# Wu0409/DuPL

Hardware: AMD Instinct MI355X
Metric: training img/s at 448^2, VOC dual-student ViT-B/16, phase B step (higher is better)
Workload: dtype f32 storage / accumulation / results; Linear GEMMs (forward, dgrad, wgrad), attention (forward, backward) and the decoder convs as fp32-equivalent f16x3 split products on the f16 MFMA (operands as fp16 hi / lo planes, 3 products per block, fp32 accumulate; error vs fp64 <= the f32 MFMA kernels'); CA

## Files before the change

### dupl_amd/csrc/attn_split.hip

```cpp
#include "common.h"
#include <type_traits>
#include "../../include/dupl_hip.h"

#ifndef ATT_PRIO
#define ATT_PRIO 0
#endif
#ifndef ATT_ABL
#define ATT_ABL 0
#endif

namespace {

typedef _Float16 h8 __attribute__((ext_vector_type(8)));
typedef _Float16 h4 __attribute__((ext_vector_type(4)));
typedef float f32x2 __attribute__((ext_vector_type(2)));
template <int N, int I = 0, class F>
__device__ __forceinline__ void static_for(F&& f) {
    if constexpr (I < N) {
        f(std::integral_constant<int, I>{});
        static_for<N, I + 1>(f);
    }
}
constexpr float LO_INV = 1.f / DUPL_LO_SCALE;
constexpr int HD = 64, KT = 64;
constexpr int PLANE = KT * 128;
constexpr int STAGE = 4 * PLANE;

#define MFMA16(a, b, c) __builtin_amdgcn_mfma_f32_32x32x16_f16((a), (b), (c), 0, 0, 0)

__device__ __forceinline__ float fast_exp(float x) { return __builtin_amdgcn_exp2f(x * 1.4426950408889634f); }

__device__ __forceinline__ void xcd_remap3(int remap, int& bx, int& by, int& bz) {
    bx = blockIdx.x; by = blockIdx.y; bz = blockIdx.z;
    if (!remap) return;
    const int gx = gridDim.x, gy = gridDim.y;
    const int total = gx * gy * gridDim.z;
    const int L = bx + gx * (by + gy * bz);
    const int q = total >> 3, r = total & 7;
    const int xcd = L & 7, idx = L >> 3;
    const int w = (xcd < r ? xcd * (q + 1) : r * (q + 1) + (xcd - r) * q) + idx;
    bx = w % gx;
    by = (w / gx) % gy;
    bz = w / (gx * gy);
}

struct AttnSegs {
    int n;
    int row0[DUPL_ATTN_SEGS_MAX], B[DUPL_ATTN_SEGS_MAX], N[DUPL_ATTN_SEGS_MAX], B_f32[DUPL_ATTN_SEGS_MAX], first[DUPL_ATTN_SEGS_MAX + 1];
    float* out[DUPL_ATTN_SEGS_MAX];
    float* lse[DUPL_ATTN_SEGS_MAX];
};

__global__ __launch_bounds__(256, 2) void attn_fwd16_kernel(const __half* __restrict__ qkv_hi, const __half* __restrict__ qkv_lo,
                                                            __half* __restrict__ out_hi, __half* __restrict__ out_lo,
                                                            const AttnSegs segs, int H, float scale, int remap, float out_scale) {
    __shared__ __attribute__((aligned(1024))) char smem[2 * STAGE];
    const int tid = threadIdx.x, lane = tid & 63, l31 = lane & 31, hf = lane >> 5;
    const int wave = __builtin_amdgcn_readfirstlane(tid >> 6);
    int sg = 0;
#pragma unroll 1
    while (sg + 1 < segs.n && (int)blockIdx.x >= segs.first[sg + 1]) ++sg;
    sg = __builtin_amdgcn_readfirstlane(sg);
    const int N = segs.N[sg], B_f32 = segs.B_f32[sg];
    float* __restrict__ out = segs.out[sg];
    float* __restrict__ lse = segs.lse[sg];
    int bx, h, b;
    {
        const int gx = (N + 127) / 128;
        const int G = gx * H * segs.B[sg];
        const int L = (int)blockIdx.x - segs.first[sg];
        int w = L;
        if (remap) {
            const int q = G >> 3, r = G & 7;
            const int xcd = L & 7, idx = L >> 3;
            w = (xcd < r ? xcd * (q + 1) : r * (q + 1) + (xcd - r) * q) + idx;
        }
        bx = w % gx; h = (w / gx) % H; b = w / (gx * H);
    }
    {
        const size_t r0 = (size_t)segs.row0[sg];
        qkv_hi += r0 * (size_t)(3 * H * HD);
        qkv_lo += r0 * (size_t)(3 * H * HD);
        if (out_hi) { out_hi += r0 * (size_t)(H * HD); out_lo += r0 * (size_t)(H * HD); }
    }
    const int q0 = bx * 128 + wave * 32;
    const int D = H * HD, ld = 3 * D;
    const int qrow = q0 + l31;
    const bool wave_active = q0 < N;

    h8 qh[4], ql[4];
    {
        const size_t off = ((size_t)b * N + min(qrow, N - 1)) * ld + h * HD + 8 * hf;
#pragma unroll
        for (int s = 0; s < 4; ++s) {
            qh[s] = *reinterpret_cast<const h8*>(qkv_hi + off + 16 * s);
            ql[s] = *reinterpret_cast<const h8*>(qkv_lo + off + 16 * s);
        }
    }

    const int prow = lane >> 3, pch = lane & 7;
    const char* kbase[2];
    kbase[0] = reinterpret_cast<const char*>(qkv_hi + (size_t)b * N * ld + D + h * HD);
    kbase[1] = reinterpret_cast<const char*>(qkv_lo + (size_t)b * N * ld + D + h * HD);
    const char* vbase[2];
    vbase[0] = kbase[0] + D * 2;
    vbase[1] = kbase[1] + D * 2;
    int krow[2], kch[2], vrow[2];
    const int vch = ((lane >> 5) * 32 + (lane & 3) * 8) * 2;
#pragma unroll
    for (int j = 0; j < 2; ++j) {
        const int r = 8 * (wave + 4 * j) + prow;
        const int c = pch ^ ((r >> 1) & 7);
        krow[j] = r;
        kch[j] = c * 16;
        const int q = wave + 4 * j, srow = (lane >> 2) & 7;
        vrow[j] = (q >> 1) * 16 + (srow >> 2) * 8 + (q & 1) * 4 + (srow & 3);
    }
    const size_t tstride = (size_t)KT * ld * 2;
    unsigned koff[2], voff[2];
#pragma unroll
    for (int j = 0; j < 2; ++j) {
        koff[j] = (unsigned)krow[j] * (unsigned)(ld * 2) + kch[j];
        voff[j] = (unsigned)vrow[j] * (unsigned)(ld * 2) + vch;
    }
    auto dma16 = [](const char* ubase, const unsigned off, char* dst) __attribute__((always_inline)) {
        __builtin_amdgcn_global_load_lds((const __attribute__((address_space(1))) void*)(ubase + off),
                                         (__attribute__((address_space(3))) void*)dst, 16, 0, 0);
    };
    auto issue = [&](int t, int buf) __attribute__((always_inline)) {
        char* dst = smem + buf * STAGE + wave * 1024;
        const size_t o = t * tstride;
        if (t * KT + KT <= N) {
#pragma unroll
            for (int i = 0; i < 4; ++i) dma16(kbase[i >> 1] + o, koff[i & 1], dst + i * 4096);
#pragma unroll
            for (int i = 0; i < 4; ++i) dma16(vbase[i >> 1] + o, voff[i & 1], dst + (4 + i) * 4096);
        } else {
#pragma unroll
            for (int i = 0; i < 4; ++i)
                dma16(kbase[i >> 1] + o, (unsigned)(min(t * KT + krow[i & 1], N - 1) - t * KT) * (unsigned)(ld * 2) + kch[i & 1], dst + i * 4096);
#pragma unroll
            for (int i = 0; i < 4; ++i)
                dma16(vbase[i >> 1] + o, (unsigned)(min(t * KT + vrow[i & 1], N - 1) - t * KT) * (unsigned)(ld * 2) + vch, dst + (4 + i) * 4096);
        }
    };

    const int g4 = (l31 >> 2) & 3;
    const int krow_a = (l31 & ~12) | ((g4 == 1 ? 2 : (g4 == 2 ? 1 : g4)) << 2);
    const int k_off = krow_a * 128, k_sw = (krow_a >> 1) & 7;
    const int vg = lane >> 4, vq = lane & 15;
    const unsigned v_lds = (unsigned)(uintptr_t)((__attribute__((address_space(3))) char*)smem) + 2 * PLANE +
                           ((vg >> 1) * 4 + (vq >> 2)) * 64 + (16 * (vg & 1) + 4 * (vq & 3)) * 2;

    f32x16 oM[2], oX[2];
#pragma unroll
    for (int d = 0; d < 2; ++d)
#pragma unroll
        for (int e = 0; e < 16; ++e) { oM[d][e] = 0.f; oX[d][e] = 0.f; }
    float m_run = -INFINITY, l_run = 0.f;

    const int nkt = (N + KT - 1) / KT;
    long long tph[4] = {0, 0, 0, 0}, tlast = 0;
    if (ATT_ABL & 16) tlast = clock64();
#define ATT_STAMP(i)                                  \
    if (ATT_ABL & 16) {                               \
        const long long now_ = clock64();             \
        tph[i] += now_ - tlast;                       \
        tlast = now_;                                 \
    }
    issue(0, 0);
    for (int t = 0; t < nkt; ++t) {
        asm volatile("s_waitcnt vmcnt(0)" ::: "memory");
        __syncthreads();
        if (t + 1 < nkt) issue(t + 1, (t + 1) & 1);
        if (!wave_active) continue;
        const char* st = smem + (t & 1) * STAGE;
        ATT_STAMP(0)

        f32x16 sM[2], sX[2];
        const f32x16 zero16 = {0.f, 0.f, 0.f, 0.f, 0.f, 0.f, 0.f, 0.f, 0.f, 0.f, 0.f, 0.f, 0.f, 0.f, 0.f, 0.f};
        h8 kh[2][2], kl[2][2];
        auto k_read = [&](const int sstep, h8(&fh)[2], h8(&fl)[2]) __attribute__((always_inline)) {
            const int ch = ((2 * sstep + hf) ^ k_sw) * 16;
#pragma unroll
            for (int kt2 = 0; kt2 < 2; ++kt2) {
                fh[kt2] = *reinterpret_cast<const h8*>(st + kt2 * 4096 + k_off + ch);
                fl[kt2] = *reinterpret_cast<const h8*>(st + PLANE + kt2 * 4096 + k_off + ch);
            }
        };
        k_read(0, kh[0], kl[0]);
        __builtin_amdgcn_s_setprio(ATT_PRIO);
#pragma unroll
        for (int sstep = 0; sstep < 4; ++sstep) {
            const int cur = sstep & 1;
            if (sstep + 1 < 4) k_read(sstep + 1, kh[cur ^ 1], kl[cur ^ 1]);
            __builtin_amdgcn_sched_barrier(0);
            sM[0] = MFMA16(kh[cur][0], qh[sstep], sstep == 0 ? zero16 : sM[0]);
            sM[1] = MFMA16(kh[cur][1], qh[sstep], sstep == 0 ? zero16 : sM[1]);
            sX[0] = MFMA16(kh[cur][0], ql[sstep], sstep == 0 ? zero16 : sX[0]);
            sX[1] = MFMA16(kh[cur][1], ql[sstep], sstep == 0 ? zero16 : sX[1]);
            sX[0] = MFMA16(kl[cur][0], qh[sstep], sX[0]);
            sX[1] = MFMA16(kl[cur][1], qh[sstep], sX[1]);
            __builtin_amdgcn_sched_barrier(0);
        }
        __builtin_amdgcn_s_setprio(0);
        if (ATT_ABL & 16) { asm volatile("" ::"v"(sM[0]), "v"(sM[1]), "v"(sX[0]), "v"(sX[1])); }
        ATT_STAMP(1)
        h4 vf[2][8];
        const unsigned v_st = v_lds + (t & 1) * STAGE;
        auto tr_read = [](const unsigned addr, auto offc) __attribute__((always_inline)) {
            h4 v;
            asm volatile("ds_read_b64_tr_b16 %0, %1 offset:%2" : "=v"(v) : "v"(addr), "n"(decltype(offc)::value) : "memory");
            return v;
        };
        auto v_read = [&](auto sgc, h4(&f)[8]) __attribute__((always_inline)) {
            constexpr int SG = decltype(sgc)::value;
            static_for<8>([&](auto ic) __attribute__((always_inline)) {
                constexpr int i = decltype(ic)::value, pl = i >> 2, dd = (i >> 1) & 1, jj = i & 1;
                f[i] = tr_read(v_st, std::integral_constant<int, pl * PLANE + ((SG * 2 + jj) * 2 + dd) * 512>{});
            });
        };
        v_read(std::integral_constant<int, 0>{}, vf[0]);
        const float c1 = scale * 1.4426950408889634f, c2 = c1 * LO_INV;
        if (t == nkt - 1) {
            const int kbase_t = t * KT + 8 * hf;
#pragma unroll
            for (int kt2 = 0; kt2 < 2; ++kt2)
#pragma unroll
                for (int e = 0; e < 16; ++e)
                    if (kbase_t + 32 * kt2 + 16 * (e >> 3) + (e & 7) >= N) sM[kt2][e] = -INFINITY;
        }
        float mx = -INFINITY;
#pragma unroll
        for (int kt2 = 0; kt2 < 2; ++kt2)
#pragma unroll
            for (int e = 0; e < 16; ++e) mx = fmaxf(mx, sM[kt2][e]);
        {
            typedef unsigned u2v __attribute__((ext_vector_type(2)));
            const u2v sw = __builtin_amdgcn_permlane32_swap(__float_as_uint(mx), __float_as_uint(mx), false, false);
            mx = fmaxf(__uint_as_float(sw[0]), __uint_as_float(sw[1])) * c1;
        }
        const float m_cand = fmaxf(m_run, mx);
        const bool move = __builtin_amdgcn_ballot_w64(m_cand - m_run > 8.f) != 0;
        const float m_run2 = move ? m_cand : m_run;
        const float m_new = m_run2 == -INFINITY ? 0.f : m_run2;
        const float alpha = __builtin_amdgcn_exp2f(m_run - m_new);
        f32x2 psum2 = {0.f, 0.f};
        h8 ph[4], pl[4];
        typedef _Float16 h2v __attribute__((ext_vector_type(2)));
#pragma unroll
        for (int kt2 = 0; kt2 < 2; ++kt2)
#pragma unroll
            for (int e = 0; e < 16; e += 2) {
                const f32x2 m2 = {sM[kt2][e], sM[kt2][e + 1]}, x2 = {sX[kt2][e], sX[kt2][e + 1]};
                const f32x2 v2 = __builtin_elementwise_fma(x2, f32x2{c2, c2}, __builtin_elementwise_fma(m2, f32x2{c1, c1}, f32x2{-m_new, -m_new}));
                const f32x2 p2 = {__builtin_amdgcn_exp2f(v2[0]), __builtin_amdgcn_exp2f(v2[1])};
                psum2 += p2;
                const h2v hh = __builtin_convertvector(p2, h2v);
                const f32x2 q2 = p2 * f32x2{DUPL_LO_SCALE, DUPL_LO_SCALE};
                const int idx = 2 * kt2 + (e >> 3);
                ph[idx][e & 7] = hh[0];
                ph[idx][(e & 7) + 1] = hh[1];
                pl[idx][e & 7] = (_Float16)__builtin_fmaf((float)hh[0], -DUPL_LO_SCALE, q2[0]);
                pl[idx][(e & 7) + 1] = (_Float16)__builtin_fmaf((float)hh[1], -DUPL_LO_SCALE, q2[1]);
            }
        const float psum = psum2[0] + psum2[1];
        l_run = l_run * alpha + psum;
        if (move) {
#pragma unroll
            for (int d = 0; d < 2; ++d)
#pragma unroll
                for (int e = 0; e < 16; ++e) { oM[d][e] *= alpha; oX[d][e] *= alpha; }
        }
        m_run = m_run2;
        if (ATT_ABL & 16) { asm volatile("" ::"v"(ph[0]), "v"(ph[3]), "v"(pl[0]), "v"(pl[3]), "v"(oM[0]), "v"(oX[1])); }
        ATT_STAMP(2)
        __builtin_amdgcn_s_setprio(ATT_PRIO);
        static_for<4>([&](auto sgc) __attribute__((always_inline)) {
            constexpr int sg = decltype(sgc)::value, cur = sg & 1;
            if constexpr (sg + 1 < 4) {
                v_read(std::integral_constant<int, sg + 1>{}, vf[cur ^ 1]);
                asm volatile("s_waitcnt lgkmcnt(8)" ::: "memory");
            } else {
                asm volatile("s_waitcnt lgkmcnt(0)" ::: "memory");
            }
            __builtin_amdgcn_sched_barrier(0);
            const h4(&f)[8] = vf[cur];
            const h8 vh0 = __builtin_shufflevector(f[0], f[1], 0, 1, 2, 3, 4, 5, 6, 7), vh1 = __builtin_shufflevector(f[2], f[3], 0, 1, 2, 3, 4, 5, 6, 7);
            const h8 vl0 = __builtin_shufflevector(f[4], f[5], 0, 1, 2, 3, 4, 5, 6, 7), vl1 = __builtin_shufflevector(f[6], f[7], 0, 1, 2, 3, 4, 5, 6, 7);
            oM[0] = MFMA16(vh0, ph[sg], oM[0]);
            oM[1] = MFMA16(vh1, ph[sg], oM[1]);
            oX[0] = MFMA16(vh0, pl[sg], oX[0]);
            oX[1] = MFMA16(vh1, pl[sg], oX[1]);
            oX[0] = MFMA16(vl0, ph[sg], oX[0]);
            oX[1] = MFMA16(vl1, ph[sg], oX[1]);
            __builtin_amdgcn_sched_barrier(0);
        });
        __builtin_amdgcn_s_setprio(0);
        if (ATT_ABL & 16) { asm volatile("" ::"v"(oM[0]), "v"(oM[1]), "v"(oX[0]), "v"(oX[1])); }
        ATT_STAMP(3)
    }
    if ((ATT_ABL & 16) && lse && tid == 0) {
        long long* q = reinterpret_cast<long long*>(lse + (((size_t)gridDim.z * H * N + 1) & ~(size_t)1)) +
                       (size_t)(blockIdx.x + gridDim.x * (blockIdx.y + gridDim.y * blockIdx.z)) * 4;
        q[0] = tph[0]; q[1] = tph[1]; q[2] = tph[2]; q[3] = tph[3];
    }
    if (!wave_active) return;
    const float l_tot = l_run + __shfl_xor(l_run, 32, 64);
    const float inv = 1.f / l_tot;
    if (b >= B_f32) { out = nullptr; lse = nullptr; }
    if (qrow < N) {
        const size_t ro = ((size_t)b * N + qrow) * D + h * HD;
#pragma unroll
        for (int d = 0; d < 2; ++d)
#pragma unroll
            for (int g = 0; g < 4; ++g) {
                float v[4];
#pragma unroll
                for (int j = 0; j < 4; ++j) v[j] = (oM[d][4 * g + j] + oX[d][4 * g + j] * LO_INV) * inv;
                const int col = d * 32 + 8 * g + 4 * hf;
                if (out) *reinterpret_cast<float4*>(out + ro + col) = make_float4(v[0], v[1], v[2], v[3]);
                if (out_hi) {
                    __half hh[4], ll[4];
#pragma unroll
                    for (int j = 0; j < 4; ++j) {
                        if (out_scale > 0.f) split_f32_u(v[j] * out_scale, hh[j], ll[j]);
                        else split_f32(v[j], hh[j], ll[j]);
                    }
                    *reinterpret_cast<uint2*>(out_hi + ro + col) = *reinterpret_cast<const uint2*>(hh);
                    *reinterpret_cast<uint2*>(out_lo + ro + col) = *reinterpret_cast<const uint2*>(ll);
                }
            }
        if (lse && hf == 0) lse[((size_t)b * H + h) * N + qrow] = m_run * 0.6931471805599453f + logf(l_tot);
    }
}


}

constexpr int g_attn16_remap = 1;

static int attn_fwd16_launch(const void* qkv_hi, const void* qkv_lo, void* out_hi, void* out_lo, const dupl_attn_seg* sv, int32_t n,
                             int32_t H, int32_t hd, float scale, int32_t out_exp, dupl_stream_t s) {
    if (out_exp < 0 || out_exp > 15 || !sv || n < 1 || n > DUPL_ATTN_SEGS_MAX) return DUPL_ERR_ARG;
    if (!qkv_hi || !qkv_lo || ((out_hi == nullptr) != (out_lo == nullptr)) || H <= 0 || hd != HD) return DUPL_ERR_ARG;
    auto al16 = [](const void* q) { return (reinterpret_cast<uintptr_t>(q) & 15) == 0; };
    if (!al16(qkv_hi) || !al16(qkv_lo)) return DUPL_ERR_ARG;
    int order[DUPL_ATTN_SEGS_MAX];
    for (int i = 0; i < n; ++i) order[i] = i;
    for (int i = 1; i < n; ++i)
        for (int j = i; j > 0 && sv[order[j]].N > sv[order[j - 1]].N; --j) { const int t = order[j]; order[j] = order[j - 1]; order[j - 1] = t; }
    AttnSegs g;
    g.n = n;
    int total = 0;
    for (int k = 0; k < n; ++k) {
        const dupl_attn_seg& q = sv[order[k]];
        int bf = q.B_f32 == 0 ? q.B : q.B_f32;
        if (q.B <= 0 || q.N <= 0 || q.row0 < 0 || bf < 0 || bf > q.B || (!q.out && !out_hi) || (bf < q.B && q.out && !out_hi)) return DUPL_ERR_ARG;
        g.row0[k] = (int)q.row0; g.B[k] = q.B; g.N[k] = q.N; g.B_f32[k] = bf; g.out[k] = q.out; g.lse[k] = q.lse;
        g.first[k] = total;
        total += ((q.N + 127) / 128) * H * q.B;
    }
    g.first[n] = total;
    DUPL_LAUNCH(attn_fwd16_kernel, dim3((unsigned)total), dim3(256), 0, (hipStream_t)s, (const __half*)qkv_hi, (const __half*)qkv_lo,
                       (__half*)out_hi, (__half*)out_lo, g, H, scale, g_attn16_remap, out_exp ? ldexpf(1.f, out_exp) : 0.f);
    return dupl_launch_status();
}

extern "C" int dupl_attention_fwd16(const void* qkv_hi, const void* qkv_lo, float* out, void* out_hi, void* out_lo, float* lse,
                                    int32_t B, int32_t N, int32_t H, int32_t hd, float scale, int32_t B_f32, int32_t out_exp,
                                    dupl_stream_t s) {
    if (B_f32 < 0 || B_f32 > B || (B_f32 != 0 && B_f32 < B && !out_hi) || (!out && !out_hi)) return DUPL_ERR_ARG;
    dupl_attn_seg q;
    q.row0 = 0; q.B = B; q.N = N; q.B_f32 = B_f32; q.out = out; q.lse = lse;
    return attn_fwd16_launch(qkv_hi, qkv_lo, out_hi, out_lo, &q, 1, H, hd, scale, out_exp, s);
}

extern "C" int dupl_attention_fwd16_segs(const void* qkv_hi, const void* qkv_lo, void* out_hi, void* out_lo, const dupl_attn_seg* segs,
                                         int32_t n, int32_t H, int32_t hd, float scale, int32_t out_exp, dupl_stream_t s) {
    return attn_fwd16_launch(qkv_hi, qkv_lo, out_hi, out_lo, segs, n, H, hd, scale, out_exp, s);
}
```

### dupl_amd/csrc/attn_split_bwd.hip

```cpp
#include "common.h"
#include "../../include/dupl_hip.h"

namespace {

typedef _Float16 h8 __attribute__((ext_vector_type(8)));
typedef _Float16 h4 __attribute__((ext_vector_type(4)));
constexpr float LO_INV = 1.f / DUPL_LO_SCALE;
constexpr int HD = 64, TT = 32;
constexpr int PL = 4096;
constexpr int MAXN = 2048;

#define MFMA16(a, b, c) __builtin_amdgcn_mfma_f32_32x32x16_f16((a), (b), (c), 0, 0, 0)

__device__ __forceinline__ float fast_exp(float x) { return __builtin_amdgcn_exp2f(x * 1.4426950408889634f); }

__device__ __forceinline__ void xcd_remap3(int remap, int& bx, int& by, int& bz) {
    bx = blockIdx.x; by = blockIdx.y; bz = blockIdx.z;
    if (!remap) return;
    const int gx = gridDim.x, gy = gridDim.y;
    const int total = gx * gy * gridDim.z;
    const int L = bx + gx * (by + gy * bz);
    const int q = total >> 3, r = total & 7;
    const int xcd = L & 7, idx = L >> 3;
    const int w = (xcd < r ? xcd * (q + 1) : r * (q + 1) + (xcd - r) * q) + idx;
    bx = w % gx;
    by = (w / gx) % gy;
    bz = w / (gx * gy);
}

__device__ __forceinline__ void dma16(const char* src, char* dst) {
    __builtin_amdgcn_global_load_lds((const __attribute__((address_space(1))) void*)src,
                                     (__attribute__((address_space(3))) void*)dst, 16, 0, 0);
}

__device__ __forceinline__ int pi_row(int r) {
    const int g = (r >> 2) & 3;
    return (r & ~12) | ((g == 1 ? 2 : (g == 2 ? 1 : g)) << 2);
}

__device__ __forceinline__ int km_piece_row(int wave, int lane) {
    const int srow = (lane >> 2) & 7;
    return (wave >> 1) * 16 + (srow >> 2) * 8 + (wave & 1) * 4 + (srow & 3);
}
__device__ __forceinline__ int km_piece_col_bytes(int lane) { return ((lane >> 5) * 32 + (lane & 3) * 8) * 2; }
__device__ __forceinline__ int km_read_lane_off(int lane) {
    const int g = lane >> 4, q = lane & 15;
    return ((g >> 1) * 4 + (q >> 2)) * 64 + (16 * (g & 1) + 4 * (q & 3)) * 2;
}
template <int OFF>
__device__ __forceinline__ h4 km_tr_read(const unsigned addr) {
    h4 v;
    asm volatile("ds_read_b64_tr_b16 %0, %1 offset:%2" : "=v"(v) : "v"(addr), "n"(OFF) : "memory");
    return v;
}
__device__ __forceinline__ void km_read_tile(const unsigned base_hi, h4 (&f)[8][2]) {
#define KM_RD(SG, DD, PLN, JJ) f[((SG) * 2 + (DD)) * 2 + (PLN)][JJ] = km_tr_read<(PLN) * PL + (((SG) * 2 + (JJ)) * 2 + (DD)) * 512>(base_hi)
    KM_RD(0, 0, 0, 0); KM_RD(0, 0, 0, 1); KM_RD(0, 0, 1, 0); KM_RD(0, 0, 1, 1);
    KM_RD(0, 1, 0, 0); KM_RD(0, 1, 0, 1); KM_RD(0, 1, 1, 0); KM_RD(0, 1, 1, 1);
    KM_RD(1, 0, 0, 0); KM_RD(1, 0, 0, 1); KM_RD(1, 0, 1, 0); KM_RD(1, 0, 1, 1);
    KM_RD(1, 1, 0, 0); KM_RD(1, 1, 0, 1); KM_RD(1, 1, 1, 0); KM_RD(1, 1, 1, 1);
#undef KM_RD
}
__device__ __forceinline__ void km_wait(h4 (&f)[8][2]) {
    asm volatile("s_waitcnt lgkmcnt(0)"
                 : "+v"(f[0][0]), "+v"(f[0][1]), "+v"(f[1][0]), "+v"(f[1][1]), "+v"(f[2][0]), "+v"(f[2][1]), "+v"(f[3][0]), "+v"(f[3][1]),
                   "+v"(f[4][0]), "+v"(f[4][1]), "+v"(f[5][0]), "+v"(f[5][1]), "+v"(f[6][0]), "+v"(f[6][1]), "+v"(f[7][0]), "+v"(f[7][1])
                 :
                 : "memory");
    __builtin_amdgcn_sched_barrier(0);
}
__device__ __forceinline__ h8 h8of(const h4 lo, const h4 hi) { return __builtin_shufflevector(lo, hi, 0, 1, 2, 3, 4, 5, 6, 7); }

__device__ __forceinline__ void split_regs(const f32x16& v, h8 (&hi)[2], h8 (&lo)[2]) {
    typedef _Float16 h2v __attribute__((ext_vector_type(2)));
    typedef float f2v __attribute__((ext_vector_type(2)));
#pragma unroll
    for (int e = 0; e < 16; e += 2) {
        const f2v x2 = {v[e], v[e + 1]};
        const h2v hh = __builtin_convertvector(x2, h2v);
        const f2v q2 = x2 * f2v{DUPL_LO_SCALE, DUPL_LO_SCALE};
        hi[e >> 3][e & 7] = hh[0];
        hi[e >> 3][(e & 7) + 1] = hh[1];
        lo[e >> 3][e & 7] = (_Float16)__builtin_fmaf((float)hh[0], -DUPL_LO_SCALE, q2[0]);
        lo[e >> 3][(e & 7) + 1] = (_Float16)__builtin_fmaf((float)hh[1], -DUPL_LO_SCALE, q2[1]);
    }
}

__device__ __forceinline__ void attn_bwd_amax_flush(unsigned int* amax_out, float amx) {
    if (!amax_out) return;
    amx = wave_max(amx);
    if ((threadIdx.x & 63) == 0 && amx > 0.f) atomicMax(amax_out, __float_as_uint(amx));
}

__global__ __launch_bounds__(256) void delta_kernel(const float* __restrict__ out, const float* __restrict__ dout,
                                                    float* __restrict__ delta, int B, int N, int H) {
    const long idx = (long)blockIdx.x * blockDim.x + threadIdx.x;
    const long total = (long)B * N * H;
    if (idx >= total) return;
    const int h = (int)(idx % H);
    const long bn = idx / H;
    const int n = (int)(bn % N), b = (int)(bn / N);
    const float4* o = reinterpret_cast<const float4*>(out + bn * (long)(H * HD) + h * HD);
    const float4* d = reinterpret_cast<const float4*>(dout + bn * (long)(H * HD) + h * HD);
    float s = 0.f;
#pragma unroll
    for (int i = 0; i < HD / 4; ++i) {
        const float4 a = o[i], c = d[i];
        s += (a.x * c.x + a.y * c.y) + (a.z * c.z + a.w * c.w);
    }
    delta[((long)b * H + h) * N + n] = s;
}

__device__ __forceinline__ void attn_bwd16_dq_body(char* __restrict__ smem, const int bx, const int h, const int b,
                                                   const __half* __restrict__ qkv_hi, const __half* __restrict__ qkv_lo,
                                                   const __half* __restrict__ do_hi, const __half* __restrict__ do_lo,
                                                   const float* __restrict__ lse, const float* __restrict__ delta,
                                                   const float* __restrict__ slot, float* __restrict__ dqkv, unsigned int* __restrict__ amax_out, int N, int H,
                                                   float scale) {
    constexpr int STAGE = 6 * PL;
    const int tid = threadIdx.x, lane = tid & 63, wave = tid >> 6, l31 = lane & 31, hf = lane >> 5;
    const int q0 = bx * 128 + wave * 32;
    const int D = H * HD, ld = 3 * D;
    const int qrow = q0 + l31;
    const bool wave_active = q0 < N, qv = qrow < N;
    const float s_do = slot[0], inv_s = slot[1];

    h8 qh[4], ql[4], oh[4], ol[4];
    {
        const int rr = min(qrow, N - 1);
        const size_t qo = ((size_t)b * N + rr) * ld + h * HD + 8 * hf;
        const size_t oo = ((size_t)b * N + rr) * D + h * HD + 8 * hf;
#pragma unroll
        for (int s = 0; s < 4; ++s) {
            qh[s] = *reinterpret_cast<const h8*>(qkv_hi + qo + 16 * s);
            ql[s] = *reinterpret_cast<const h8*>(qkv_lo + qo + 16 * s);
            oh[s] = *reinterpret_cast<const h8*>(do_hi + oo + 16 * s);
            ol[s] = *reinterpret_cast<const h8*>(do_lo + oo + 16 * s);
        }
    }
    const float my_lse = qv ? lse[((size_t)b * H + h) * N + qrow] : 0.f;
    const float my_delta = qv ? delta[((size_t)b * H + h) * N + qrow] * s_do : 0.f;

    const int rrow = 8 * wave + (lane >> 3), rch = ((lane & 7) ^ ((rrow >> 1) & 7)) * 16;
    const int trow = km_piece_row(wave, lane), tcb = km_piece_col_bytes(lane);
    const char* k_hi = reinterpret_cast<const char*>(qkv_hi + (size_t)b * N * ld + D + h * HD);
    const char* k_lo = reinterpret_cast<const char*>(qkv_lo + (size_t)b * N * ld + D + h * HD);
    auto issue = [&](int t, int buf) __attribute__((always_inline)) {
        char* dst = smem + buf * STAGE + wave * 1024;
        const size_t ro = (size_t)min(t * TT + rrow, N - 1) * (ld * 2) + rch;
        dma16(k_hi + ro, dst);
        dma16(k_lo + ro, dst + PL);
        dma16(k_hi + ro + D * 2, dst + 2 * PL);
        dma16(k_lo + ro + D * 2, dst + 3 * PL);
        const size_t to = (size_t)min(t * TT + trow, N - 1) * (ld * 2) + tcb;
        dma16(k_hi + to, dst + 4 * PL);
        dma16(k_lo + to, dst + 5 * PL);
    };
    const int prow = pi_row(l31);
    const int a_off = prow * 128, a_sw = (prow >> 1) & 7;
    const unsigned km_lds = (unsigned)(uintptr_t)((__attribute__((address_space(3))) char*)smem) + 4 * PL + km_read_lane_off(lane);

    f32x16 dqM[2], dqX[2];
#pragma unroll
    for (int d = 0; d < 2; ++d)
#pragma unroll
        for (int e = 0; e < 16; ++e) { dqM[d][e] = 0.f; dqX[d][e] = 0.f; }

    const int nkt = (N + TT - 1) / TT;
    issue(0, 0);
    for (int t = 0; t < nkt; ++t) {
        asm volatile("s_waitcnt vmcnt(0)" ::: "memory");
        __syncthreads();
        if (t + 1 < nkt) issue(t + 1, (t + 1) & 1);
        if (!wave_active) continue;
        const char* st = smem + (t & 1) * STAGE;
        f32x16 sM, sX, pM, pX;
#pragma unroll
        for (int e = 0; e < 16; ++e) { sM[e] = 0.f; sX[e] = 0.f; pM[e] = 0.f; pX[e] = 0.f; }
#pragma unroll
        for (int s = 0; s < 4; ++s) {
            const int ch = ((2 * s + hf) ^ a_sw) * 16;
            const h8 kh = *reinterpret_cast<const h8*>(st + a_off + ch);
            const h8 kl = *reinterpret_cast<const h8*>(st + PL + a_off + ch);
            const h8 vh = *reinterpret_cast<const h8*>(st + 2 * PL + a_off + ch);
            const h8 vl = *reinterpret_cast<const h8*>(st + 3 * PL + a_off + ch);
            sM = MFMA16(kh, qh[s], sM);
            sX = MFMA16(kh, ql[s], sX);
            sX = MFMA16(kl, qh[s], sX);
            pM = MFMA16(vh, oh[s], pM);
            pX = MFMA16(vh, ol[s], pX);
            pX = MFMA16(vl, oh[s], pX);
        }
        const int kb = t * TT + 8 * hf;
        f32x16 ds;
#pragma unroll
        for (int e = 0; e < 16; ++e) {
            const bool kvld = kb + 16 * (e >> 3) + (e & 7) < N;
            const float sv = (sM[e] + sX[e] * LO_INV) * scale;
            const float p = kvld ? fast_exp(sv - my_lse) : 0.f;
            ds[e] = __fmul_rn(p, __fsub_rn(pM[e] + pX[e] * LO_INV, my_delta));
        }
        h4 kf[8][2];
        km_read_tile(km_lds + (t & 1) * STAGE, kf);
        h8 dh[2], dl[2];
        split_regs(ds, dh, dl);
        km_wait(kf);
#pragma unroll
        for (int sg = 0; sg < 2; ++sg) {
#pragma unroll
            for (int d = 0; d < 2; ++d) {
                const h8 th = h8of(kf[(sg * 2 + d) * 2][0], kf[(sg * 2 + d) * 2][1]);
                const h8 tl = h8of(kf[(sg * 2 + d) * 2 + 1][0], kf[(sg * 2 + d) * 2 + 1][1]);
                dqM[d] = MFMA16(th, dh[sg], dqM[d]);
                dqX[d] = MFMA16(th, dl[sg], dqX[d]);
                dqX[d] = MFMA16(tl, dh[sg], dqX[d]);
            }
        }
    }
    float amx = 0.f;
    if (wave_active && qv) {
        const float f = scale * inv_s;
        float* op = dqkv + ((size_t)b * N + qrow) * ld + h * HD;
#pragma unroll
        for (int d = 0; d < 2; ++d)
#pragma unroll
            for (int g = 0; g < 4; ++g) {
                float4 v;
                v.x = (dqM[d][4 * g + 0] + dqX[d][4 * g + 0] * LO_INV) * f;
                v.y = (dqM[d][4 * g + 1] + dqX[d][4 * g + 1] * LO_INV) * f;
                v.z = (dqM[d][4 * g + 2] + dqX[d][4 * g + 2] * LO_INV) * f;
                v.w = (dqM[d][4 * g + 3] + dqX[d][4 * g + 3] * LO_INV) * f;
                amx = fmaxf(fmaxf(amx, fmaxf(fabsf(v.x), fabsf(v.y))), fmaxf(fabsf(v.z), fabsf(v.w)));
                *reinterpret_cast<float4*>(op + d * 32 + 8 * g + 4 * hf) = v;
            }
    }
    attn_bwd_amax_flush(amax_out, amx);
}

template <int MODE>
__device__ __forceinline__ void attn_bwd16_dkv_body(char* __restrict__ smem, const int bx, const int h, const int b,
                                                    const __half* __restrict__ qkv_hi, const __half* __restrict__ qkv_lo,
                                                    const __half* __restrict__ do_hi, const __half* __restrict__ do_lo,
                                                    const float* __restrict__ lse, const float* __restrict__ delta,
                                                    const float* __restrict__ slot, float* __restrict__ dqkv, unsigned int* __restrict__ amax_out, int N, int H,
                                                    float scale) {
    constexpr int NPL = MODE == 0 ? 4 : 6;
    constexpr int STAGE = NPL * PL;
    float* Ls = reinterpret_cast<float*>(smem + 2 * STAGE);
    float* Ds = Ls + MAXN;
    const int tid = threadIdx.x, lane = tid & 63, wave = tid >> 6, l31 = lane & 31, hf = lane >> 5;
    const int k0 = bx * 128 + wave * 32;
    const int D = H * HD, ld = 3 * D;
    const int krow = k0 + l31;
    const bool wave_active = k0 < N, kv = krow < N;
    const float s_do = slot[0], inv_s = slot[1];

    for (int i = tid; i < N; i += 256) {
        Ls[i] = lse[((size_t)b * H + h) * N + i];
        if (MODE == 1) Ds[i] = delta[((size_t)b * H + h) * N + i] * s_do;
    }

    h8 kh[4], kl[4], vh[4], vl[4];
    {
        const size_t ko = ((size_t)b * N + min(krow, N - 1)) * ld + D + h * HD + 8 * hf;
#pragma unroll
        for (int s = 0; s < 4; ++s) {
            kh[s] = *reinterpret_cast<const h8*>(qkv_hi + ko + 16 * s);
            kl[s] = *reinterpret_cast<const h8*>(qkv_lo + ko + 16 * s);
            if (MODE == 1) {
                vh[s] = *reinterpret_cast<const h8*>(qkv_hi + ko + D + 16 * s);
                vl[s] = *reinterpret_cast<const h8*>(qkv_lo + ko + D + 16 * s);
            }
        }
    }

    const int rrow = 8 * wave + (lane >> 3), rch = ((lane & 7) ^ ((rrow >> 1) & 7)) * 16;
    const int trow = km_piece_row(wave, lane), tcb = km_piece_col_bytes(lane);
    const char* q_hi = reinterpret_cast<const char*>(qkv_hi + (size_t)b * N * ld + h * HD);
    const char* q_lo = reinterpret_cast<const char*>(qkv_lo + (size_t)b * N * ld + h * HD);
    const char* o_hi = reinterpret_cast<const char*>(do_hi + (size_t)b * N * D + h * HD);
    const char* o_lo = reinterpret_cast<const char*>(do_lo + (size_t)b * N * D + h * HD);
    auto issue = [&](int t, int buf) __attribute__((always_inline)) {
        char* dst = smem + buf * STAGE + wave * 1024;
        const int rr = min(t * TT + rrow, N - 1);
        dma16(q_hi + (size_t)rr * (ld * 2) + rch, dst);
        dma16(q_lo + (size_t)rr * (ld * 2) + rch, dst + PL);
        if (MODE == 1) {
            dma16(o_hi + (size_t)rr * (D * 2) + rch, dst + 2 * PL);
            dma16(o_lo + (size_t)rr * (D * 2) + rch, dst + 3 * PL);
        }
        const int tr = min(t * TT + trow, N - 1);
        if (MODE == 0) {
            dma16(o_hi + (size_t)tr * (D * 2) + tcb, dst + (NPL - 2) * PL);
            dma16(o_lo + (size_t)tr * (D * 2) + tcb, dst + (NPL - 1) * PL);
        } else {
            dma16(q_hi + (size_t)tr * (ld * 2) + tcb, dst + (NPL - 2) * PL);
            dma16(q_lo + (size_t)tr * (ld * 2) + tcb, dst + (NPL - 1) * PL);
        }
    };
    const int prow = pi_row(l31);
    const int a_off = prow * 128, a_sw = (prow >> 1) & 7;
    const unsigned km_lds = (unsigned)(uintptr_t)((__attribute__((address_space(3))) char*)smem) + (NPL - 2) * PL + km_read_lane_off(lane);

    f32x16 gM[2], gX[2];
#pragma unroll
    for (int d = 0; d < 2; ++d)
#pragma unroll
        for (int e = 0; e < 16; ++e) { gM[d][e] = 0.f; gX[d][e] = 0.f; }

    const int nqt = (N + TT - 1) / TT;
    issue(0, 0);
    for (int t = 0; t < nqt; ++t) {
        asm volatile("s_waitcnt vmcnt(0)" ::: "memory");
        __syncthreads();
        if (t + 1 < nqt) issue(t + 1, (t + 1) & 1);
        if (!wave_active) continue;
        const char* st = smem + (t & 1) * STAGE;
        f32x16 sM, sX, pM, pX;
#pragma unroll
        for (int e = 0; e < 16; ++e) { sM[e] = 0.f; sX[e] = 0.f; pM[e] = 0.f; pX[e] = 0.f; }
#pragma unroll
        for (int s = 0; s < 4; ++s) {
            const int ch = ((2 * s + hf) ^ a_sw) * 16;
            const h8 ah = *reinterpret_cast<const h8*>(st + a_off + ch);
            const h8 al = *reinterpret_cast<const h8*>(st + PL + a_off + ch);
            sM = MFMA16(ah, kh[s], sM);
            sX = MFMA16(ah, kl[s], sX);
            sX = MFMA16(al, kh[s], sX);
            if (MODE == 1) {
                const h8 bh = *reinterpret_cast<const h8*>(st + 2 * PL + a_off + ch);
                const h8 bl = *reinterpret_cast<const h8*>(st + 3 * PL + a_off + ch);
                pM = MFMA16(bh, vh[s], pM);
                pX = MFMA16(bh, vl[s], pX);
                pX = MFMA16(bl, vh[s], pX);
            }
        }
        const int qb = t * TT + 8 * hf;
        f32x16 w;
#pragma unroll
        for (int e = 0; e < 16; ++e) {
            const int qi = qb + 16 * (e >> 3) + (e & 7);
            const bool ok = qi < N && kv;
            const int qc = min(qi, N - 1);
            const float sv = (sM[e] + sX[e] * LO_INV) * scale;
            const float p = ok ? fast_exp(sv - Ls[qc]) : 0.f;
            w[e] = MODE == 0 ? p : __fmul_rn(p, __fsub_rn(pM[e] + pX[e] * LO_INV, Ds[qc]));
        }
        h4 xf[8][2];
        km_read_tile(km_lds + (t & 1) * STAGE, xf);
        h8 wh[2], wl[2];
        split_regs(w, wh, wl);
        km_wait(xf);
#pragma unroll
        for (int sg = 0; sg < 2; ++sg) {
#pragma unroll
            for (int d = 0; d < 2; ++d) {
                const h8 th = h8of(xf[(sg * 2 + d) * 2][0], xf[(sg * 2 + d) * 2][1]);
                const h8 tl = h8of(xf[(sg * 2 + d) * 2 + 1][0], xf[(sg * 2 + d) * 2 + 1][1]);
                gM[d] = MFMA16(th, wh[sg], gM[d]);
                gX[d] = MFMA16(th, wl[sg], gX[d]);
                gX[d] = MFMA16(tl, wh[sg], gX[d]);
            }
        }
    }
    float amx = 0.f;
    if (wave_active && kv) {
        const float f = MODE == 0 ? inv_s : scale * inv_s;
        float* op = dqkv + ((size_t)b * N + krow) * ld + (MODE == 0 ? 2 * D : D) + h * HD;
#pragma unroll
        for (int d = 0; d < 2; ++d)
#pragma unroll
            for (int g = 0; g < 4; ++g) {
                float4 v;
                v.x = (gM[d][4 * g + 0] + gX[d][4 * g + 0] * LO_INV) * f;
                v.y = (gM[d][4 * g + 1] + gX[d][4 * g + 1] * LO_INV) * f;
                v.z = (gM[d][4 * g + 2] + gX[d][4 * g + 2] * LO_INV) * f;
                v.w = (gM[d][4 * g + 3] + gX[d][4 * g + 3] * LO_INV) * f;
                amx = fmaxf(fmaxf(amx, fmaxf(fabsf(v.x), fabsf(v.y))), fmaxf(fabsf(v.z), fabsf(v.w)));
                *reinterpret_cast<float4*>(op + d * 32 + 8 * g + 4 * hf) = v;
            }
    }
    attn_bwd_amax_flush(amax_out, amx);
}

constexpr int ATTNB_LDS = 2 * 6 * PL + 2 * MAXN * 4;
__global__ __launch_bounds__(256, 2) void attn_bwd16_all_kernel(const __half* __restrict__ qkv_hi, const __half* __restrict__ qkv_lo,
                                                                const __half* __restrict__ do_hi, const __half* __restrict__ do_lo,
                                                                const float* __restrict__ lse, const float* __restrict__ delta,
                                                                const float* __restrict__ slot, float* __restrict__ dqkv,
                                                                unsigned int* __restrict__ amax_out, int N, int H, int B, float scale,
                                                                int remap) {
    __shared__ __attribute__((aligned(1024))) char smem[ATTNB_LDS];
    const int gx = (N + 127) / 128;
    const int G = gx * H * B;
    const int role = __builtin_amdgcn_readfirstlane((int)blockIdx.x / G);
    const int L = (int)blockIdx.x - role * G;
    int w = L;
    if (remap) {
        const int q = G >> 3, r = G & 7;
        const int xcd = L & 7, idx = L >> 3;
        w = (xcd < r ? xcd * (q + 1) : r * (q + 1) + (xcd - r) * q) + idx;
    }
    const int bx = w % gx, h = (w / gx) % H, b = w / (gx * H);
    if (role == 0) attn_bwd16_dkv_body<1>(smem, bx, h, b, qkv_hi, qkv_lo, do_hi, do_lo, lse, delta, slot, dqkv, amax_out, N, H, scale);
    else if (role == 1) attn_bwd16_dq_body(smem, bx, h, b, qkv_hi, qkv_lo, do_hi, do_lo, lse, delta, slot, dqkv, amax_out, N, H, scale);
    else attn_bwd16_dkv_body<0>(smem, bx, h, b, qkv_hi, qkv_lo, do_hi, do_lo, lse, delta, slot, dqkv, amax_out, N, H, scale);
}

}

constexpr int g_attnb16_remap = 1;

extern "C" int dupl_attention_bwd16(const void* qkv_hi, const void* qkv_lo, const float* out, const float* dout, const void* do_hi,
                                    const void* do_lo, const float* do_slot, const float* lse, float* delta, float* dqkv, int32_t B,
                                    int32_t N, int32_t H, int32_t hd, float scale, void* amax_out, dupl_stream_t stream) {
    unsigned int* ax = static_cast<unsigned int*>(amax_out);
    if (!qkv_hi || !qkv_lo || !out || !dout || !do_hi || !do_lo || !do_slot || !lse || !delta || !dqkv || B <= 0 || N <= 0 ||
        N > MAXN || H <= 0 || hd != HD)
        return DUPL_ERR_ARG;
    hipStream_t s = (hipStream_t)stream;
    const long total = (long)B * N * H;
    DUPL_LAUNCH(delta_kernel, dim3((unsigned)((total + 255) / 256)), dim3(256), 0, s, out, dout, delta, B, N, H);
    const unsigned blocks = 3u * (unsigned)(((N + 127) / 128) * H * B);
    DUPL_LAUNCH(attn_bwd16_all_kernel, dim3(blocks), dim3(256), 0, s, (const __half*)qkv_hi, (const __half*)qkv_lo,
                       (const __half*)do_hi, (const __half*)do_lo, lse, delta, do_slot, dqkv, ax, N, H, B, scale, g_attnb16_remap);
    return dupl_launch_status();
}
```

### dupl_amd/engine.py

```python
from __future__ import annotations

import os
from dataclasses import dataclass, field
from typing import Dict, List, Optional, Tuple

import torch

from . import ops

Tensor = torch.Tensor

GEMM_MODE = os.environ.get("DUPL_GEMM", "f16x3")


def set_gemm_mode(mode: str):
    global GEMM_MODE
    assert mode in ("f32", "f16x3"), mode
    GEMM_MODE = mode


@dataclass(frozen=True)
class EncoderConfig:
    embed_dim: int = 768
    depth: int = 12
    num_heads: int = 12
    mlp_ratio: int = 4
    patch: int = 16
    img_size: int = 224
    aux_layer: int = -3
    ln_eps: float = 1e-6
    head_classes: int = 1000
    decoder_dim: int = 512
    decoder_dilation: int = 5

    @property
    def grid(self) -> int:
        return self.img_size // self.patch

    @property
    def head_dim(self) -> int:
        return self.embed_dim // self.num_heads


def student_param_shapes(cfg: EncoderConfig, num_classes: int) -> Dict[str, Tuple[int, ...]]:
    D, Hd = cfg.embed_dim, cfg.embed_dim * cfg.mlp_ratio
    s: Dict[str, Tuple[int, ...]] = {}
    s["encoder.cls_token"] = (1, 1, D)
    s["encoder.pos_embed"] = (1, cfg.grid * cfg.grid + 1, D)
    s["encoder.patch_embed.proj.weight"] = (D, 3, cfg.patch, cfg.patch)
    s["encoder.patch_embed.proj.bias"] = (D,)
    for i in range(cfg.depth):
        p = f"encoder.blocks.{i}."
        s[p + "norm1.weight"] = (D,)
        s[p + "norm1.bias"] = (D,)
        s[p + "attn.qkv.weight"] = (3 * D, D)
        s[p + "attn.qkv.bias"] = (3 * D,)
        s[p + "attn.proj.weight"] = (D, D)
        s[p + "attn.proj.bias"] = (D,)
        s[p + "norm2.weight"] = (D,)
        s[p + "norm2.bias"] = (D,)
        s[p + "mlp.fc1.weight"] = (Hd, D)
        s[p + "mlp.fc1.bias"] = (Hd,)
        s[p + "mlp.fc2.weight"] = (D, Hd)
        s[p + "mlp.fc2.bias"] = (D,)
    s["encoder.norm.weight"] = (D,)
    s["encoder.norm.bias"] = (D,)
    s["encoder.head.weight"] = (cfg.head_classes, D)
    s["encoder.head.bias"] = (cfg.head_classes,)
    s["decoder.conv6.weight"] = (cfg.decoder_dim, D, 3, 3)
    s["decoder.conv7.weight"] = (cfg.decoder_dim, cfg.decoder_dim, 3, 3)
    s["decoder.conv8.weight"] = (num_classes, cfg.decoder_dim, 1, 1)
    s["classifier.weight"] = (num_classes - 1, D, 1, 1)
    s["aux_classifier.weight"] = (num_classes - 1, D, 1, 1)
    return s


SEG_FROZEN, SEG_BACKBONE, SEG_NORM, SEG_CLS, SEG_DECODER = 0, 1, 2, 3, 4


def param_segment(key: str) -> int:
    if key in ("encoder.pos_embed", "encoder.head.weight", "encoder.head.bias"):
        return SEG_FROZEN
    if key.startswith("encoder."):
        return SEG_NORM if "norm" in key[len("encoder."):] else SEG_BACKBONE
    if key.startswith("decoder."):
        return SEG_DECODER
    return SEG_CLS


FMT1 = os.environ.get("DUPL_FMT1", "1") != "0"
KM_BWD = os.environ.get("DUPL_KM_BWD", "1") != "0"
SK_DGRAD = os.environ.get("DUPL_SK_DGRAD", "1") != "0"
WGRAD_GROUP = os.environ.get("DUPL_WGRAD_GROUP", "1") != "0"

SK_DGRAD_MAX_COLS = 1024
ZERO_WS = os.environ.get("DUPL_ZERO_WS", "1") != "0"
FUSED_PLANES = os.environ.get("DUPL_ADAMW_PLANES", "1") != "0"
MERGED_PASS = int(os.environ.get("DUPL_MERGED_PASS", "16384"))
ATTN_SEGS = int(os.environ.get("DUPL_ATTN_SEGS", "1536"))


class FlatStorage:

    def __init__(self, cfg: EncoderConfig, num_classes: int, n_students: int, device="cpu"):
        self.cfg, self.num_classes, self.n_students = cfg, num_classes, n_students
        shapes = student_param_shapes(cfg, num_classes)
        self.shapes = shapes
        self.layout: Dict[str, Tuple[int, int]] = {}
        self.seg_bounds: List[Tuple[int, int]] = []
        off = 0
        for seg in range(5):
            start = off
            for k, shp in shapes.items():
                if param_segment(k) != seg:
                    continue
                n = 1
                for d in shp:
                    n *= d
                self.layout[k] = (off, n)
                off += (n + 7) // 8 * 8
            self.seg_bounds.append((start, off))
        self.student_numel = off
        self.data = torch.zeros(n_students * off, dtype=torch.float32, device=device)
        self.grad = torch.zeros(n_students * off, dtype=torch.float32, device=device)
        self.seg_has_grad = [[False] * 5 for _ in range(n_students)]
        self.streams: List = []
        self.version_anchor = None
        self.gemm16_tuning = dict(ops.GEMM16_TUNING)
        self.data16: Optional[Tensor] = None
        self.dirty = 0
        self.rewrites = 0
        self._w16_key = [None] * n_students
        self._planes_fresh: Dict = {}
        self._w16T: Dict = {}
        self._w16F0: Dict = {}
        self.guard = RangeGuard(self)

    def wait_streams(self):
        if self.streams:
            cur = torch.cuda.current_stream()
            for s in self.streams:
                cur.wait_stream(s)

    def view(self, student: int, key: str, grad: bool = False) -> Tensor:
        off, n = self.layout[key]
        base = student * self.student_numel + off
        buf = self.grad if grad else self.data
        return buf[base:base + n].view(self.shapes[key])

    def apply(self, fn):
        self.data = fn(self.data)
        self.grad = fn(self.grad)
        self.data16 = None
        self._w16_key = [None] * self.n_students
        self._w16T = {}

    def mark_dirty(self, rewritten: bool = False):
        self.dirty += 1
        if rewritten:
            self.rewrites += 1

    def _param_key(self):
        a = self.version_anchor
        return (self.data._version + (a._version if a is not None else 0), self.dirty, self.data.data_ptr(), self.rewrites)

    def planes_current(self, student: int) -> bool:
        return FUSED_PLANES and self.data16 is not None and self._w16_key[student] == self._param_key()

    def plane_pointers(self, offset: int, seg: int):
        lo, hi = self.seg_bounds[seg]
        assert lo <= offset % self.student_numel < max(hi, lo + 1), \
            f"offset {offset} is not inside segment {seg}: the optimiser's ranges must be the plane-format ranges of ensure_w16"
        return (self.data16.data_ptr() + 2 * offset, self.data16.data_ptr() + 2 * (self.data.numel() + offset),
                ops.EXP_W if (FMT1 and seg == SEG_BACKBONE) else 0)

    def planes_written(self, student: int):
        self._planes_fresh[student] = self._param_key()

    def ensure_w16(self, student: int):
        key = self._param_key()
        if self._w16_key[student] == key and self.data16 is not None:
            return
        if self.data16 is None or self.data16.device != self.data.device:
            self.data16 = torch.empty((2, self.data.numel()), device=self.data.device, dtype=torch.float16)
            self._w16_key = [None] * self.n_students
            self._planes_fresh = {}
        n, base = self.student_numel, student * self.student_numel
        tot = self.data.numel()
        if self._planes_fresh.get(student) == key:
            pass
        elif FMT1:
            b0, b1 = self.seg_bounds[SEG_BACKBONE]
            for lo_, hi_, e in ((0, b0, 0), (b0, b1, ops.EXP_W), (b1, n, 0)):
                if hi_ > lo_:
                    o = base + lo_
                    args = (self.data.data_ptr() + 4 * o, self.data16.data_ptr() + 2 * o, self.data16.data_ptr() + 2 * (tot + o), hi_ - lo_)
                    if e:
                        ops.L().dupl_split_f16x2b(*args, e, ops._stream())
                    else:
                        ops.L().dupl_split_f16x2(*args, ops._stream())
        else:
            ops.L().dupl_split_f16x2(self.data.data_ptr() + 4 * base, self.data16.data_ptr() + 2 * base,
                                     self.data16.data_ptr() + 2 * (tot + base), n, ops._stream())
        old = self._w16_key[student]
        self._w16_key[student] = key
        self.guard.params_changed(student, rewritten=(old is None or old[0] != key[0] or old[2] != key[2] or old[3] != key[3]),
                                  key=key)

    def w16T(self, student: int, key: str, rows: int):
        ver = self._param_key()
        hit = self._w16T.get((student, key))
        if hit is not None and hit[0] == ver:
            return hit[1]
        w = self.view(student, key).view(rows, -1)
        _, T, _ = ops.split_prepare(w, scaled=False, want_rm=False, want_T=True, rows_pad=rows)
        self._w16T[(student, key)] = (ver, T)
        return T

    def w16T_missing(self, student: int, keys_rows):
        ver = self._param_key()
        out = []
        for key, rows in keys_rows:
            hit = self._w16T.get((student, key))
            if hit is None or hit[0] != ver:
                out.append((key, rows, self.view(student, key).view(rows, -1)))
        return out

    def w16T_put(self, student: int, key: str, T):
        self._w16T[(student, key)] = (self._param_key(), T)

    def w16(self, student: int, key: str, rows: int, fmt1: Optional[bool] = None) -> "ops.W16":
        off, n = self.layout[key]
        base = student * self.student_numel + off
        p = self.data16.data_ptr()
        have = ops.EXP_W if (FMT1 and param_segment(key) == SEG_BACKBONE) else 0
        if fmt1 is None:
            fmt1 = bool(have)
        if bool(have) == bool(fmt1):
            return ops.W16(p + 2 * base, p + 2 * (self.data.numel() + base), rows, n // rows, have)
        assert not fmt1
        ver = self._param_key()
        hit = self._w16F0.get((student, key))
        if hit is None or hit[0] != ver:
            hit = (ver, ops.split16(self.view(student, key).view(rows, -1)))
            self._w16F0[(student, key)] = hit
        return hit[1]

    def trainable_range(self, student: int) -> Tuple[int, int]:
        s = student * self.student_numel
        return s + self.seg_bounds[SEG_BACKBONE][0], s + self.seg_bounds[SEG_DECODER][1]

    def block_range(self, i: int) -> Tuple[int, int]:
        pre = f"encoder.blocks.{i}."
        offs = [(o, n) for k, (o, n) in self.layout.items() if k.startswith(pre) and param_segment(k) == SEG_BACKBONE]
        return min(o for o, _ in offs), max((o + n + 7) // 8 * 8 for o, n in offs)

    def grad_buckets(self, student: int, blocks_per_bucket: int = 2) -> List[Tuple[int, int, object]]:
        s = student * self.student_numel
        depth = self.cfg.depth
        k = max(1, int(blocks_per_bucket))
        out = [(s + self.seg_bounds[SEG_CLS][0], s + self.seg_bounds[SEG_DECODER][1], "heads")]
        i = depth
        while i - k > 0:
            out.append((s + self.block_range(i - k)[0], s + self.block_range(i - 1)[1], i - k))
            i -= k
        out.append((s + self.seg_bounds[SEG_BACKBONE][0], s + self.block_range(i - 1)[1], "stem"))
        out.append((s + self.seg_bounds[SEG_NORM][0], s + self.seg_bounds[SEG_NORM][1], "stem"))
        return out


F16_MAX = 65504.0


class RangeGuard:

    SITES = ("qkv", "attn", "proj", "fc1", "fc2")

    def __init__(self, store: "FlatStorage", margin: float = 2.0, period: int = 8):
        self.store, self.margin, self.period = store, float(margin), int(period)
        cfg = store.cfg
        self.entries: List[Tuple[str, int, int]] = []
        D, Hd, dd = cfg.embed_dim, cfg.embed_dim * cfg.mlp_ratio, cfg.decoder_dim

        def add(key, rows):
            n = store.layout[key][1]
            self.entries.append((key, rows, n // rows))

        add("encoder.patch_embed.proj.weight", D)
        for i in range(cfg.depth):
            p = f"encoder.blocks.{i}."
            for k, r in ((p + "norm1.weight", 1), (p + "norm1.bias", 1), (p + "attn.qkv.weight", 3 * D), (p + "attn.qkv.bias", 1),
                         (p + "attn.proj.weight", D), (p + "norm2.weight", 1), (p + "norm2.bias", 1), (p + "mlp.fc1.weight", Hd),
                         (p + "mlp.fc1.bias", 1), (p + "mlp.fc2.weight", D)):
                add(k, r)
        for k, r in (("encoder.norm.weight", 1), ("encoder.norm.bias", 1), ("decoder.conv6.weight", dd), ("decoder.conv7.weight", dd)):
            add(k, r)
        self.index = {k: i for i, (k, _, _) in enumerate(self.entries)}
        self._table = None
        self._dev_out = None
        self._host = None
        self._event = None
        self._pending = False
        self._steps = [0] * store.n_students
        self.safe: List[Optional[dict]] = [None] * store.n_students
        self.headroom = float("inf")
        self.headroom1 = float("inf")
        self.checks = 0
        self._checked_key = None

    def _ensure_buffers(self):
        dev = self.store.data.device
        if self._table is None or self._table.device != dev:
            import numpy as np
            tab = np.zeros((len(self.entries), 2), dtype=np.int64)
            for i, (k, rows, cols) in enumerate(self.entries):
                tab[i, 0] = self.store.layout[k][0]
                tab[i, 1] = rows | (cols << 32)
            self._table = torch.from_numpy(tab).to(dev)
            self._dev_out = torch.zeros((self.store.n_students, len(self.entries), 2), device=dev, dtype=torch.float32)
            self._host = torch.zeros((self.store.n_students, len(self.entries), 2), dtype=torch.float32).pin_memory()
            self._event = torch.cuda.Event()

    def _launch(self, students):
        self._ensure_buffers()
        st = self.store
        for s in students:
            ops.L().dupl_param_bounds(st.data.data_ptr() + 4 * s * st.student_numel, self._table.data_ptr(), len(self.entries),
                                      self._dev_out[s].data_ptr(), ops._stream())
        self._host.copy_(self._dev_out, non_blocking=True)
        self._event.record()
        self._pending = True

    def _harvest(self, wait: bool):
        if not self._pending:
            return
        if wait:
            self._event.synchronize()
        elif not self._event.query():
            return
        self._pending = False
        self.headroom = self.headroom1 = float("inf")
        for s in range(self.store.n_students):
            self.safe[s] = self._decide(self._host[s].double().numpy())
        self.checks += 1

    def _decide(self, v):
        cfg = self.store.cfg
        sq = float(cfg.embed_dim) ** 0.5
        lim = F16_MAX / self.margin
        ix = self.index
        worst = [0.0]

        def ok(*bounds):
            good = True
            for b in bounds:
                b = float(b)
                if not (b <= lim):
                    good = False
                if b == b:
                    worst[0] = max(worst[0], b)
            return good

        def amax(k):
            return v[ix[k], 0]

        def rown(k):
            return v[ix[k], 1]

        sw = 2.0 ** ops.EXP_W
        worst1 = [0.0]

        def exp1(ea_, ew_):
            if not FMT1 or not (ew_ * sw <= lim):
                worst1[0] = max(worst1[0], ew_ * sw if FMT1 else 0.0)
                return 0
            for e in range(ops.EXP_ACT, 0, -1):
                if ea_ * 2.0 ** e <= lim:
                    worst1[0] = max(worst1[0], ea_ * 2.0 ** e, ew_ * sw)
                    return e
            worst1[0] = max(worst1[0], ea_ * 2.0)
            return 0

        wp = amax("encoder.patch_embed.proj.weight")
        out = {"patch": ok(wp), "blocks": []}
        out["patch_f1"] = exp1(3.0, wp) if out["patch"] else 0
        for i in range(cfg.depth):
            p = f"encoder.blocks.{i}."
            g1, g2 = amax(p + "norm1.weight"), amax(p + "norm2.weight")
            el1, n1 = g1 * sq + amax(p + "norm1.bias"), g1 * sq + rown(p + "norm1.bias")
            el2, n2 = g2 * sq + amax(p + "norm2.bias"), g2 * sq + rown(p + "norm2.bias")
            e_qkv = n1 * rown(p + "attn.qkv.weight") + amax(p + "attn.qkv.bias")
            e_h = n2 * rown(p + "mlp.fc1.weight") + amax(p + "mlp.fc1.bias")
            ops_ = {"qkv": (el1, amax(p + "attn.qkv.weight")), "proj": (e_qkv, amax(p + "attn.proj.weight")),
                    "fc1": (el2, amax(p + "mlp.fc1.weight")), "fc2": (e_h, amax(p + "mlp.fc2.weight"))}
            blk = {"attn": ok(e_qkv)}
            for site, (ea_, ew_) in ops_.items():
                blk[site] = ok(ea_, ew_)
                blk[site + "_f1"] = exp1(ea_, ew_) if blk[site] else 0
            out["blocks"].append(blk)
        gf = amax("encoder.norm.weight")
        elf, nf = gf * sq + amax("encoder.norm.bias"), gf * sq + rown("encoder.norm.bias")
        e_c6 = 3.0 * nf * rown("decoder.conv6.weight")
        out["conv6"] = ok(elf, amax("decoder.conv6.weight"))
        out["conv7"] = ok(e_c6, amax("decoder.conv7.weight"))
        self.headroom = min(self.headroom, float(lim / max(worst[0], 1e-30)))
        self.headroom1 = min(self.headroom1, float(lim / max(worst1[0], 1e-30)))
        return out

    def params_changed(self, student: int, rewritten: bool, key=None):
        if rewritten or self.safe[student] is None:
            if key is not None and key == self._checked_key and self.safe[student] is not None:
                return
            self._launch(range(self.store.n_students))
            self._harvest(wait=True)
            self._steps = [0] * self.store.n_students
            self._checked_key = key
            return
        self._steps[student] += 1
        if student == 0 and self._steps[0] % self.period == 0:
            self._harvest(wait=True)
            self._launch(range(self.store.n_students))

    def sites(self, student: int) -> dict:
        if self.safe[student] is None:
            self._launch(range(self.store.n_students))
            self._harvest(wait=True)
        return self.safe[student]

    def summary(self) -> dict:
        n = n0 = 0
        for s in self.safe:
            if s is None:
                continue
            n += sum(not s[k] for k in ("patch", "conv6", "conv7")) + sum(not b[k] for b in s["blocks"] for k in self.SITES)
            if FMT1:
                n0 += int(s["patch"] and not s["patch_f1"]) + sum(b[k] and not b[k + "_f1"] for b in s["blocks"]
                                                                  for k in ("qkv", "proj", "fc1", "fc2"))
        return {"sites_on_f32": n, "sites_on_fmt0": n0, "checks": self.checks, "margin": self.margin,
                "headroom": (None if self.headroom == float("inf") else round(self.headroom, 1)),
                "headroom_fmt1": (None if self.headroom1 == float("inf") else round(self.headroom1, 1))}



def _lin16(P: "StudentParams", *a, **kw):
    return ops.linear16(*a, tuning=P.store.gemm16_tuning, **kw)


class StudentParams:

    def __init__(self, store: FlatStorage, student: int):
        self.store, self.student = store, student
        self.cfg, self.num_classes = store.cfg, store.num_classes
        self.w = {k: store.view(student, k) for k in store.layout}
        self.g = {k: store.view(student, k, grad=True) for k in store.layout}
        self._pos_cache: Dict[Tuple[int, int], Tensor] = {}
        self._pos_version = None

    def pos_embed_for(self, h: int, w: int) -> Tensor:
        pe = self.w["encoder.pos_embed"]
        ver = (pe._version, pe.data_ptr())
        if ver != self._pos_version:
            self._pos_cache.clear()
            self._pos_version = ver
        key = (h, w)
        if key not in self._pos_cache:
            self._pos_cache[key] = ops.pos_embed_resize(pe, self.cfg.grid, h, w)
        return self._pos_cache[key]

    def mark_grad(self, seg: int):
        self.store.seg_has_grad[self.student][seg] = True

    def w16(self, key: str, rows: int, fmt1: Optional[bool] = None):
        return self.store.w16(self.student, key, rows, fmt1)

    def w16T(self, key: str, rows: int):
        return self.store.w16T(self.student, key, rows)


@dataclass
class BlockSaved:
    x_in: Tensor = None
    mean1: Tensor = None
    rstd1: Tensor = None
    ln1: Tensor = None
    qkv: Tensor = None
    lse: Tensor = None
    att: Tensor = None
    x_mid: Tensor = None
    mean2: Tensor = None
    rstd2: Tensor = None
    ln2: Tensor = None
    pre1: Tensor = None
    h1: Tensor = None
    qkv16: object = None
    ln1_16: object = None
    att16: object = None
    ln2_16: object = None
    h1_16: object = None


@dataclass
class EncoderSaved:
    B: int = 0
    h: int = 0
    w: int = 0
    x_img: Tensor = None
    blocks: List[BlockSaved] = field(default_factory=list)
    x_last: Tensor = None
    mean_f: Tensor = None
    rstd_f: Tensor = None
    guard: dict = None


def encoder_forward(P: StudentParams, x: Tensor, save: bool, save_rows: int = 0):
    if GEMM_MODE == "f16x3":
        return _encoder_forward16(P, [x], save, save_rows)[0]
    cfg = P.cfg
    B, _, Himg, Wimg = x.shape
    h, w = Himg // cfg.patch, Wimg // cfg.patch
    n, D, H, hd = h * w, cfg.embed_dim, cfg.num_heads, cfg.head_dim
    N = n + 1
    W = P.w
    rows = ops.patch_im2row(x, cfg.patch)
    patch = ops.linear(rows, W["encoder.patch_embed.proj.weight"], W["encoder.patch_embed.proj.bias"])
    del rows
    t = ops.assemble_tokens(patch, W["encoder.cls_token"], P.pos_embed_for(h, w), B, n, D)
    del patch
    sv = EncoderSaved(B=B, h=h, w=w, x_img=x if save else None) if save else None
    aux_idx = cfg.aux_layer % cfg.depth
    aux = None
    scale = hd ** -0.5
    for i in range(cfg.depth):
        p = f"encoder.blocks.{i}."
        ln1, m1, r1 = ops.layernorm_fwd(t, W[p + "norm1.weight"], W[p + "norm1.bias"], cfg.ln_eps, save)
        qkv = ops.linear(ln1, W[p + "attn.qkv.weight"], W[p + "attn.qkv.bias"])
        att, lse = ops.attention_fwd(qkv, B, N, H, hd, scale, need_lse=save)
        x_mid = ops.linear(att, W[p + "attn.proj.weight"], W[p + "attn.proj.bias"], res=t)
        ln2, m2, r2 = ops.layernorm_fwd(x_mid, W[p + "norm2.weight"], W[p + "norm2.bias"], cfg.ln_eps, save)
        pre1 = torch.empty((t.shape[0], D * cfg.mlp_ratio), device=t.device, dtype=torch.float32) if save else None
        h1 = ops.linear(ln2, W[p + "mlp.fc1.weight"], W[p + "mlp.fc1.bias"], gelu=True, store_pre=pre1)
        x_out = ops.linear(h1, W[p + "mlp.fc2.weight"], W[p + "mlp.fc2.bias"], res=x_mid)
        if save:
            sv.blocks.append(BlockSaved(x_in=t, mean1=m1, rstd1=r1, ln1=ln1, qkv=qkv, lse=lse, att=att, x_mid=x_mid,
                                        mean2=m2, rstd2=r2, ln2=ln2, pre1=pre1, h1=h1))
        t = x_out
        if i == aux_idx and i != cfg.depth - 1:
            aux = t
    tf, mf, rf = ops.layernorm_fwd(t, W["encoder.norm.weight"], W["encoder.norm.bias"], cfg.ln_eps, save)
    if save:
        sv.x_last, sv.mean_f, sv.rstd_f = t, mf, rf
    if aux is None:
        aux = tf
    return tf, aux, sv


def _encoder_forward16(P: StudentParams, xs, save: bool, save_rows: int = 0, whole: bool = False):
    cfg = P.cfg
    D, H, hd = cfg.embed_dim, cfg.num_heads, cfg.head_dim
    W = P.w
    P.store.ensure_w16(P.student)
    guard = P.store.guard.sites(P.student)
    if save_rows and not partial_save_ok(P, guard):
        save_rows = 0
    assert not (save and len(xs) > 1 and not save_rows), "a merged pass can only save a row prefix of its first batch (partial_save_ok)"
    def ea(site_flags, site):
        return int(site_flags[site + "_f1"]) if FMT1 else 0
    toks, groups = [], []
    r0 = 0
    for x in xs:
        B, _, Himg, Wimg = x.shape
        h, w = Himg // cfg.patch, Wimg // cfg.patch
        n = h * w
        if guard["patch"]:
            e = ea(guard, "patch")
            rows16 = ops.split16(ops.patch_im2row(x, cfg.patch), exp=e)
            patch, _ = _lin16(P, rows16, P.w16("encoder.patch_embed.proj.weight", D, bool(e)), W["encoder.patch_embed.proj.bias"])
            del rows16
        else:
            patch = ops.linear(ops.patch_im2row(x, cfg.patch), W["encoder.patch_embed.proj.weight"], W["encoder.patch_embed.proj.bias"])
        toks.append(ops.assemble_tokens(patch, W["encoder.cls_token"], P.pos_embed_for(h, w), B, n, D))
        groups.append((r0, B, n + 1, h, w))
        r0 += B * (n + 1)
    t = torch.cat(toks, dim=0) if len(toks) > 1 else toks[0]
    del toks
    R = t.shape[0]
    sv = None
    if save:
        _, B, _, h, w = groups[0]
        sv = EncoderSaved(B=B, h=h, w=w, x_img=xs[0], guard=guard)
    aux_idx = cfg.aux_layer % cfg.depth
    aux = None
    scale = hd ** -0.5
    for i in range(cfg.depth):
        p = f"encoder.blocks.{i}."
        g = guard["blocks"][i]
        attn16 = hd == 64 and g["attn"]
        km = {st_: bool(save and KM_BWD and g[st_] and ea(g, st_) > 0) for st_ in ("qkv", "proj", "fc1", "fc2")}
        ln1, ln1_16, m1, r1 = ops.layernorm_fwd16(t, W[p + "norm1.weight"], W[p + "norm1.bias"], cfg.ln_eps, save,
                                                  want_f32=(save and not km["qkv"]) or not g["qkv"], f32_rows=save_rows,
                                                  exp=ea(g, "qkv"))
        lse = None
        need_qkv32 = (not attn16) or (save and groups[0][2] > 2048)
        if g["qkv"]:
            qkv, qkv16 = _lin16(P, ln1_16, P.w16(p + "attn.qkv.weight", 3 * D, bool(ln1_16.exp)), W[p + "attn.qkv.bias"],
                                      want_f32=need_qkv32, want16=attn16)
        else:
            qkv = ops.linear(ln1, W[p + "attn.qkv.weight"], W[p + "attn.qkv.bias"])
            qkv16 = ops.split16(qkv) if attn16 else None
        ln1_keep = ln1_16 if km["qkv"] else None
        del ln1_16
        need_att32 = save or not g["proj"]
        att = torch.empty((save_rows or R, D), device=t.device, dtype=torch.float32) if (need_att32 or not attn16) else None
        att16 = ops.split16_empty(R, D, t.device, ea(g, "proj")) if (attn16 and g["proj"]) else None
        lse = None
        use_segs = attn16 and 1 < len(groups) <= ops._lib.ATTN_SEGS_MAX and \
            sum(B_ * H * ((N_ + 127) // 128) for (_, B_, N_, _, _) in groups) <= ATTN_SEGS
        if use_segs:
            segs = []
            for gi, (g0, B, N, _, _) in enumerate(groups):
                planes_only = bool(save_rows and gi > 0) or att is None
                bf = save_rows // N if (save_rows and gi == 0) else 0
                segs.append((g0, B, N, None if planes_only else att[g0:g0 + (bf or B) * N], bool(save and gi == 0), bf))
            lse = ops.attention_fwd16_segs(qkv16, segs, H, hd, scale, out16=att16)[0]
        for gi, (g0, B, N, _, _) in enumerate(() if use_segs else groups):
            if attn16:
                if save_rows and gi > 0:
                    ops.attention_fwd16(qkv16.rows_slice(g0, g0 + B * N), B, N, H, hd, scale, need_lse=False, out=None,
                                        out16=att16.rows_slice(g0, g0 + B * N))
                    continue
                bf = save_rows // N if save_rows else 0
                lse_g = ops.attention_fwd16(qkv16.rows_slice(g0, g0 + B * N), B, N, H, hd, scale, need_lse=save,
                                            out=att[g0:g0 + (bf or B) * N] if att is not None else None,
                                            out16=att16.rows_slice(g0, g0 + B * N) if att16 is not None else None, b_f32=bf)
            else:
                _, lse_g = ops.attention_fwd(qkv[g0:g0 + B * N], B, N, H, hd, scale, need_lse=save, out=att[g0:g0 + B * N])
            if gi == 0:
                lse = lse_g
        if not attn16 and g["proj"]:
            att16 = ops.split16(att, exp=ea(g, "proj"))
        qkv16_keep = qkv16 if (save and attn16) else None
        del qkv16
        if g["proj"]:
            x_mid, _ = _lin16(P, att16, P.w16(p + "attn.proj.weight", D, bool(att16.exp)), W[p + "attn.proj.bias"], res=t)
        else:
            x_mid = ops.linear(att, W[p + "attn.proj.weight"], W[p + "attn.proj.bias"], res=t)
        att_keep = att16 if (km["proj"] and att16 is not None and att16.exp > 0) else None
        del att16
        ln2, ln2_16, m2, r2 = ops.layernorm_fwd16(x_mid, W[p + "norm2.weight"], W[p + "norm2.bias"], cfg.ln_eps, save,
                                                  want_f32=(save and not km["fc1"]) or not g["fc1"], f32_rows=save_rows,
                                                  exp=ea(g, "fc1"))
        pre1 = torch.empty((save_rows or R, D * cfg.mlp_ratio), device=t.device, dtype=torch.float32) if save else None
        if g["fc1"]:
            e2 = ea(g, "fc2") if ln2_16.exp else 0
            km["fc2"] = km["fc2"] and e2 > 0
            h1, h1_16 = _lin16(P, ln2_16, P.w16(p + "mlp.fc1.weight", D * cfg.mlp_ratio, bool(ln2_16.exp)), W[p + "mlp.fc1.bias"],
                                     gelu=True, store_pre=pre1, want_f32=(save and not km["fc2"]) or not g["fc2"], want16=g["fc2"],
                                     c_rows=save_rows, out_exp=e2)
        else:
            h1 = ops.linear(ln2, W[p + "mlp.fc1.weight"], W[p + "mlp.fc1.bias"], gelu=True, store_pre=pre1)
            h1_16 = ops.split16(h1, exp=ea(g, "fc2")) if g["fc2"] else None
            km["fc2"] = False
        ln2_keep = ln2_16 if km["fc1"] else None
        h1_keep = h1_16 if km["fc2"] else None
        del ln2_16
        if g["fc2"]:
            x_out, _ = _lin16(P, h1_16, P.w16(p + "mlp.fc2.weight", D, bool(h1_16.exp)), W[p + "mlp.fc2.bias"], res=x_mid)
        else:
            x_out = ops.linear(h1, W[p + "mlp.fc2.weight"], W[p + "mlp.fc2.bias"], res=x_mid)
        del h1_16
        if save:
            sv.blocks.append(BlockSaved(x_in=t, mean1=m1, rstd1=r1, ln1=ln1, qkv=qkv, lse=lse, att=att, x_mid=x_mid,
                                        mean2=m2, rstd2=r2, ln2=ln2, pre1=pre1, h1=h1, qkv16=qkv16_keep,
                                        ln1_16=ln1_keep, att16=att_keep, ln2_16=ln2_keep, h1_16=h1_keep))
        del ln1_keep, att_keep, ln2_keep, h1_keep
        t = x_out
        if i == aux_idx and i != cfg.depth - 1:
            aux = t
    tf, mf, rf = ops.layernorm_fwd(t, W["encoder.norm.weight"], W["encoder.norm.bias"], cfg.ln_eps, save)
    if save:
        sv.x_last, sv.mean_f, sv.rstd_f = t, mf, rf
    if aux is None:
        aux = tf
    outs = [(tf[g0:g0 + B * N], aux[g0:g0 + B * N], sv) for (g0, B, N, _, _) in groups]
    if whole:
        return outs, tf, aux
    return outs


def partial_save_ok(P: StudentParams, guard=None) -> bool:
    if GEMM_MODE != "f16x3" or P.cfg.head_dim != 64:
        return False
    guard = guard if guard is not None else P.store.guard.sites(P.student)
    return all(b[k] for b in guard["blocks"] for k in RangeGuard.SITES)


def cam_logits(P: StudentParams, x: Tensor):
    tf, aux, _ = encoder_forward(P, x, save=False)
    Wc = P.w["classifier.weight"].view(P.num_classes - 1, -1)
    Wa = P.w["aux_classifier.weight"].view(P.num_classes - 1, -1)
    cam = ops.linear(tf, Wc)
    cam_aux = ops.linear(aux, Wa)
    return cam_aux, cam


def cam_logits_multi(P: StudentParams, xs):
    cfg = P.cfg
    D, H, hd = cfg.embed_dim, cfg.num_heads, cfg.head_dim
    W = P.w
    if GEMM_MODE == "f16x3":
        C = P.num_classes - 1
        outs, tf_all, aux_all = _encoder_forward16(P, list(xs), save=False, whole=True)
        cam = ops.linear(tf_all, W["classifier.weight"].view(C, -1))
        cam_aux = ops.linear(aux_all, W["aux_classifier.weight"].view(C, -1))
        res, g0 = [], 0
        for o in outs:
            r = o[0].shape[0]
            res.append((cam_aux[g0:g0 + r], cam[g0:g0 + r]))
            g0 += r
        return res
    toks, groups = [], []
    r0 = 0
    for x in xs:
        B, _, Himg, Wimg = x.shape
        h, w = Himg // cfg.patch, Wimg // cfg.patch
        n = h * w
        rows = ops.patch_im2row(x, cfg.patch)
        patch = ops.linear(rows, W["encoder.patch_embed.proj.weight"], W["encoder.patch_embed.proj.bias"])
        toks.append(ops.assemble_tokens(patch, W["encoder.cls_token"], P.pos_embed_for(h, w), B, n, D))
        groups.append((r0, B, n + 1))
        r0 += B * (n + 1)
    t = torch.cat(toks, dim=0) if len(toks) > 1 else toks[0]
    del toks
    aux_idx = cfg.aux_layer % cfg.depth
    aux = None
    scale = hd ** -0.5
    for i in range(cfg.depth):
        p = f"encoder.blocks.{i}."
        ln1, _, _ = ops.layernorm_fwd(t, W[p + "norm1.weight"], W[p + "norm1.bias"], cfg.ln_eps, False)
        qkv = ops.linear(ln1, W[p + "attn.qkv.weight"], W[p + "attn.qkv.bias"])
        att = torch.empty((t.shape[0], D), device=t.device, dtype=torch.float32)
        for (g0, B, N) in groups:
            ops.attention_fwd(qkv[g0:g0 + B * N], B, N, H, hd, scale, out=att[g0:g0 + B * N])
        x_mid = ops.linear(att, W[p + "attn.proj.weight"], W[p + "attn.proj.bias"], res=t)
        ln2, _, _ = ops.layernorm_fwd(x_mid, W[p + "norm2.weight"], W[p + "norm2.bias"], cfg.ln_eps, False)
        h1 = ops.linear(ln2, W[p + "mlp.fc1.weight"], W[p + "mlp.fc1.bias"], gelu=True)
        t = ops.linear(h1, W[p + "mlp.fc2.weight"], W[p + "mlp.fc2.bias"], res=x_mid)
        if i == aux_idx and i != cfg.depth - 1:
            aux = t
    tf, _, _ = ops.layernorm_fwd(t, W["encoder.norm.weight"], W["encoder.norm.bias"], cfg.ln_eps, False)
    if aux is None:
        aux = tf
    C = P.num_classes - 1
    cam = ops.linear(tf, W["classifier.weight"].view(C, -1))
    cam_aux = ops.linear(aux, W["aux_classifier.weight"].view(C, -1))
    return [(cam_aux[g0:g0 + B * N], cam[g0:g0 + B * N]) for (g0, B, N) in groups]


@dataclass
class HeadSaved:
    enc: EncoderSaved = None
    tf: Tensor = None
    aux: Tensor = None
    pooled: Tensor = None
    pooled_idx: Tensor = None
    pooled_aux: Tensor = None
    pooled_aux_idx: Tensor = None
    col6: Tensor = None
    h6: Tensor = None
    col7: Tensor = None
    h7: Tensor = None
    guard: dict = None


def _prefix_saved(sv: EncoderSaved, b: int, rows: int) -> EncoderSaved:
    out = EncoderSaved(B=b, h=sv.h, w=sv.w, x_img=sv.x_img[:b], guard=sv.guard)
    for s in sv.blocks:
        def pre(t_):
            return t_[:rows] if t_ is not None else None

        out.blocks.append(BlockSaved(x_in=s.x_in[:rows], mean1=s.mean1[:rows], rstd1=s.rstd1[:rows], ln1=pre(s.ln1),
                                     qkv=s.qkv[:rows] if s.qkv is not None else None, lse=s.lse[:b], att=s.att[:rows],
                                     x_mid=s.x_mid[:rows],
                                     mean2=s.mean2[:rows], rstd2=s.rstd2[:rows], ln2=pre(s.ln2), pre1=s.pre1[:rows],
                                     h1=pre(s.h1), qkv16=s.qkv16.rows_slice(0, rows) if s.qkv16 is not None else None,
                                     ln1_16=s.ln1_16, att16=s.att16, ln2_16=s.ln2_16, h1_16=s.h1_16))
    out.x_last, out.mean_f, out.rstd_f = sv.x_last[:rows], sv.mean_f[:rows], sv.rstd_f[:rows]
    return out


def cam_logits_shared(P: StudentParams, x2: Tensor, b: int):
    C = P.num_classes - 1
    Wc = P.w["classifier.weight"].view(C, -1)
    Wa = P.w["aux_classifier.weight"].view(C, -1)
    rows = (x2.shape[0] // 2) * ((x2.shape[2] // P.cfg.patch) * (x2.shape[3] // P.cfg.patch) + 1)
    tf, aux, enc = encoder_forward(P, x2, save=True, save_rows=rows)
    cam = ops.linear(tf, Wc)
    cam_aux = ops.linear(aux, Wa)
    assert rows == tf.shape[0] // 2
    return cam_aux, cam, (tf[:rows], aux[:rows], _prefix_saved(enc, b, rows))


def cam_logits_shared_multi(P: StudentParams, xs, b: int):
    C = P.num_classes - 1
    n0 = (xs[0].shape[2] // P.cfg.patch) * (xs[0].shape[3] // P.cfg.patch) + 1
    rows = (xs[0].shape[0] // 2) * n0
    P.store.ensure_w16(P.student)
    if not partial_save_ok(P):
        cam_aux_t, cam_t, cache = cam_logits_shared(P, xs[0], b)
        return [(cam_aux_t, cam_t)] + (cam_logits_multi(P, xs[1:]) if len(xs) > 1 else []), cache
    outs, tf, aux = _encoder_forward16(P, list(xs), save=True, save_rows=rows, whole=True)
    enc = outs[0][2]
    cam = ops.linear(tf, P.w["classifier.weight"].view(C, -1))
    cam_aux = ops.linear(aux, P.w["aux_classifier.weight"].view(C, -1))
    res, g0 = [], 0
    for o in outs:
        r = o[0].shape[0]
        res.append((cam_aux[g0:g0 + r], cam[g0:g0 + r]))
        g0 += r
    return res, (tf[:rows], aux[:rows], _prefix_saved(enc, b, rows))


def network_forward(P: StudentParams, x: Tensor, save: bool, enc_cache=None):
    cfg = P.cfg
    if enc_cache is not None:
        tf, aux, enc = enc_cache
    else:
        tf, aux, enc = encoder_forward(P, x, save)
    B = x.shape[0]
    h, w = x.shape[2] // cfg.patch, x.shape[3] // cfg.patch
    n, D, C = h * w, cfg.embed_dim, P.num_classes - 1
    Wc = P.w["classifier.weight"].view(C, D)
    Wa = P.w["aux_classifier.weight"].view(C, D)
    pooled, pidx = ops.gmp_fwd(tf, B, n, D)
    pooled_a, paidx = ops.gmp_fwd(aux, B, n, D)
    cls_x4 = ops.linear(pooled, Wc)
    cls_aux = ops.linear(pooled_a, Wa)
    x4 = ops.tokens_to_nchw(tf, B, n, D, h, w, skip_cls=True)
    dd, dil = cfg.decoder_dim, cfg.decoder_dilation
    col6 = torch.empty((B * n, 9 * D), device=x.device, dtype=torch.float32)
    ops.L().dupl_im2col_dil3(tf.data_ptr() + 4 * D, col6.data_ptr(), B, h, w, D, dil, D, (n + 1) * D, ops._stream())
    f16 = GEMM_MODE == "f16x3"
    guard = None
    if f16:
        P.store.ensure_w16(P.student)
        guard = P.store.guard.sites(P.student)
    if f16 and guard["conv6"]:
        h6, _ = _lin16(P, ops.split16(col6), P.w16("decoder.conv6.weight", dd), relu=True)
    else:
        h6 = ops.linear(col6, P.w["decoder.conv6.weight"].view(dd, -1), relu=True)
    col7 = torch.empty((B * n, 9 * dd), device=x.device, dtype=torch.float32)
    ops.L().dupl_im2col_dil3(h6.data_ptr(), col7.data_ptr(), B, h, w, dd, dil, dd, n * dd, ops._stream())
    if f16 and guard["conv7"]:
        h7, _ = _lin16(P, ops.split16(col7), P.w16("decoder.conv7.weight", dd), relu=True)
    else:
        h7 = ops.linear(col7, P.w["decoder.conv7.weight"].view(dd, -1), relu=True)
    seg_tok = ops.linear(h7, P.w["decoder.conv8.weight"].view(P.num_classes, dd))
    seg = ops.tokens_to_nchw(seg_tok, B, n, P.num_classes, h, w, skip_cls=False)
    sv = None
    if save:
        sv = HeadSaved(enc=enc, tf=tf, aux=aux, pooled=pooled, pooled_idx=pidx, pooled_aux=pooled_a, pooled_aux_idx=paidx,
                       col6=col6, h6=h6, col7=col7, h7=h7, guard=guard)
    return (cls_x4, seg, x4, cls_aux), sv


def large_fov_forward(x: Tensor, W6: Tensor, W7: Tensor, W8: Tensor, dil: int, keep: Optional[list] = None) -> Tensor:
    B, C, h, w = x.shape
    n, dd, NC = h * w, W6.shape[0], W8.shape[0]
    tok = ops.zeros((B * n, C), x.device)
    ops.nchw_to_tokens_add(x, tok, B, n, C, skip_cls=False)
    col6 = torch.empty((B * n, 9 * C), device=x.device, dtype=torch.float32)
    ops.L().dupl_im2col_dil3(tok.data_ptr(), col6.data_ptr(), B, h, w, C, dil, C, n * C, ops._stream())
    h6 = ops.linear(col6, W6.reshape(dd, -1), relu=True)
    col7 = torch.empty((B * n, 9 * dd), device=x.device, dtype=torch.float32)
    ops.L().dupl_im2col_dil3(h6.data_ptr(), col7.data_ptr(), B, h, w, dd, dil, dd, n * dd, ops._stream())
    h7 = ops.linear(col7, W7.reshape(W7.shape[0], -1), relu=True)
    seg_tok = ops.linear(h7, W8.reshape(NC, -1))
    seg = ops.tokens_to_nchw(seg_tok, B, n, NC, h, w, skip_cls=False)
    if keep is not None:
        keep.extend((col6, h6, col7, h7))
    return seg


class LargeFOVFn(torch.autograd.Function):

    @staticmethod
    def forward(ctx, x, W6, W7, W8, dil):
        keep = []
        with torch.no_grad():
            seg = large_fov_forward(x.contiguous().float(), W6, W7, W8, dil, keep=keep)
        ctx.save_for_backward(W6, W7, W8, *keep)
        ctx.dil, ctx.xshape = dil, tuple(x.shape)
        return seg

    @staticmethod
    def backward(ctx, dseg):
        W6, W7, W8, col6, h6, col7, h7 = ctx.saved_tensors
        B, C, h, w = ctx.xshape
        n, dd, NC, dil = h * w, W6.shape[0], W8.shape[0], ctx.dil
        dev = dseg.device
        dseg_tok = ops.zeros((B * n, NC), dev)
        ops.nchw_to_tokens_add(dseg.contiguous().float(), dseg_tok, B, n, NC, skip_cls=False)
        need = ctx.needs_input_grad
        dW8 = dW7 = dW6 = dx = None
        if need[3]:
            dW8 = torch.empty_like(W8)
            ops.linear_wgrad(dseg_tok, h7, dW8)
        dh7 = ops.linear_dgrad(dseg_tok, W8.reshape(NC, dd), relumask_of=h7)
        if need[2]:
            dW7 = torch.empty_like(W7)
            ops.linear_wgrad(dh7, col7, dW7)
        dcol7 = ops.linear_dgrad(dh7, W7.reshape(dd, -1))
        dh6 = torch.empty((B * n, dd), device=dev, dtype=torch.float32)
        ops.L().dupl_col2im_dil3(dcol7.data_ptr(), dh6.data_ptr(), B, h, w, dd, dil, dd, n * dd, 0, h6.data_ptr(), ops._stream())
        del dcol7
        if need[1]:
            dW6 = torch.empty_like(W6)
            ops.linear_wgrad(dh6, col6, dW6)
        if need[0]:
            dcol6 = ops.linear_dgrad(dh6, W6.reshape(dd, -1))
            dtok = torch.empty((B * n, C), device=dev, dtype=torch.float32)
            ops.L().dupl_col2im_dil3(dcol6.data_ptr(), dtok.data_ptr(), B, h, w, C, dil, C, n * C, 0, None, ops._stream())
            dx = ops.tokens_to_nchw(dtok, B, n, C, h, w, skip_cls=False)
        return dx, dW6, dW7, dW8, None


def _linear_backward32(P: StudentParams, dy: Tensor, x: Tensor, name: str, dgelu_of: Optional[Tensor] = None,
                       has_bias: bool = True) -> Tensor:
    N = dy.shape[1]
    ops.linear_wgrad(dy, x, P.g[name + ".weight"], accumulate=True)
    if has_bias:
        ops.colsum(dy, P.g[name + ".bias"], accumulate=True)
    return ops.linear_dgrad(dy, P.w[name + ".weight"].view(N, -1), dgelu_of=dgelu_of)


def _linear_backward16_km(P: StudentParams, dy: Tensor, x16, name: str, dgelu_of: Optional[Tensor] = None,
                          dx_feeds_split: bool = False, wgrads: Optional[list] = None) -> Tensor:
    M, N = dy.shape
    Kp = max(96, (M + 31) // 32 * 32)
    fuse_bias = not ops.deterministic()
    dy16, _, alpha = ops.split_prepare(dy, scaled=True, want_rm=True, want_T=False, fmt1=True, rm_rows=Kp,
                                       colsum_into=P.g[name + ".bias"] if fuse_bias else None)
    gw = P.g[name + ".weight"]
    if wgrads is not None:
        wgrads.append((dy16, x16, gw.view(N, -1), alpha))
    else:
        _lin16(P, dy16, x16, out=gw.view(N, -1), accumulate=True, alpha=alpha, a_kmajor=True, b_kmajor=True, k_pad=Kp)
    if not fuse_bias:
        ops.colsum(dy, P.g[name + ".bias"], accumulate=True)
    W16 = P.w16(name + ".weight", N, True)
    if SK_DGRAD and dgelu_of is None and not dx_feeds_split and not ops.deterministic() and W16.cols <= SK_DGRAD_MAX_COLS:
        dx = ops.zero_workspace(M, W16.cols, dy.device) if ZERO_WS else ops.zeros((M, W16.cols), dy.device)
        _lin16(P, dy16.rows_slice(0, M), W16, out=dx, accumulate=True, alpha=alpha, b_kmajor=True)
        return dx
    dx, _ = _lin16(P, dy16.rows_slice(0, M), W16, alpha=alpha, dgelu_of=dgelu_of, amax_for_next=dx_feeds_split, b_kmajor=True)
    return dx


def _linear_backward16(P: StudentParams, dy: Tensor, x: Tensor, name: str, dgelu_of: Optional[Tensor] = None,
                       has_bias: bool = True, dx_feeds_split: bool = False, xT16=None) -> Tensor:
    M, N = dy.shape
    Mp = (M + 31) // 32 * 32
    fuse_bias = has_bias and not ops.deterministic()
    dy16, dyT16, alpha = ops.split_prepare(dy, scaled=True, want_rm=True, want_T=True, rows_pad=Mp,
                                           colsum_into=P.g[name + ".bias"] if fuse_bias else None)
    if xT16 is None:
        _, xT16, _ = ops.split_prepare(x, scaled=False, want_rm=False, want_T=True, rows_pad=Mp)
    gw = P.g[name + ".weight"]
    _lin16(P, dyT16, xT16, out=gw.view(N, -1), accumulate=True, alpha=alpha)
    if has_bias and not fuse_bias:
        ops.colsum(dy, P.g[name + ".bias"], accumulate=True)
    dx, _ = _lin16(P, dy16, P.w16T(name + ".weight", N), alpha=alpha, dgelu_of=dgelu_of, amax_for_next=dx_feeds_split)
    return dx


BLOCK_OPERANDS_MULTI = os.environ.get("DUPL_BLOCK_OPERANDS_MULTI", "1") != "0"


def _block_operands16(P: StudentParams, p: str, s: "BlockSaved", g: dict, D: int, Hd: int) -> dict:
    sites = [("fc2", s.h1, "mlp.fc2", D, s.h1_16), ("fc1", s.ln2, "mlp.fc1", Hd, s.ln2_16), ("proj", s.att, "attn.proj", D, s.att16),
             ("qkv", s.ln1, "attn.qkv", 3 * D, s.ln1_16)]
    sites = [t[:4] for t in sites if g[t[0]] and t[4] is None]
    if not sites:
        return {}
    items = []
    for _, x, _, _ in sites:
        items.append((x, False, True, (x.shape[0] + 31) // 32 * 32))
    stale = P.store.w16T_missing(P.student, [(p + nm + ".weight", N) for _, _, nm, N in sites])
    for _, rows, w in stale:
        items.append((w, False, True, rows))
    out = ops.split_prepare_multi(items)
    for (key, _, _), (_, T) in zip(stale, out[len(sites):]):
        P.store.w16T_put(P.student, key, T)
    return {site: T for (site, _, _, _), (_, T) in zip(sites, out)}


def network_backward(P: StudentParams, sv: HeadSaved, dcls: Optional[Tensor], dseg: Optional[Tensor],
                     dx4: Optional[Tensor], dcls_aux: Optional[Tensor], on_ready=None):
    cfg = P.cfg
    enc = sv.enc
    B, h, w = enc.B, enc.h, enc.w
    n, D, C, NC = h * w, cfg.embed_dim, P.num_classes - 1, P.num_classes
    N = n + 1
    dev = sv.tf.device
    G, W = P.g, P.w
    dtf = ops.zeros((B * N, D), dev)
    dta = None
    aux_is_final = sv.aux.data_ptr() == sv.tf.data_ptr()
    if dx4 is not None:
        ops.nchw_to_tokens_add(dx4.contiguous(), dtf, B, n, D, skip_cls=True)
    if dcls is not None:
        dcls = dcls.contiguous()
        ops.linear_wgrad(dcls, sv.pooled, G["classifier.weight"], accumulate=True)
        dpool = ops.linear_dgrad(dcls, W["classifier.weight"].view(C, D))
        ops.gmp_bwd(dpool, sv.pooled_idx, dtf, B, n, D)
        P.mark_grad(SEG_CLS)
    if dcls_aux is not None:
        dcls_aux = dcls_aux.contiguous()
        ops.linear_wgrad(dcls_aux, sv.pooled_aux, G["aux_classifier.weight"], accumulate=True)
        dpool = ops.linear_dgrad(dcls_aux, W["aux_classifier.weight"].view(C, D))
        if aux_is_final:
            ops.gmp_bwd(dpool, sv.pooled_aux_idx, dtf, B, n, D)
        else:
            dta = ops.zeros((B * N, D), dev)
            ops.gmp_bwd(dpool, sv.pooled_aux_idx, dta, B, n, D)
        P.mark_grad(SEG_CLS)
    if dseg is not None:
        dd, dil = cfg.decoder_dim, cfg.decoder_dilation
        dseg_tok = ops.zeros((B * n, NC), dev)
        ops.nchw_to_tokens_add(dseg.contiguous(), dseg_tok, B, n, NC, skip_cls=False)
        ops.linear_wgrad(dseg_tok, sv.h7, G["decoder.conv8.weight"], accumulate=True)
        dh7 = ops.linear_dgrad(dseg_tok, W["decoder.conv8.weight"].view(NC, dd), relumask_of=sv.h7)
        f16 = GEMM_MODE == "f16x3"
        guard = (sv.guard or P.store.guard.sites(P.student)) if f16 else None
        conv_bwd = _linear_backward16 if (f16 and guard["conv7"]) else _linear_backward32
        dcol7 = conv_bwd(P, dh7, sv.col7, "decoder.conv7", has_bias=False)
        dh6 = torch.empty((B * n, dd), device=dev, dtype=torch.float32)
        ops.L().dupl_col2im_dil3(dcol7.data_ptr(), dh6.data_ptr(), B, h, w, dd, dil, dd, n * dd, 0, sv.h6.data_ptr(), ops._stream())
        del dcol7
        conv_bwd = _linear_backward16 if (f16 and guard["conv6"]) else _linear_backward32
        dcol6 = conv_bwd(P, dh6, sv.col6, "decoder.conv6", has_bias=False)
        ops.L().dupl_col2im_dil3(dcol6.data_ptr(), dtf.data_ptr() + 4 * D, B, h, w, D, dil, D, N * D, 1, None, ops._stream())
        del dcol6
        P.mark_grad(SEG_DECODER)
    if on_ready is not None:
        on_ready("heads")
    encoder_backward(P, enc, dtf, dta, on_ready=on_ready)


def encoder_backward(P: StudentParams, enc: "EncoderSaved", dtf: Tensor, dta: Optional[Tensor], on_ready=None):
    cfg = P.cfg
    B, h, w = enc.B, enc.h, enc.w
    n, D = h * w, cfg.embed_dim
    N = n + 1
    G, W = P.g, P.w
    f16 = GEMM_MODE == "f16x3"
    gb = (enc.guard or P.store.guard.sites(P.student))["blocks"] if f16 else None
    dx = ops.layernorm_bwd(dtf, enc.x_last, W["encoder.norm.weight"], enc.mean_f, enc.rstd_f,
                           G["encoder.norm.weight"], G["encoder.norm.bias"], amax_for_next=f16 and gb[cfg.depth - 1]["fc2"])
    aux_idx = cfg.aux_layer % cfg.depth
    Hh, hd = cfg.num_heads, cfg.head_dim
    scale = hd ** -0.5
    for i in reversed(range(cfg.depth)):
        p = f"encoder.blocks.{i}."
        s = enc.blocks[i]
        if dta is not None and i == aux_idx:
            ops.axpy_(dx, dta, 1.0)
            dx._dupl_amax = None
        g = gb[i] if f16 else None

        def lin_bwd(site):
            return _linear_backward16 if (f16 and g[site]) else _linear_backward32

        wg = [] if WGRAD_GROUP else None

        def lin(site, dy_, x_, x16_, nm, **kw):
            if f16 and g[site] and x16_ is not None:
                return _linear_backward16_km(P, dy_, x16_, nm, dgelu_of=kw.get("dgelu_of"), dx_feeds_split=kw.get("dx_feeds_split", False),
                                             wgrads=wg)
            return lin_bwd(site)(P, dy_, x_, nm, **kw)

        def feeds(site):
            return {"dx_feeds_split": bool(g[site])} if f16 else {}
        att16 = f16 and s.qkv16 is not None and N <= 2048
        xT = _block_operands16(P, p, s, g, D, D * cfg.mlp_ratio) if (f16 and BLOCK_OPERANDS_MULTI) else {}

        def pre(site):
            return {"xT16": xT[site]} if site in xT else {}
        dpre1 = lin("fc2", dx, s.h1, s.h1_16, p + "mlp.fc2", dgelu_of=s.pre1, **(feeds("fc1") if g and g["fc2"] else {}), **pre("fc2"))
        dln2 = lin("fc1", dpre1, s.ln2, s.ln2_16, p + "mlp.fc1", **pre("fc1"))
        del dpre1
        dx_mid = ops.layernorm_bwd(dln2, s.x_mid, W[p + "norm2.weight"], s.mean2, s.rstd2,
                                   G[p + "norm2.weight"], G[p + "norm2.bias"], dres=dx, amax_for_next=f16 and g["proj"])
        datt = lin("proj", dx_mid, s.att, s.att16, p + "attn.proj",
                   **({"dx_feeds_split": bool(att16)} if g and g["proj"] else {}), **pre("proj"))
        if att16:
            dqkv = ops.attention_bwd16(s.qkv16, s.att, datt, s.lse, B, N, Hh, hd, scale, amax_for_next=bool(g["qkv"]))
        else:
            dqkv = ops.attention_bwd(s.qkv, s.att, datt, s.lse, B, N, Hh, hd, scale)
        dln1 = lin("qkv", dqkv, s.ln1, s.ln1_16, p + "attn.qkv", **pre("qkv"))
        del dqkv, datt, xT
        dx = ops.layernorm_bwd(dln1, s.x_in, W[p + "norm1.weight"], s.mean1, s.rstd1,
                               G[p + "norm1.weight"], G[p + "norm1.bias"], dres=dx_mid,
                               amax_for_next=f16 and i > 0 and gb[i - 1]["fc2"])
        if wg:
            ops.wgrad16_group(wg, tuning=P.store.gemm16_tuning)
        del wg
        enc.blocks[i] = None
        if on_ready is not None:
            on_ready(i)
    dpatch = ops.assemble_tokens_bwd(dx, G["encoder.cls_token"], B, n, D)
    rows = ops.patch_im2row(enc.x_img, cfg.patch)
    ops.linear_wgrad(dpatch, rows, G["encoder.patch_embed.proj.weight"], accumulate=True)
    ops.colsum(dpatch, G["encoder.patch_embed.proj.bias"], accumulate=True)
    P.mark_grad(SEG_BACKBONE)
    P.mark_grad(SEG_NORM)
    if on_ready is not None:
        on_ready("stem")
```

### dupl_amd/ops.py

```python
from __future__ import annotations

import ctypes
import os
from typing import Optional, Sequence

import numpy as np
import torch

from . import _lib
from ._lib import GemmDesc

Tensor = torch.Tensor


def L():
    return _lib.lib()


_DETERMINISTIC = [os.environ.get("DUPL_DETERMINISTIC", "0") == "1"]


def deterministic() -> bool:
    return _DETERMINISTIC[0]


def set_deterministic(on) -> None:
    _DETERMINISTIC[0] = bool(on)


def _stream() -> int:
    return torch.cuda.current_stream().cuda_stream


def _p(t: Optional[Tensor]) -> Optional[int]:
    return None if t is None else t.data_ptr()


def _chk(t: Tensor, dtype=torch.float32):
    assert t.is_cuda, "dupl_amd ops need device tensors (no CPU fallback)"
    assert t.dtype == dtype, f"expected {dtype}, got {t.dtype}"
    assert t.is_contiguous(), "expected a contiguous tensor"
    return t


GEMM32_TUNING = {"tile_rows": 0, "tile_cols": 0, "group": 0}


def gemm_raw(A: int, B: int, C: int, M: int, N: int, K: int, lda: int, ldb: int, ldc: int, *, flags: int = 0,
             bias: Optional[int] = None, res: Optional[int] = None, ldr: int = 0, aux: Optional[int] = None,
             ldaux: int = 0, alpha: float = 1.0, batch: int = 1, zdiv: int = 1,
             sA=(0, 0), sB=(0, 0), sC=(0, 0), sR=(0, 0), sX=(0, 0), sBias=(0, 0)):
    d = GemmDesc()
    d.A, d.B, d.C = A, B, C
    d.bias, d.res, d.aux = bias, res, aux
    d.M, d.N, d.K = M, N, K
    d.lda, d.ldb, d.ldc, d.ldr, d.ldaux = lda, ldb, ldc, ldr, ldaux
    d.batch, d.zdiv = batch, zdiv
    d.sA0, d.sA1 = sA
    d.sB0, d.sB1 = sB
    d.sC0, d.sC1 = sC
    d.sR0, d.sR1 = sR
    d.sX0, d.sX1 = sX
    d.sBias0, d.sBias1 = sBias
    d.alpha, d.flags = alpha, flags
    d.deterministic = int(deterministic())
    d.tile_rows, d.tile_cols, d.group = GEMM32_TUNING["tile_rows"], GEMM32_TUNING["tile_cols"], GEMM32_TUNING["group"]
    L().dupl_gemm_f32(ctypes.byref(d), _stream())


class Split16:
    __slots__ = ("planes", "rows", "cols", "exp", "fmt", "valid_rows")

    def __init__(self, planes: Tensor, exp: int = 0, fmt: Optional[int] = None, valid_rows: Optional[int] = None):
        assert planes.dtype == torch.float16 and planes.dim() == 3 and planes.shape[0] == 2 and planes.is_contiguous()
        self.planes, self.rows, self.cols, self.exp = planes, planes.shape[1], planes.shape[2], int(exp)
        self.fmt = int(fmt) if fmt is not None else int(exp > 0)
        self.valid_rows = int(valid_rows) if valid_rows is not None else self.rows

    @property
    def hi(self) -> int:
        return self.planes.data_ptr()

    @property
    def lo(self) -> int:
        return self.planes.data_ptr() + 2 * self.rows * self.cols

    def rows_slice(self, r0: int, r1: int) -> "Split16View":
        return Split16View(self, r0, r1)


class Split16View:
    __slots__ = ("hi", "lo", "rows", "cols", "base", "exp", "fmt")

    def __init__(self, base: Split16, r0: int, r1: int):
        self.base = base
        self.exp = base.exp
        self.fmt = base.fmt
        self.hi = base.hi + 2 * r0 * base.cols
        self.lo = base.lo + 2 * r0 * base.cols
        self.rows, self.cols = r1 - r0, base.cols


class W16:
    __slots__ = ("hi", "lo", "rows", "cols", "exp", "fmt")

    def __init__(self, hi: int, lo: int, rows: int, cols: int, exp: int = 0):
        self.hi, self.lo, self.rows, self.cols, self.exp = hi, lo, rows, cols, int(exp)
        self.fmt = int(exp > 0)


import os as _os
GEMM16_TUNING = {"tile": int(_os.environ.get("DUPL_GEMM16_TILE", "0")), "concurrency": 1,
                 "persist_blocks": int(_os.environ.get("DUPL_PERSIST_BLOCKS", "0")), "group": 0,
                 "sk_slices": int(_os.environ.get("DUPL_SK_SLICES", "0"))}


EXP_ACT, EXP_W = 3, 9


def split16_empty(rows: int, cols: int, device, exp: int = 0) -> Split16:
    return Split16(torch.empty((2, rows, cols), device=device, dtype=torch.float16), exp)


def split16(x: Tensor, out: Optional[Split16] = None, exp: int = 0) -> Split16:
    _chk(x)
    rows, cols = x.shape[0], x.numel() // x.shape[0]
    out = out if out is not None else split16_empty(rows, cols, x.device, exp)
    assert out.exp == exp
    if exp:
        L().dupl_split_f16x2b(x.data_ptr(), out.hi, out.lo, x.numel(), exp, _stream())
    else:
        L().dupl_split_f16x2(x.data_ptr(), out.hi, out.lo, x.numel(), _stream())
    return out


_SCALE_RINGS = {}
_RING = 128


def _scale_ring(device):
    key = (device.index, torch.cuda.current_stream(device).cuda_stream)
    ring = _SCALE_RINGS.get(key)
    if ring is None:
        ring = [torch.zeros((_RING, 4), device=device, dtype=torch.float32), 0, None, 0]
        _SCALE_RINGS[key] = ring
    return ring


def _scale_slot(device):
    ring = _scale_ring(device)
    buf, i = ring[0], ring[1]
    ring[1] = (i + 1) % _RING
    ring[3] += 1
    base = buf.data_ptr()
    return base + 16 * i, base + 16 * ((i + 1) % _RING) + 8, buf[i]


class _Alpha(int):

    def bind(self, ring, stream):
        self.ring, self.stream, self.gen = ring, stream, ring[3]
        return self

    def check(self):
        cur = torch.cuda.current_stream().cuda_stream
        assert cur == self.stream, "a scaled operand's alpha is only valid on the stream that prepared it"
        assert self.ring[3] - self.gen < _RING - 1, "scale slot reused: the alpha of a scaled split_prepare expires after ~128 later ones"


class _AmaxToken:
    __slots__ = ("word",)


def reserve_amax(device):
    ring = _scale_ring(device)
    if ring[2] is not None:
        return None, None
    tok = _AmaxToken()
    tok.word = ring[0].data_ptr() + 16 * ring[1] + 8
    ring[2] = tok
    return tok.word, tok


def split_prepare(x: Tensor, scaled: bool, want_rm: bool, want_T: bool, rows_pad: int = 0, target_exp: int = 15,
                  colsum_into: Optional[Tensor] = None, fmt1: bool = False, rm_rows: int = 0):
    _chk(x)
    R, C = x.shape
    Rp = rows_pad if rows_pad else (R + 31) // 32 * 32
    rm = None
    if want_rm:
        rm = Split16(torch.empty((2, max(R, rm_rows), C), device=x.device, dtype=torch.float16), 0, fmt=int(fmt1), valid_rows=R)
    T = Split16(torch.empty((2, C, Rp), device=x.device, dtype=torch.float16), 0, fmt=int(fmt1)) if want_T else None
    slot = nxt = rec = None
    amax_mode = 0
    if scaled:
        ring = _scale_ring(x.device)
        pending, ring[2] = ring[2], None
        if pending is not None:
            amax_mode = 1 if getattr(x, "_dupl_amax", None) is pending else 2
        slot, nxt, rec = _scale_slot(x.device)
        assert pending is None or pending.word == slot + 8
    d = _lib.SplitDesc()
    d.x, d.ld, d.R, d.C = x.data_ptr(), x.stride(0), R, C
    d.slot, d.next_bits = slot, nxt
    d.hi, d.lo = (rm.hi, rm.lo) if rm else (None, None)
    d.hiT, d.loT = (T.hi, T.lo) if T else (None, None)
    d.Rp, d.target_exp, d.colsum_accum, d.amax_mode = Rp, target_exp, _p(colsum_into), amax_mode
    d.fmt, d.rows_zero_to = int(fmt1), (rm_rows if (rm is not None and rm_rows > R) else 0)
    d.deterministic = int(deterministic())
    L().dupl_split_prepare(ctypes.byref(d), _stream())
    if scaled:
        for o in (rm, T):
            if o is not None:
                o.planes._dupl_scale = rec
        return rm, T, _Alpha(slot + 4).bind(ring, torch.cuda.current_stream(x.device).cuda_stream)
    return rm, T, None


def split_prepare_multi(items):
    out, descs = [], []
    for x, want_rm, want_T, rows_pad in items:
        _chk(x)
        R, C = x.shape
        Rp = rows_pad if rows_pad else (R + 31) // 32 * 32
        rm = split16_empty(R, C, x.device) if want_rm else None
        T = split16_empty(C, Rp, x.device) if want_T else None
        d = _lib.SplitItem()
        d.x, d.ld, d.R, d.C, d.Rp = x.data_ptr(), x.stride(0), R, C, Rp
        d.hi, d.lo = (rm.hi, rm.lo) if rm else (None, None)
        d.hiT, d.loT = (T.hi, T.lo) if T else (None, None)
        descs.append(d)
        out.append((rm, T))
    for i in range(0, len(descs), _lib.SPLIT_MULTI_MAX):
        chunk = descs[i:i + _lib.SPLIT_MULTI_MAX]
        arr = (_lib.SplitItem * len(chunk))(*chunk)
        L().dupl_split_prepare_multi(ctypes.cast(arr, ctypes.c_void_p), len(chunk), _stream())
    return out


def linear16(x, W: Split16, bias: Optional[Tensor] = None, *, gelu: bool = False, relu: bool = False,
             res: Optional[Tensor] = None, out: Optional[Tensor] = None, store_pre: Optional[Tensor] = None,
             want_f32: bool = True, out16: Optional[Split16] = None, want16: bool = False, device=None,
             alpha: Optional[int] = None, accumulate: bool = False, dgelu_of: Optional[Tensor] = None,
             relumask_of: Optional[Tensor] = None, c_rows: int = 0, amax_for_next: bool = False, out_exp: int = 0,
             a_kmajor: bool = False, b_kmajor: bool = False, k_pad: int = 0, post_exp: int = 0, tuning: Optional[dict] = None):
    M, Ka = (x.cols, x.rows) if a_kmajor else (x.rows, x.cols)
    N, Kb = (W.cols, W.rows) if b_kmajor else (W.rows, W.cols)
    if a_kmajor or b_kmajor:
        K = k_pad if k_pad else max(Ka, Kb)
        assert K % 32 == 0 and K >= 96 and (a_kmajor or Ka == K) and (b_kmajor or Kb == K), (Ka, Kb, K)
    else:
        K = Ka
        assert Kb == K and K % 32 == 0
    if dgelu_of is not None or relumask_of is not None:
        assert store_pre is None
        store_pre = dgelu_of if dgelu_of is not None else relumask_of
    dev = device if device is not None else (x.planes.device if isinstance(x, Split16) else x.base.planes.device)
    y = None
    if want_f32 or out is not None:
        y = out if out is not None else torch.empty((c_rows or M, N), device=dev, dtype=torch.float32)
    y16 = out16 if out16 is not None else (split16_empty(M, N, dev, out_exp) if want16 else None)
    d = _lib.Gemm16Desc()
    d.deterministic = int(deterministic())
    xe, we = getattr(x, "exp", 0), getattr(W, "exp", 0)
    xf, wf = getattr(x, "fmt", int(xe > 0)), getattr(W, "fmt", int(we > 0))
    assert xf == wf, f"operand planes in different formats (fmt {xf} / {wf}, exp {xe} / {we})"
    if xf:
        assert (a_kmajor or b_kmajor) or (not accumulate and not amax_for_next)
        assert not (accumulate and b_kmajor and not a_kmajor and deterministic()), "stream-K data gradients use fp32 atomics"
        d.fmt, d.post_scale = 1, 2.0 ** -(xe + we + post_exp)
    if a_kmajor or b_kmajor:
        assert xf == 1, "k-major operands need format 1 planes"
        d.a_layout, d.b_layout = int(a_kmajor), int(b_kmajor)
        d.ka_valid = min(Ka, K) if a_kmajor else 0
        d.kb_valid = min(Kb, K) if b_kmajor else 0
    if y16 is not None:
        assert y16.exp == 0 or xe, "format 1 output planes come from format 1 GEMMs"
        d.out_exp = y16.exp
    d.A_hi, d.A_lo, d.B_hi, d.B_lo = x.hi, x.lo, W.hi, W.lo
    d.C = _p(y)
    d.C_hi, d.C_lo = (y16.hi, y16.lo) if y16 is not None else (None, None)
    d.bias, d.res, d.aux = _p(bias), _p(res), _p(store_pre)
    d.M, d.N, d.K = M, N, K
    d.lda, d.ldb = x.cols, W.cols
    d.ldc = y.stride(0) if y is not None else 0
    d.ldo = N
    d.ldr = res.stride(0) if res is not None else 0
    d.ldaux = store_pre.stride(0) if store_pre is not None else 0
    aux_flag = _lib.GEMM_MUL_DGELU if dgelu_of is not None else (_lib.GEMM_MUL_RELUMASK if relumask_of is not None else
                                                                  (_lib.GEMM_STORE_PRE if store_pre is not None else 0))
    d.flags = (_lib.GEMM_GELU if gelu else 0) | (_lib.GEMM_RELU if relu else 0) | aux_flag | (_lib.GEMM_ACCUM if accumulate else 0)
    if isinstance(alpha, _Alpha):
        alpha.check()
    d.alpha_dev = int(alpha) if alpha is not None else None
    d.c_rows = int(c_rows)
    tn = tuning if tuning is not None else GEMM16_TUNING
    d.tile, d.concurrency = tn["tile"], tn["concurrency"]
    d.persist_blocks, d.group = tn["persist_blocks"], tn["group"]
    d.sk_slices = tn["sk_slices"]
    tok = None
    if amax_for_next and y is not None and not accumulate and not c_rows:
        d.amax_out, tok = reserve_amax(dev)
    if c_rows:
        assert y16 is not None and (y is None or y.shape[0] >= c_rows) and (store_pre is None or store_pre.shape[0] >= c_rows)
    L().dupl_gemm_f16x3(ctypes.byref(d), _stream())
    if tok is not None:
        y._dupl_amax = tok
    return y, y16


def wgrad16_group(items, tuning: Optional[dict] = None):
    descs = []
    for dy16, x16, out, alpha in items:
        assert dy16.fmt == 1 and getattr(x16, "fmt", 0) == 1, "grouped weight gradients read format 1 planes k-major"
        Kp = dy16.rows
        assert Kp % 32 == 0 and Kp >= 96 and out.is_contiguous() and out.shape == (dy16.cols, x16.cols)
        if isinstance(alpha, _Alpha):
            alpha.check()
        d = _lib.Gemm16Desc()
        d.deterministic = int(deterministic())
        d.A_hi, d.A_lo, d.B_hi, d.B_lo = dy16.hi, dy16.lo, x16.hi, x16.lo
        d.C = out.data_ptr()
        d.M, d.N, d.K = dy16.cols, x16.cols, Kp
        d.lda, d.ldb, d.ldc, d.ldo = dy16.cols, x16.cols, out.stride(0), x16.cols
        d.flags = _lib.GEMM_ACCUM
        d.alpha_dev = int(alpha) if alpha is not None else None
        d.fmt, d.post_scale = 1, 2.0 ** -(getattr(dy16, "exp", 0) + getattr(x16, "exp", 0))
        d.a_layout, d.b_layout = 1, 1
        d.ka_valid, d.kb_valid = Kp, min(x16.rows, Kp)
        d.group = (tuning if tuning is not None else GEMM16_TUNING)["group"]
        descs.append(d)
    for i in range(0, len(descs), _lib.GEMM16_GROUP_MAX):
        chunk = descs[i:i + _lib.GEMM16_GROUP_MAX]
        arr = (_lib.Gemm16Desc * len(chunk))(*chunk)
        L().dupl_gemm_f16x3_group(arr, len(chunk), _stream())


def linear(x: Tensor, W: Tensor, bias: Optional[Tensor] = None, *, gelu: bool = False, relu: bool = False,
           res: Optional[Tensor] = None, out: Optional[Tensor] = None, store_pre: Optional[Tensor] = None) -> Tensor:
    M, K = x.shape
    N = W.shape[0]
    assert W.numel() == N * K
    y = out if out is not None else torch.empty((M, N), device=x.device, dtype=torch.float32)
    fl = (_lib.GEMM_GELU if gelu else 0) | (_lib.GEMM_RELU if relu else 0)
    if store_pre is not None:
        fl |= _lib.GEMM_STORE_PRE
    gemm_raw(x.data_ptr(), W.data_ptr(), y.data_ptr(), M, N, K, x.stride(0), K, y.stride(0), flags=fl,
             bias=_p(bias), res=_p(res), ldr=(res.stride(0) if res is not None else 0),
             aux=_p(store_pre), ldaux=(store_pre.stride(0) if store_pre is not None else 0))
    return y


def linear_dgrad(dy: Tensor, W: Tensor, *, dgelu_of: Optional[Tensor] = None, relumask_of: Optional[Tensor] = None,
                 out: Optional[Tensor] = None, accumulate: bool = False) -> Tensor:
    M, N = dy.shape
    K = W.numel() // N
    dx = out if out is not None else torch.empty((M, K), device=dy.device, dtype=torch.float32)
    fl = _lib.GEMM_B_NCONTIG | (_lib.GEMM_ACCUM if accumulate else 0)
    aux = None
    if dgelu_of is not None:
        fl |= _lib.GEMM_MUL_DGELU
        aux = dgelu_of
    if relumask_of is not None:
        fl |= _lib.GEMM_MUL_RELUMASK
        aux = relumask_of
    gemm_raw(dy.data_ptr(), W.data_ptr(), dx.data_ptr(), M, K, N, dy.stride(0), K, dx.stride(0), flags=fl,
             aux=_p(aux), ldaux=(aux.stride(0) if aux is not None else 0))
    return dx


def linear_wgrad(dy: Tensor, x: Tensor, out: Tensor, accumulate: bool = False):
    M, N = dy.shape
    K = x.shape[1]
    assert out.numel() == N * K
    fl = _lib.GEMM_A_MCONTIG | _lib.GEMM_B_NCONTIG | (_lib.GEMM_ACCUM if accumulate else 0)
    gemm_raw(dy.data_ptr(), x.data_ptr(), out.data_ptr(), N, K, M, dy.stride(0), x.stride(0), K, flags=fl)


def colsum(x: Tensor, out: Tensor, accumulate: bool = False):
    M, N = x.shape
    L().dupl_colsum(x.data_ptr(), out.data_ptr(), M, N, x.stride(0), int(accumulate), int(deterministic()), _stream())


def layernorm_fwd(x: Tensor, gamma: Tensor, beta: Tensor, eps: float, save: bool = False):
    rows, D = x.shape
    y = torch.empty_like(x)
    mean = rstd = None
    if save:
        mean = torch.empty(rows, device=x.device, dtype=torch.float32)
        rstd = torch.empty(rows, device=x.device, dtype=torch.float32)
    L().dupl_layernorm_fwd(x.data_ptr(), gamma.data_ptr(), beta.data_ptr(), y.data_ptr(), _p(mean), _p(rstd), rows, D,
                           eps, _stream())
    return y, mean, rstd


def layernorm_fwd16(x: Tensor, gamma: Tensor, beta: Tensor, eps: float, save: bool = False, want_f32: bool = False,
                    f32_rows: int = 0, exp: int = 0):
    rows, D = x.shape
    keep = f32_rows or rows
    y = torch.empty((keep, D), device=x.device, dtype=torch.float32) if want_f32 else None
    y16 = split16_empty(rows, D, x.device, exp)
    mean = rstd = None
    if save:
        mean = torch.empty(keep, device=x.device, dtype=torch.float32)
        rstd = torch.empty(keep, device=x.device, dtype=torch.float32)
    L().dupl_layernorm_fwd16(x.data_ptr(), gamma.data_ptr(), beta.data_ptr(), _p(y), y16.hi, y16.lo, _p(mean), _p(rstd), rows, D,
                             eps, int(f32_rows), int(exp), _stream())
    return y, y16, mean, rstd


LNB_ROWS_PER_WAVE = 0


def layernorm_bwd(dy: Tensor, x: Tensor, gamma: Tensor, mean: Tensor, rstd: Tensor, dgamma: Tensor, dbeta: Tensor,
                  dres: Optional[Tensor] = None, amax_for_next: bool = False, two_stage: Optional[bool] = None) -> Tensor:
    rows, D = x.shape
    if two_stage is None:
        two_stage = deterministic()
    dx = torch.empty_like(x)
    word, tok = reserve_amax(x.device) if amax_for_next else (None, None)
    part, nb = None, 0
    if two_stage:
        nb = L().dupl_layernorm_bwd_blocks(rows, LNB_ROWS_PER_WAVE)
        part = torch.empty((nb, 2 * D), device=x.device, dtype=torch.float32)
    ws = getattr(dy, "_dupl_zero_ws", None)
    if ws is not None:
        assert ws.stream == _stream() and ws.dirty == dy.numel(), "a zero_workspace view is produced and consumed on its own stream"
    L().dupl_layernorm_bwd(dy.data_ptr(), x.data_ptr(), gamma.data_ptr(), mean.data_ptr(), rstd.data_ptr(), _p(dres),
                           dx.data_ptr(), dgamma.data_ptr(), dbeta.data_ptr(), rows, D, word, _p(part), nb, LNB_ROWS_PER_WAVE,
                           dy.data_ptr() if ws is not None else None, int(deterministic()), _stream())
    if ws is not None:
        ws.dirty = 0
    if tok is not None:
        dx._dupl_amax = tok
    return dx


_ZERO_WS = {}
_ZERO_WS_MAX = 8


class _ZeroWs:
    __slots__ = ("buf", "dirty", "stream")

    def __init__(self, n, device, stream):
        self.buf = torch.zeros(n, device=device, dtype=torch.float32)
        self.dirty = 0
        self.stream = stream


def zero_workspace(rows: int, cols: int, device) -> Tensor:
    stream = torch.cuda.current_stream(device).cuda_stream
    key = (device.index, stream)
    n = rows * cols
    ws = _ZERO_WS.pop(key, None)
    if ws is None or ws.buf.numel() < n:
        ws = _ZeroWs(n, device, stream)
    _ZERO_WS[key] = ws
    while len(_ZERO_WS) > _ZERO_WS_MAX:
        _ZERO_WS.pop(next(iter(_ZERO_WS)))
    if ws.dirty:
        fill_(ws.buf[:ws.dirty], 0.0)
    ws.dirty = n
    view = ws.buf[:n].view(rows, cols)
    view._dupl_zero_ws = ws
    return view


def attention_fwd(qkv: Tensor, B: int, N: int, H: int, hd: int, scale: float, need_lse: bool = False, out: Tensor = None):
    if out is None:
        out = torch.empty((B * N, H * hd), device=qkv.device, dtype=torch.float32)
    else:
        assert out.shape == (B * N, H * hd) and out.is_contiguous() and qkv.is_contiguous()
    lse = torch.empty((B, H, N), device=qkv.device, dtype=torch.float32) if need_lse else None
    L().dupl_attention_fwd(qkv.data_ptr(), out.data_ptr(), _p(lse), B, N, H, hd, scale, _stream())
    return out, lse


def attention_fwd16(qkv16, B: int, N: int, H: int, hd: int, scale: float, need_lse: bool = False,
                    out: Optional[Tensor] = None, out16=None, b_f32: int = 0):
    assert hd == 64 and qkv16.rows == B * N and qkv16.cols == 3 * H * hd and (out is not None or out16 is not None)
    dev = out.device if out is not None else (out16.planes.device if isinstance(out16, Split16) else out16.base.planes.device)
    bf = b_f32 or B
    lse = torch.empty((bf, H, N), device=dev, dtype=torch.float32) if need_lse else None
    if out is not None:
        assert out.shape == (bf * N, H * hd) and out.is_contiguous()
    assert getattr(qkv16, "exp", 0) == 0, "the split attention reads format 0 planes"
    L().dupl_attention_fwd16(qkv16.hi, qkv16.lo, _p(out), out16.hi if out16 is not None else None,
                              out16.lo if out16 is not None else None, _p(lse), B, N, H, hd, float(scale), bf,
                              out16.exp if out16 is not None else 0, _stream())
    return lse


def attention_fwd16_segs(qkv16, segs, H: int, hd: int, scale: float, out16=None):
    assert hd == 64 and 1 <= len(segs) <= _lib.ATTN_SEGS_MAX and getattr(qkv16, "exp", 0) == 0
    dev = qkv16.planes.device if isinstance(qkv16, Split16) else qkv16.base.planes.device
    arr = (_lib.AttnSeg * len(segs))()
    lses = []
    for i, (row0, B, N, out, need_lse, b_f32) in enumerate(segs):
        bf = b_f32 or B
        assert out is not None or out16 is not None
        if out is not None:
            assert out.shape == (bf * N, H * hd) and out.is_contiguous()
        lse = torch.empty((bf, H, N), device=dev, dtype=torch.float32) if need_lse else None
        lses.append(lse)
        arr[i].row0, arr[i].B, arr[i].N, arr[i].B_f32 = int(row0), int(B), int(N), int(b_f32)
        arr[i].out, arr[i].lse = _p(out), _p(lse)
    L().dupl_attention_fwd16_segs(qkv16.hi, qkv16.lo, out16.hi if out16 is not None else None,
                                   out16.lo if out16 is not None else None, ctypes.cast(arr, ctypes.c_void_p), len(segs), H, hd,
                                   float(scale), out16.exp if out16 is not None else 0, _stream())
    return lses


def attention_bwd16(qkv16, out: Tensor, dout: Tensor, lse: Tensor, B: int, N: int, H: int, hd: int, scale: float,
                    amax_for_next: bool = False) -> Tensor:
    assert hd == 64 and N <= 2048 and qkv16.rows == B * N
    dev = out.device
    dout = dout.contiguous()
    do16, _, alpha = split_prepare(dout, scaled=True, want_rm=True, want_T=False, target_exp=4)
    alpha.check()
    delta = torch.empty((B, H, N), device=dev, dtype=torch.float32)
    dqkv = torch.empty((B * N, 3 * H * hd), device=dev, dtype=torch.float32)
    word, tok = reserve_amax(dev) if amax_for_next else (None, None)
    L().dupl_attention_bwd16(qkv16.hi, qkv16.lo, out.data_ptr(), dout.data_ptr(), do16.hi, do16.lo, int(alpha) - 4, lse.data_ptr(),
                             delta.data_ptr(), dqkv.data_ptr(), B, N, H, hd, float(scale), word, _stream())
    if tok is not None:
        dqkv._dupl_amax = tok
    return dqkv


def attention_bwd(qkv: Tensor, out: Tensor, dout: Tensor, lse: Tensor, B: int, N: int, H: int, hd: int, scale: float) -> Tensor:
    dqkv = torch.empty_like(qkv)
    delta = torch.empty((B, H, N), device=qkv.device, dtype=torch.float32)
    L().dupl_attention_bwd(qkv.data_ptr(), out.data_ptr(), dout.data_ptr(), lse.data_ptr(), delta.data_ptr(),
                           dqkv.data_ptr(), B, N, H, hd, scale, _stream())
    return dqkv


def patch_im2row(x: Tensor, P: int) -> Tensor:
    B, C, H, W = x.shape
    assert C == 3
    rows = torch.empty((B * (H // P) * (W // P), 3 * P * P), device=x.device, dtype=torch.float32)
    L().dupl_patch_im2row(x.data_ptr(), rows.data_ptr(), B, H, W, P, _stream())
    return rows


def pos_embed_resize(pos_embed: Tensor, g: int, h: int, w: int) -> Tensor:
    D = pos_embed.shape[-1]
    out = torch.empty((1 + h * w, D), device=pos_embed.device, dtype=torch.float32)
    L().dupl_pos_embed_resize(pos_embed.data_ptr(), out.data_ptr(), g, h, w, D, _stream())
    return out


def assemble_tokens(patch: Tensor, cls: Tensor, pos: Tensor, B: int, n: int, D: int) -> Tensor:
    tok = torch.empty((B * (n + 1), D), device=patch.device, dtype=torch.float32)
    L().dupl_assemble_tokens(patch.data_ptr(), cls.data_ptr(), pos.data_ptr(), tok.data_ptr(), B, n, D, _stream())
    return tok


def assemble_tokens_bwd(dtok: Tensor, dcls: Tensor, B: int, n: int, D: int) -> Tensor:
    dpatch = torch.empty((B * n, D), device=dtok.device, dtype=torch.float32)
    L().dupl_assemble_tokens_bwd(dtok.data_ptr(), dpatch.data_ptr(), dcls.data_ptr(), B, n, D, _stream())
    return dpatch


def gmp_fwd(tokens: Tensor, B: int, n: int, D: int):
    out = torch.empty((B, D), device=tokens.device, dtype=torch.float32)
    idx = torch.empty((B, D), device=tokens.device, dtype=torch.int32)
    L().dupl_gmp_fwd(tokens.data_ptr(), out.data_ptr(), idx.data_ptr(), B, n, D, _stream())
    return out, idx


def gmp_bwd(dout: Tensor, idx: Tensor, dtokens: Tensor, B: int, n: int, D: int):
    L().dupl_gmp_bwd(dout.data_ptr(), idx.data_ptr(), dtokens.data_ptr(), B, n, D, _stream())


def tokens_to_nchw(tokens: Tensor, B: int, n: int, D: int, h: int, w: int, skip_cls: bool = True) -> Tensor:
    out = torch.empty((B, D, h, w), device=tokens.device, dtype=torch.float32)
    L().dupl_tokens_to_nchw(tokens.data_ptr(), out.data_ptr(), B, n, D, int(skip_cls), _stream())
    return out


def nchw_to_tokens_add(dnchw: Tensor, dtokens: Tensor, B: int, n: int, D: int, skip_cls: bool = True):
    L().dupl_nchw_to_tokens_add(dnchw.data_ptr(), dtokens.data_ptr(), B, n, D, int(skip_cls), _stream())


def resize_bilinear(x: Tensor, Ho: int, Wo: int, flip_cat: bool = False, align_corners: bool = False) -> Tensor:
    B, C, Hi, Wi = x.shape
    x = _chk(x.contiguous())
    out = torch.empty(((2 * B) if flip_cat else B, C, Ho, Wo), device=x.device, dtype=torch.float32)
    L().dupl_resize_bilinear(x.data_ptr(), out.data_ptr(), B, C, Hi, Wi, Ho, Wo, int(flip_cat), int(align_corners), _stream())
    return out


def cam_fuse(lows: Sequence[Tensor], sizes: Sequence[tuple], B: int, C: int, H: int, W: int, row_off: int, ldc: int,
             impl: int = 0, band_blocks: int = 0):
    n = len(lows)
    ptrs = (ctypes.c_void_p * n)(*[t.data_ptr() for t in lows])
    hs = (ctypes.c_int32 * n)(*[s[0] for s in sizes])
    ws = (ctypes.c_int32 * n)(*[s[1] for s in sizes])
    cam = torch.empty((B, C, H, W), device=lows[0].device, dtype=torch.float32)
    mm = torch.empty((B * C, 2), device=lows[0].device, dtype=torch.float32)
    L().dupl_cam_fuse(ctypes.cast(ptrs, ctypes.c_void_p), ctypes.cast(hs, ctypes.c_void_p), ctypes.cast(ws, ctypes.c_void_p),
                      n, row_off, ldc, cam.data_ptr(), mm.data_ptr(), B, C, H, W, int(impl), int(band_blocks), _stream())
    return cam, mm


def cam_normalise_(cam: Tensor, mm: Optional[Tensor] = None) -> Tensor:
    _chk(cam)
    planes = cam.shape[0] * cam.shape[1]
    HW = cam.shape[2] * cam.shape[3]
    have = mm is not None
    if mm is None:
        mm = torch.empty((planes, 2), device=cam.device, dtype=torch.float32)
    L().dupl_cam_minmax_normalise(cam.data_ptr(), mm.data_ptr(), planes, HW, int(have), _stream())
    return cam


def cam_to_label(cam: Tensor, cls_label: Tensor, img_box: Optional[Tensor], high_thre: Optional[Tensor], bkg_thre: float,
                 low_thre: float, ignore_mid: bool, ignore_index: int, want_valid: bool = False):
    b, C, h, w = cam.shape
    _chk(cam), _chk(cls_label)
    label = torch.empty((b, h, w), device=cam.device, dtype=torch.int64)
    valid = torch.empty_like(cam) if want_valid else None
    L().dupl_cam_to_label(cam.data_ptr(), cls_label.data_ptr(), _p(img_box), _p(high_thre), float(bkg_thre),
                          float(low_thre if low_thre is not None else 0.0), int(ignore_mid),
                          int(ignore_index if ignore_index is not None else 0), label.data_ptr(), _p(valid), b, C, h, w,
                          _stream())
    return valid, label


def denormalize_img(x: Tensor, mean=None, std=None) -> Tensor:
    B, C, H, W = x.shape
    assert C == 3
    x = _chk(x.contiguous())
    out = torch.empty_like(x)
    ms = None
    if mean is not None or std is not None:
        m = list(mean) if mean is not None else [123.675, 116.28, 103.53]
        sd = list(std) if std is not None else [58.395, 57.12, 57.375]
        assert len(m) == 3 and len(sd) == 3
        ms = (ctypes.c_float * 6)(*m, *sd)
    L().dupl_denormalize_img(x.data_ptr(), out.data_ptr(), B, H * W, ms, _stream())
    return out


def par_pos_term(dilations: Sequence[int], w1: float = 0.3, w2: float = 0.01) -> np.ndarray:
    ker = np.ones(8, dtype=np.float32)
    ker[[0, 2, 5, 7]] = np.float32(np.sqrt(2))
    pos = np.concatenate([ker * np.float32(d) for d in dilations]).astype(np.float32)
    std = np.float32(np.std(pos.astype(np.float64), ddof=1))
    a = -((pos / (std + np.float32(1e-8)) / np.float32(w1)) ** 2)
    e = np.exp(a - a.max())
    return (np.float32(w2) * (e / e.sum())).astype(np.float32)


def par_affinity(imgs: Tensor, dilations: Sequence[int], pos_term: Tensor) -> Tensor:
    B, C, h, w = imgs.shape
    assert C == 3
    nd = len(dilations)
    aff = torch.empty((B, 8 * nd, h, w), device=imgs.device, dtype=torch.float32)
    dil = (ctypes.c_int32 * nd)(*dilations)
    L().dupl_par_affinity(imgs.data_ptr(), aff.data_ptr(), ctypes.cast(dil, ctypes.c_void_p), nd, pos_term.data_ptr(), B, h, w,
                          _stream())
    return aff


def par_propagate(aff: Tensor, masks: Tensor, job_img: Tensor, job_K: Tensor, dilations: Sequence[int], num_iter: int) -> Tensor:
    njobs, Kmax, h, w = masks.shape
    nd = len(dilations)
    dil = (ctypes.c_int32 * nd)(*dilations)
    a, b = masks, torch.empty_like(masks)
    for _ in range(num_iter):
        L().dupl_par_propagate(aff.data_ptr(), a.data_ptr(), b.data_ptr(), job_img.data_ptr(), job_K.data_ptr(),
                               ctypes.cast(dil, ctypes.c_void_p), nd, njobs, Kmax, h, w, _stream())
        a, b = b, a
    return a


def refine_pre(cams: Tensor, thr_map: Optional[Tensor], thr: Optional[Tensor], job_img: Tensor, job_K: Tensor, keys: Tensor,
               down_scale: int = 2) -> Tensor:
    b, C, H, W = cams.shape
    _chk(cams)
    njobs, Kmax = keys.shape
    h, w = H // down_scale, W // down_scale
    masks = zeros((njobs, Kmax, h, w), cams.device)
    L().dupl_refine_pre(cams.data_ptr(), _p(thr_map), _p(thr), job_img.data_ptr(), job_K.data_ptr(), keys.data_ptr(), njobs, Kmax,
                        masks.data_ptr(), C, H, W, h, w, _stream())
    return masks


def refine_post(masks: Tensor, job_img: Tensor, job_K: Tensor, keys: Tensor, box: Tensor, ignore_index: float,
                out_size=None) -> Tensor:
    njobs, Kmax, h, w = masks.shape
    H, W = out_size if out_size is not None else (2 * h, 2 * w)
    label = torch.empty((njobs, H, W), device=masks.device, dtype=torch.float32)
    L().dupl_refine_post(masks.data_ptr(), job_img.data_ptr(), job_K.data_ptr(), keys.data_ptr(), njobs, Kmax, box.data_ptr(),
                         float(ignore_index), label.data_ptr(), h, w, H, W, _stream())
    return label


def refine_merge(lab_h: Tensor, lab_l: Tensor, ignore_index: float) -> Tensor:
    out = torch.empty_like(lab_h)
    L().dupl_refine_merge(lab_h.data_ptr(), lab_l.data_ptr(), out.data_ptr(), float(ignore_index), lab_h.numel(), _stream())
    return out


def to_device_async(host, dtype, device) -> Tensor:
    t = torch.as_tensor(np.asarray(host), dtype=dtype)
    if device.type != "cuda":
        return t.to(device)
    return t.pin_memory().to(device, non_blocking=True)


def fill_(t: Tensor, v: float):
    L().dupl_fill(t.data_ptr(), float(v), t.numel(), _stream())
    return t


def axpy_(y: Tensor, x: Tensor, a: float = 1.0):
    assert y.numel() == x.numel()
    L().dupl_axpy(y.data_ptr(), x.data_ptr(), float(a), y.numel(), _stream())
    return y


def scale_(y: Tensor, a: float):
    L().dupl_scale(y.data_ptr(), float(a), y.numel(), _stream())
    return y


LOSS_SUMS_FLOATS = 136


def zeros(shape, device) -> Tensor:
    t = torch.empty(shape, device=device, dtype=torch.float32)
    return fill_(t, 0.0)


def upsample_argmax(logits: Tensor, H: int, W: int) -> Tensor:
    B, C, h, w = logits.shape
    logits = _chk(logits.contiguous())
    out = torch.empty((B, H, W), device=logits.device, dtype=torch.int64)
    L().dupl_upsample_argmax(logits.data_ptr(), out.data_ptr(), B, C, h, w, int(H), int(W), _stream())
    return out


def msc_seg_accum_(acc: Tensor, segs: Tensor, mode: int) -> Tensor:
    two, C, h, w = segs.shape
    assert two == 2 and acc.shape[1] == C and acc.is_contiguous()
    segs = _chk(segs.contiguous())
    H, W = acc.shape[-2:]
    L().dupl_msc_seg_accum(segs.data_ptr(), acc.data_ptr(), C, h, w, H, W, int(mode), _stream())
    return acc


def argmax_channels(x: Tensor) -> Tensor:
    B, C = x.shape[:2]
    HW = x[0, 0].numel()
    x = _chk(x.contiguous())
    out = torch.empty((B,) + tuple(x.shape[2:]), device=x.device, dtype=torch.int64)
    L().dupl_argmax_channels(x.data_ptr(), out.data_ptr(), B, C, HW, _stream())
    return out


def confusion_accum(gt: Tensor, pred: Tensor, hist: Tensor) -> Tensor:
    assert gt.dtype == torch.int64 and pred.dtype == torch.int64 and hist.dtype == torch.int64
    assert gt.numel() == pred.numel() and gt.is_cuda and pred.is_cuda and hist.is_cuda and hist.is_contiguous()
    gt, pred = gt.contiguous(), pred.contiguous()
    L().dupl_confusion_accum(gt.data_ptr(), pred.data_ptr(), gt.numel(), hist.shape[0], hist.data_ptr(), _stream())
    return hist


def multilabel_f1_accum(logits: Tensor, label: Tensor, total: Tensor) -> Tensor:
    B, C = logits.shape
    logits, label = _chk(logits.contiguous()), _chk(label.contiguous().float())
    L().dupl_multilabel_f1_accum(logits.data_ptr(), label.data_ptr(), B, C, total.data_ptr(), _stream())
    return total
```

### include/dupl_hip.h

```cpp
#ifndef DUPL_HIP_H
#define DUPL_HIP_H

#include <stdint.h>

#ifdef __cplusplus
extern "C" {
#endif

typedef void* dupl_stream_t;

int dupl_abi_version(void);
int dupl_build_digest(char* out, int32_t cap);

#define DUPL_LOSS_SUMS_FLOATS 136
#define DUPL_GEMM_A_MCONTIG 1
#define DUPL_GEMM_B_NCONTIG 2
#define DUPL_GEMM_GELU 4
#define DUPL_GEMM_ACCUM 8
#define DUPL_GEMM_MUL_DGELU 16
#define DUPL_GEMM_RELU 32
#define DUPL_GEMM_MUL_RELUMASK 64
#define DUPL_GEMM_ABS 128
#define DUPL_GEMM_STORE_PRE 256
typedef struct dupl_gemm_desc {
    uint32_t struct_size;
    int32_t tile_rows;
    int32_t tile_cols;
    int32_t group;
    const float* A; const float* B; float* C;
    const float* bias;
    const float* res;
    const float* aux;
    int32_t M, N, K;
    int32_t lda, ldb, ldc, ldr, ldaux;
    int32_t batch;
    int32_t zdiv;
    int64_t sA0, sA1, sB0, sB1, sC0, sC1, sR0, sR1, sX0, sX1, sBias0, sBias1;
    float alpha;
    int32_t flags;
    int32_t deterministic;
    int32_t reserved0;
} dupl_gemm_desc;
int dupl_gemm_f32(const dupl_gemm_desc* d, dupl_stream_t stream);
typedef struct dupl_gemm16_desc {
    uint32_t struct_size;
    int32_t deterministic;
    const void* A_hi; const void* A_lo;
    const void* B_hi; const void* B_lo;
    float* C;
    void* C_hi; void* C_lo;
    const float* bias;
    const float* res;
    float* aux;
    int32_t M, N, K;
    int32_t lda, ldb, ldc, ldo, ldr, ldaux;
    int32_t flags;
    int32_t c_rows;
    const float* alpha_dev;
    int32_t fmt;
    int32_t out_exp;
    float post_scale;
    void* amax_out;
    int32_t a_layout, b_layout;
    int32_t ka_valid, kb_valid;
    int32_t tile;
    int32_t concurrency;
    int32_t persist_blocks;
    int32_t group;
    int32_t sk_slices;
    int32_t reserved1;
} dupl_gemm16_desc;
int dupl_gemm_f16x3(const dupl_gemm16_desc* d, dupl_stream_t stream);
#define DUPL_GEMM16_GROUP_MAX 8
int dupl_gemm_f16x3_group(const dupl_gemm16_desc* descs, int32_t n, dupl_stream_t stream);
int dupl_split_f16x2(const float* x, void* hi, void* lo, int64_t n, dupl_stream_t stream);
int dupl_split_f16x2b(const float* x, void* hi, void* lo, int64_t n, int32_t scale_exp, dupl_stream_t stream);
typedef struct dupl_split_desc {
    uint32_t struct_size;
    int32_t ld, R, C;
    const float* x;
    float* slot; void* next_bits;
    void* hi; void* lo; void* hiT; void* loT;
    int32_t Rp, target_exp;
    float* colsum_accum;
    int32_t amax_mode, fmt, rows_zero_to;
    int32_t deterministic;
} dupl_split_desc;
int dupl_split_prepare(const dupl_split_desc* d, dupl_stream_t stream);
#define DUPL_SPLIT_MULTI_MAX 16
typedef struct dupl_split_item {
    const float* x; void* hi; void* lo; void* hiT; void* loT;
    int32_t ld, R, C, Rp;
} dupl_split_item;
int dupl_split_prepare_multi(const dupl_split_item* items, int32_t n, dupl_stream_t stream);
typedef struct dupl_bound_desc {
    int64_t offset;
    int32_t rows, cols;
} dupl_bound_desc;
int dupl_param_bounds(const float* base, const dupl_bound_desc* table_dev, int32_t n, float* out, dupl_stream_t stream);

int dupl_layernorm_fwd(const float* x, const float* gamma, const float* beta, float* y,
                       float* mean, float* rstd, int64_t rows, int32_t D, float eps, dupl_stream_t s);
int dupl_layernorm_fwd16(const float* x, const float* gamma, const float* beta, float* y, void* y_hi, void* y_lo, float* mean,
                         float* rstd, int64_t rows, int32_t D, float eps, int64_t f32_rows, int32_t plane_exp, dupl_stream_t s);
int dupl_layernorm_bwd_blocks(int64_t rows, int32_t rows_per_wave);
int dupl_layernorm_bwd(const float* dy, const float* x, const float* gamma, const float* mean,
                       const float* rstd, const float* dres, float* dx, float* dgamma, float* dbeta,
                       int64_t rows, int32_t D, void* amax_out, float* partials, int64_t partial_rows, int32_t rows_per_wave,
                       float* dy_clear, int32_t deterministic, dupl_stream_t s);

int dupl_colsum(const float* x, float* out, int64_t M, int32_t N, int32_t ldx, int32_t accumulate,
                int32_t deterministic, dupl_stream_t s);

int dupl_attention_fwd(const float* qkv, float* out, float* lse, int32_t B, int32_t N, int32_t H,
                       int32_t hd, float scale, dupl_stream_t s);
int dupl_attention_fwd16(const void* qkv_hi, const void* qkv_lo, float* out, void* out_hi, void* out_lo, float* lse, int32_t B,
                         int32_t N, int32_t H, int32_t hd, float scale, int32_t B_f32, int32_t out_exp, dupl_stream_t s);
#define DUPL_ATTN_SEGS_MAX 4
typedef struct dupl_attn_seg {
    int64_t row0;
    int32_t B, N, B_f32, reserved0;
    float* out;
    float* lse;
} dupl_attn_seg;
int dupl_attention_fwd16_segs(const void* qkv_hi, const void* qkv_lo, void* out_hi, void* out_lo, const dupl_attn_seg* segs, int32_t n,
                              int32_t H, int32_t hd, float scale, int32_t out_exp, dupl_stream_t s);
int dupl_attention_bwd(const float* qkv, const float* out, const float* dout, const float* lse,
                       float* delta, float* dqkv, int32_t B, int32_t N, int32_t H, int32_t hd,
                       float scale, dupl_stream_t s);

int dupl_patch_im2row(const float* x, float* rows, int32_t B, int32_t H, int32_t W, int32_t P, dupl_stream_t s);
int dupl_pos_embed_resize(const float* pos_embed, float* out, int32_t g, int32_t h, int32_t w, int32_t D, dupl_stream_t s);
int dupl_assemble_tokens(const float* patch, const float* cls, const float* pos, float* tokens,
                         int32_t B, int32_t n, int32_t D, dupl_stream_t s);
int dupl_assemble_tokens_bwd(const float* dtok, float* dpatch, float* dcls, int32_t B, int32_t n, int32_t D, dupl_stream_t s);
int dupl_gmp_fwd(const float* tokens, float* out, int32_t* idx, int32_t B, int32_t n, int32_t D, dupl_stream_t s);
int dupl_gmp_bwd(const float* dout, const int32_t* idx, float* dtokens, int32_t B, int32_t n, int32_t D, dupl_stream_t s);
int dupl_tokens_to_nchw(const float* tokens, float* out, int32_t B, int32_t n, int32_t D, int32_t skip_cls, dupl_stream_t s);
int dupl_nchw_to_tokens_add(const float* dnchw, float* dtokens, int32_t B, int32_t n, int32_t D, int32_t skip_cls, dupl_stream_t s);

int dupl_resize_bilinear(const float* in, float* out, int32_t B, int32_t C, int32_t Hi, int32_t Wi,
                         int32_t Ho, int32_t Wo, int32_t flip_cat, int32_t align_corners, dupl_stream_t s);
int dupl_cam_fuse(const float* const* lows, const int32_t* hs, const int32_t* ws, int32_t nscale, int32_t row_off,
                  int32_t ldc, float* cam, float* mm, int32_t B, int32_t C, int32_t H, int32_t W, int32_t impl,
                  int32_t band_blocks, dupl_stream_t s);
int dupl_cam_minmax_normalise(float* cam, float* mm, int32_t planes, int32_t HW, int32_t have_minmax, dupl_stream_t s);
int dupl_cam_to_label(const float* cam, const float* cls_label, const int32_t* img_box, const float* high_thre,
                      float bkg_thre, float low_thre, int32_t ignore_mid, int32_t ignore_index,
                      int64_t* label, float* valid_cam, int32_t b, int32_t C, int32_t h, int32_t w, dupl_stream_t s);
int dupl_denormalize_img(const float* x, float* out, int32_t B, int32_t HW, const float* mean_std, dupl_stream_t s);

int dupl_par_affinity(const float* imgs, float* aff, const int32_t* dilations, int32_t ndil, const float* pos_term,
                      int32_t B, int32_t h, int32_t w, dupl_stream_t s);
int dupl_par_propagate(const float* aff, const float* in, float* out, const int32_t* job_img, const int32_t* job_K,
                       const int32_t* dilations, int32_t ndil, int32_t njobs, int32_t Kmax, int32_t h, int32_t w,
                       dupl_stream_t s);
int dupl_refine_pre(const float* cams, const float* thr_map, const float* thr, const int32_t* job_img,
                    const int32_t* job_K, const int32_t* keys, int32_t njobs, int32_t Kmax, float* masks, int32_t C,
                    int32_t H, int32_t W, int32_t h, int32_t w, dupl_stream_t s);
int dupl_refine_post(const float* masks, const int32_t* job_img, const int32_t* job_K, const int32_t* keys,
                     int32_t njobs, int32_t Kmax, const int32_t* box, float ignore_index, float* label, int32_t h,
                     int32_t w, int32_t H, int32_t W, dupl_stream_t s);
int dupl_refine_merge(const float* lab_h, const float* lab_l, float* out, float ignore_index, int64_t n, dupl_stream_t s);

int dupl_ptc_reduce(const float* cos, const int64_t* label, const int64_t* mask, int32_t ignore_index, float* sums,
                    int32_t b, int32_t hw, int32_t finish, dupl_stream_t s);
int dupl_ptc_bwd_mask(float* cos_signed, const int64_t* label, const int64_t* mask, int32_t ignore_index,
                      const float* sums, const float* gscale, int32_t b, int32_t hw, dupl_stream_t s);
int dupl_l2norm_rows_fwd(const float* x, float* xhat, float* norm, int64_t rows, int32_t c, int64_t ldx,
                         int32_t rows_per_img, int64_t img_stride, float eps, dupl_stream_t s);
int dupl_l2norm_rows_bwd(const float* dxhat, const float* xhat, const float* norm, float* dx, int64_t rows, int32_t c,
                         int64_t ldx, int32_t rows_per_img, int64_t img_stride, float eps, int32_t accumulate,
                         dupl_stream_t s);
int dupl_seg_loss_fwd(const float* logits, const void* label, int32_t is_i64, int32_t ignore_index, float* sums,
                      int32_t b, int32_t C1, int32_t h, int32_t w, int32_t H, int32_t W, int32_t flip, int32_t finish,
                      dupl_stream_t s);
int dupl_seg_ce_map(const float* logits, const void* label, int32_t is_i64, int32_t ignore_index, float* ce_map,
                    int32_t b, int32_t C1, int32_t h, int32_t w, int32_t H, int32_t W, int32_t flip, dupl_stream_t s);
int dupl_seg_pseudo_label(const float* logits, const float* other_label, int32_t ignore_index, float conf_thr,
                          int64_t* out_label, float* count, int32_t b, int32_t C1, int32_t h, int32_t w, int32_t H,
                          int32_t W, dupl_stream_t s);
#define DUPL_GMM_STATS 16
int dupl_gmm_noise_filter(const float* ce_map, float* label, float* xs_scratch, uint8_t* lab_scratch, float* stats,
                          int32_t B, int32_t HW, int32_t ignore_index, float min_ce, int32_t min_count,
                          float valid_thre, float gamma, float reg_covar, float em_tol, int32_t em_iters, double u0,
                          double u1, double u2, int32_t seeding, const uint32_t* mt_raw_host, dupl_stream_t s);
int dupl_mask_fill(float* label, const uint8_t* mask, float value, int64_t n, dupl_stream_t s);
int dupl_seg_loss_bwd(const float* logits, const void* label, int32_t is_i64, int32_t ignore_index, const float* sums,
                      const float* gscale, float* dlogits, int32_t b, int32_t C1, int32_t h, int32_t w, int32_t H, int32_t W,
                      int32_t flip, int32_t balanced, int32_t deterministic, dupl_stream_t s);
int dupl_cos_sim_fwd(const float* a, const float* b, float* out, float* stats, int32_t B, int32_t n, int32_t c,
                     int64_t ld, int64_t img_stride, float eps, dupl_stream_t s);
int dupl_cos_sim_bwd(const float* a, const float* b, const float* stats, const float* g, float gmul, float* db, int32_t B,
                     int32_t n, int32_t c, int64_t ld, int64_t img_stride, float eps, int32_t accumulate, dupl_stream_t s);
#define DUPL_LOSS_TERMS_MAX 16
int dupl_loss_total(const float* const* terms, const float* add, const int32_t* group, int32_t n_terms, const float* weight,
                    int32_t n_groups, float* total, float* gsums, const float* g, float* gterm, dupl_stream_t s);
int dupl_mean_accum(const float* x, float* loss, int64_t n, float mul, dupl_stream_t s);
int dupl_multilabel_soft_margin(const float* logits, const float* target, float* loss, float* dlogits, const float* gscale,
                                int32_t b, int32_t C, dupl_stream_t s);

int dupl_im2col_dil3(const float* x, float* col, int32_t B, int32_t h, int32_t w, int32_t Cin, int32_t dil, int64_t ld,
                     int64_t img_stride, dupl_stream_t s);
int dupl_col2im_dil3(const float* dcol, float* dx, int32_t B, int32_t h, int32_t w, int32_t Cin, int32_t dil, int64_t ld,
                     int64_t img_stride, int32_t accumulate, const float* relu_of, dupl_stream_t s);

int dupl_adamw(float* p, float* g, float* m, float* v, int64_t n, float lr, float beta1, float beta2,
               float eps, float wd, float bc1, float bc2_sqrt, void* p_hi, void* p_lo, int32_t plane_exp, float grad_scale,
               dupl_stream_t s);
int dupl_fill(float* p, float v, int64_t n, dupl_stream_t s);
int dupl_axpy(float* y, const float* x, float a, int64_t n, dupl_stream_t s);
int dupl_scale(float* y, float a, int64_t n, dupl_stream_t s);

int dupl_upsample_argmax(const float* logits, int64_t* out, int32_t B, int32_t C, int32_t h, int32_t w, int32_t H, int32_t W,
                         dupl_stream_t s);
int dupl_msc_seg_accum(const float* segs, float* acc, int32_t C, int32_t h, int32_t w, int32_t H, int32_t W, int32_t mode,
                       dupl_stream_t s);
int dupl_argmax_channels(const float* x, int64_t* out, int32_t B, int32_t C, int64_t HW, dupl_stream_t s);
int dupl_confusion_accum(const int64_t* gt, const int64_t* pred, int64_t n, int32_t num_classes, int64_t* hist,
                         dupl_stream_t s);
int dupl_multilabel_f1_accum(const float* logits, const float* label, int32_t B, int32_t C, float* sum, dupl_stream_t s);

int dupl_attention_bwd16(const void* qkv_hi, const void* qkv_lo, const float* out, const float* dout, const void* do_hi,
                         const void* do_lo, const float* do_slot, const float* lse, float* delta, float* dqkv, int32_t B, int32_t N,
                         int32_t H, int32_t hd, float scale, void* amax_out, dupl_stream_t stream);

int dupl_aug_to_u8(const float* x, uint8_t* out, int64_t n, dupl_stream_t s);
int dupl_aug_lut_op(uint8_t* img, int32_t H, int32_t W, int32_t mode, uint32_t* hist_scratch, uint8_t* lut_scratch,
                    dupl_stream_t s);
int dupl_aug_posterize(uint8_t* img, int64_t n, int32_t bits, dupl_stream_t s);
int dupl_aug_enhance(uint8_t* img, int32_t H, int32_t W, int32_t mode, float factor, uint64_t* sum_scratch, dupl_stream_t s);
int dupl_aug_sharpness(const uint8_t* in, uint8_t* out, int32_t H, int32_t W, float factor, dupl_stream_t s);
int dupl_aug_finish(const uint8_t* img, float* out, int32_t H, int32_t W, dupl_stream_t s);

int dupl_loader_resample_h(const uint8_t* in, uint8_t* out, const int32_t* coef, const int32_t* bounds, int32_t ksize,
                           int32_t h, int32_t w, int32_t w2, dupl_stream_t s);
int dupl_loader_resample_v_crop(const uint8_t* tmp, uint8_t* out, const int32_t* coef, const int32_t* bounds, int32_t ksize,
                                int32_t w2, int32_t h2, int32_t flip, int32_t h_pad, int32_t w_pad, int32_t h_start,
                                int32_t w_start, int32_t crop, dupl_stream_t s);
int dupl_loader_normalize(const uint8_t* in, float* out, int32_t H, int32_t W, int32_t mode, dupl_stream_t s);

int dupl_photo_enhance(uint8_t* img, int32_t H, int32_t W, int32_t mode, float factor, uint64_t* sum_scratch,
                       dupl_stream_t s);
int dupl_photo_hue(uint8_t* img, int64_t n_px, int32_t shift, dupl_stream_t s);
int dupl_photo_grayscale(uint8_t* img, int64_t n_px, dupl_stream_t s);
int dupl_photo_gaussian_blur(uint8_t* img, uint8_t* tmp, int32_t H, int32_t W, float radius, dupl_stream_t s);

#ifdef __cplusplus
}
#endif
#endif
```

Measured before the change: 78.65.

## Add scaled-plane (format 1) attention path with single accumulator and tunable wave shape

Adds a format-1 attention forward and backward entry that reads QKV hi/lo planes pre-scaled by a power-of-two exponent. The lo plane then holds an unscaled residual, so the three split products can share one accumulator instead of separate main and cross accumulators. Fewer accumulator registers and simpler softmax/epilogue arithmetic are meant to cut VGPR pressure and ALU work. It also templates the kernel on waves per block and key-tile size, with the extra waves skipping DMA issue. Python picks the exponent per block from amax bounds and enables the path by default; the risk is lower accuracy when the lo residual falls into the fp16 subnormal range.

```diff
diff --git a/dupl_amd/csrc/attn_split.hip b/dupl_amd/csrc/attn_split.hip
--- a/dupl_amd/csrc/attn_split.hip
+++ b/dupl_amd/csrc/attn_split.hip
@@ -22,9 +22,7 @@
     }
 }
 constexpr float LO_INV = 1.f / DUPL_LO_SCALE;
-constexpr int HD = 64, KT = 64;
-constexpr int PLANE = KT * 128;
-constexpr int STAGE = 4 * PLANE;
+constexpr int HD = 64;
 
 #define MFMA16(a, b, c) __builtin_amdgcn_mfma_f32_32x32x16_f16((a), (b), (c), 0, 0, 0)
 
@@ -51,9 +49,16 @@
     float* lse[DUPL_ATTN_SEGS_MAX];
 };
 
-__global__ __launch_bounds__(256, 2) void attn_fwd16_kernel(const __half* __restrict__ qkv_hi, const __half* __restrict__ qkv_lo,
+constexpr int P_EXP = 7;
+template <bool SINGLE, int NW, int KT>
+__global__ __launch_bounds__(64 * NW, (NW == 6 || KT == 32) ? 3 : 2) void attn_fwd16_kernel(const __half* __restrict__ qkv_hi, const __half* __restrict__ qkv_lo,
                                                             __half* __restrict__ out_hi, __half* __restrict__ out_lo,
-                                                            const AttnSegs segs, int H, float scale, int remap, float out_scale) {
+                                                            const AttnSegs segs, int H, float scale, int remap, float out_scale,
+                                                            float qkv_inv) {
+    static_assert(KT == 64 || (KT == 32 && SINGLE), "32-key tiles exist for the single-accumulator arm only");
+    constexpr int PLANE = KT * 128;
+    constexpr int STAGE = 4 * PLANE;
+    constexpr int NS = KT / 32;
     __shared__ __attribute__((aligned(1024))) char smem[2 * STAGE];
     const int tid = threadIdx.x, lane = tid & 63, l31 = lane & 31, hf = lane >> 5;
     const int wave = __builtin_amdgcn_readfirstlane(tid >> 6);
@@ -66,7 +71,7 @@
     float* __restrict__ lse = segs.lse[sg];
     int bx, h, b;
     {
-        const int gx = (N + 127) / 128;
+        const int gx = (N + 32 * NW - 1) / (32 * NW);
         const int G = gx * H * segs.B[sg];
         const int L = (int)blockIdx.x - segs.first[sg];
         int w = L;
@@ -83,7 +88,7 @@
         qkv_lo += r0 * (size_t)(3 * H * HD);
         if (out_hi) { out_hi += r0 * (size_t)(H * HD); out_lo += r0 * (size_t)(H * HD); }
     }
-    const int q0 = bx * 128 + wave * 32;
+    const int q0 = bx * (32 * NW) + wave * 32;
     const int D = H * HD, ld = 3 * D;
     const int qrow = q0 + l31;
     const bool wave_active = q0 < N;
@@ -128,20 +133,23 @@
                                          (__attribute__((address_space(3))) void*)dst, 16, 0, 0);
     };
     auto issue = [&](int t, int buf) __attribute__((always_inline)) {
+        if (NW > 4 && wave >= 4) return;
         char* dst = smem + buf * STAGE + wave * 1024;
         const size_t o = t * tstride;
         if (t * KT + KT <= N) {
 #pragma unroll
-            for (int i = 0; i < 4; ++i) dma16(kbase[i >> 1] + o, koff[i & 1], dst + i * 4096);
-#pragma unroll
-            for (int i = 0; i < 4; ++i) dma16(vbase[i >> 1] + o, voff[i & 1], dst + (4 + i) * 4096);
+            for (int i = 0; i < 2 * NS; ++i) dma16(kbase[i / NS] + o, koff[i % NS], dst + (i / NS) * PLANE + (i % NS) * 4096);
+#pragma unroll
+            for (int i = 0; i < 2 * NS; ++i) dma16(vbase[i / NS] + o, voff[i % NS], dst + (2 + i / NS) * PLANE + (i % NS) * 4096);
         } else {
 #pragma unroll
-            for (int i = 0; i < 4; ++i)
-                dma16(kbase[i >> 1] + o, (unsigned)(min(t * KT + krow[i & 1], N - 1) - t * KT) * (unsigned)(ld * 2) + kch[i & 1], dst + i * 4096);
-#pragma unroll
-            for (int i = 0; i < 4; ++i)
-                dma16(vbase[i >> 1] + o, (unsigned)(min(t * KT + vrow[i & 1], N - 1) - t * KT) * (unsigned)(ld * 2) + vch, dst + (4 + i) * 4096);
+            for (int i = 0; i < 2 * NS; ++i)
+                dma16(kbase[i / NS] + o, (unsigned)(min(t * KT + krow[i % NS], N - 1) - t * KT) * (unsigned)(ld * 2) + kch[i % NS],
+                      dst + (i / NS) * PLANE + (i % NS) * 4096);
+#pragma unroll
+            for (int i = 0; i < 2 * NS; ++i)
+                dma16(vbase[i / NS] + o, (unsigned)(min(t * KT + vrow[i % NS], N - 1) - t * KT) * (unsigned)(ld * 2) + vch,
+                      dst + (2 + i / NS) * PLANE + (i % NS) * 4096);
         }
     };
 
@@ -152,11 +160,14 @@
     const unsigned v_lds = (unsigned)(uintptr_t)((__attribute__((address_space(3))) char*)smem) + 2 * PLANE +
                            ((vg >> 1) * 4 + (vq >> 2)) * 64 + (16 * (vg & 1) + 4 * (vq & 3)) * 2;
 
-    f32x16 oM[2], oX[2];
+    f32x16 oM[2], oX[SINGLE ? 1 : 2];
 #pragma unroll
     for (int d = 0; d < 2; ++d)
 #pragma unroll
-        for (int e = 0; e < 16; ++e) { oM[d][e] = 0.f; oX[d][e] = 0.f; }
+        for (int e = 0; e < 16; ++e) {
+            oM[d][e] = 0.f;
+            if constexpr (!SINGLE) oX[d][e] = 0.f;
+        }
     float m_run = -INFINITY, l_run = 0.f;
 
     const int nkt = (N + KT - 1) / KT;
@@ -177,13 +188,13 @@
         const char* st = smem + (t & 1) * STAGE;
         ATT_STAMP(0)
 
-        f32x16 sM[2], sX[2];
+        f32x16 sM[2], sX[SINGLE ? 1 : 2];
         const f32x16 zero16 = {0.f, 0.f, 0.f, 0.f, 0.f, 0.f, 0.f, 0.f, 0.f, 0.f, 0.f, 0.f, 0.f, 0.f, 0.f, 0.f};
-        h8 kh[2][2], kl[2][2];
-        auto k_read = [&](const int sstep, h8(&fh)[2], h8(&fl)[2]) __attribute__((always_inline)) {
+        h8 kh[2][NS], kl[2][NS];
+        auto k_read = [&](const int sstep, h8(&fh)[NS], h8(&fl)[NS]) __attribute__((always_inline)) {
             const int ch = ((2 * sstep + hf) ^ k_sw) * 16;
 #pragma unroll
-            for (int kt2 = 0; kt2 < 2; ++kt2) {
+            for (int kt2 = 0; kt2 < NS; ++kt2) {
                 fh[kt2] = *reinterpret_cast<const h8*>(st + kt2 * 4096 + k_off + ch);
                 fl[kt2] = *reinterpret_cast<const h8*>(st + PLANE + kt2 * 4096 + k_off + ch);
             }
@@ -195,16 +206,31 @@
             const int cur = sstep & 1;
             if (sstep + 1 < 4) k_read(sstep + 1, kh[cur ^ 1], kl[cur ^ 1]);
             __builtin_amdgcn_sched_barrier(0);
-            sM[0] = MFMA16(kh[cur][0], qh[sstep], sstep == 0 ? zero16 : sM[0]);
-            sM[1] = MFMA16(kh[cur][1], qh[sstep], sstep == 0 ? zero16 : sM[1]);
-            sX[0] = MFMA16(kh[cur][0], ql[sstep], sstep == 0 ? zero16 : sX[0]);
-            sX[1] = MFMA16(kh[cur][1], ql[sstep], sstep == 0 ? zero16 : sX[1]);
-            sX[0] = MFMA16(kl[cur][0], qh[sstep], sX[0]);
-            sX[1] = MFMA16(kl[cur][1], qh[sstep], sX[1]);
+            if constexpr (NS == 1) {
+                const int a = sstep & 1;
+                sM[a] = MFMA16(kh[cur][0], qh[sstep], sstep == 0 ? zero16 : sM[a]);
+                sM[a ^ 1] = MFMA16(kh[cur][0], ql[sstep], sstep == 0 ? zero16 : sM[a ^ 1]);
+                sM[a] = MFMA16(kl[cur][0], qh[sstep], sM[a]);
+            } else {
+                sM[0] = MFMA16(kh[cur][0], qh[sstep], sstep == 0 ? zero16 : sM[0]);
+                sM[1] = MFMA16(kh[cur][1], qh[sstep], sstep == 0 ? zero16 : sM[1]);
+                if constexpr (SINGLE) {
+                    sM[0] = MFMA16(kh[cur][0], ql[sstep], sM[0]);
+                    sM[1] = MFMA16(kh[cur][1], ql[sstep], sM[1]);
+                    sM[0] = MFMA16(kl[cur][0], qh[sstep], sM[0]);
+                    sM[1] = MFMA16(kl[cur][1], qh[sstep], sM[1]);
+                } else {
+                    sX[0] = MFMA16(kh[cur][0], ql[sstep], sstep == 0 ? zero16 : sX[0]);
+                    sX[1] = MFMA16(kh[cur][1], ql[sstep], sstep == 0 ? zero16 : sX[1]);
+                    sX[0] = MFMA16(kl[cur][0], qh[sstep], sX[0]);
+                    sX[1] = MFMA16(kl[cur][1], qh[sstep], sX[1]);
+                }
+            }
             __builtin_amdgcn_sched_barrier(0);
         }
+        if constexpr (NS == 1) sM[0] += sM[1];
         __builtin_amdgcn_s_setprio(0);
-        if (ATT_ABL & 16) { asm volatile("" ::"v"(sM[0]), "v"(sM[1]), "v"(sX[0]), "v"(sX[1])); }
+        if (ATT_ABL & 16) { asm volatile("" ::"v"(sM[0]), "v"(sM[1]), "v"(sX[0])); }
         ATT_STAMP(1)
         h4 vf[2][8];
         const unsigned v_st = v_lds + (t & 1) * STAGE;
@@ -221,18 +247,18 @@
             });
         };
         v_read(std::integral_constant<int, 0>{}, vf[0]);
-        const float c1 = scale * 1.4426950408889634f, c2 = c1 * LO_INV;
+        const float c1 = scale * 1.4426950408889634f * (SINGLE ? qkv_inv * qkv_inv : 1.f), c2 = c1 * LO_INV;
         if (t == nkt - 1) {
             const int kbase_t = t * KT + 8 * hf;
 #pragma unroll
-            for (int kt2 = 0; kt2 < 2; ++kt2)
+            for (int kt2 = 0; kt2 < NS; ++kt2)
 #pragma unroll
                 for (int e = 0; e < 16; ++e)
                     if (kbase_t + 32 * kt2 + 16 * (e >> 3) + (e & 7) >= N) sM[kt2][e] = -INFINITY;
         }
         float mx = -INFINITY;
 #pragma unroll
-        for (int kt2 = 0; kt2 < 2; ++kt2)
+        for (int kt2 = 0; kt2 < NS; ++kt2)
 #pragma unroll
             for (int e = 0; e < 16; ++e) mx = fmaxf(mx, sM[kt2][e]);
         {
@@ -246,23 +272,35 @@
         const float m_new = m_run2 == -INFINITY ? 0.f : m_run2;
         const float alpha = __builtin_amdgcn_exp2f(m_run - m_new);
         f32x2 psum2 = {0.f, 0.f};
-        h8 ph[4], pl[4];
+        h8 ph[2 * NS], pl[2 * NS];
         typedef _Float16 h2v __attribute__((ext_vector_type(2)));
 #pragma unroll
-        for (int kt2 = 0; kt2 < 2; ++kt2)
+        for (int kt2 = 0; kt2 < NS; ++kt2)
 #pragma unroll
             for (int e = 0; e < 16; e += 2) {
-                const f32x2 m2 = {sM[kt2][e], sM[kt2][e + 1]}, x2 = {sX[kt2][e], sX[kt2][e + 1]};
-                const f32x2 v2 = __builtin_elementwise_fma(x2, f32x2{c2, c2}, __builtin_elementwise_fma(m2, f32x2{c1, c1}, f32x2{-m_new, -m_new}));
-                const f32x2 p2 = {__builtin_amdgcn_exp2f(v2[0]), __builtin_amdgcn_exp2f(v2[1])};
-                psum2 += p2;
-                const h2v hh = __builtin_convertvector(p2, h2v);
-                const f32x2 q2 = p2 * f32x2{DUPL_LO_SCALE, DUPL_LO_SCALE};
+                const f32x2 m2 = {sM[kt2][e], sM[kt2][e + 1]};
                 const int idx = 2 * kt2 + (e >> 3);
-                ph[idx][e & 7] = hh[0];
-                ph[idx][(e & 7) + 1] = hh[1];
-                pl[idx][e & 7] = (_Float16)__builtin_fmaf((float)hh[0], -DUPL_LO_SCALE, q2[0]);
-                pl[idx][(e & 7) + 1] = (_Float16)__builtin_fmaf((float)hh[1], -DUPL_LO_SCALE, q2[1]);
+                if constexpr (SINGLE) {
+                    const f32x2 v2 = __builtin_elementwise_fma(m2, f32x2{c1, c1}, f32x2{(float)P_EXP - m_new, (float)P_EXP - m_new});
+                    const f32x2 p2 = {__builtin_amdgcn_exp2f(v2[0]), __builtin_amdgcn_exp2f(v2[1])};
+                    psum2 += p2;
+                    const h2v hh = __builtin_convertvector(p2, h2v);
+                    ph[idx][e & 7] = hh[0];
+                    ph[idx][(e & 7) + 1] = hh[1];
+                    pl[idx][e & 7] = (_Float16)(p2[0] - (float)hh[0]);
+                    pl[idx][(e & 7) + 1] = (_Float16)(p2[1] - (float)hh[1]);
+                } else {
+                    const f32x2 x2 = {sX[kt2][e], sX[kt2][e + 1]};
+                    const f32x2 v2 = __builtin_elementwise_fma(x2, f32x2{c2, c2}, __builtin_elementwise_fma(m2, f32x2{c1, c1}, f32x2{-m_new, -m_new}));
+                    const f32x2 p2 = {__builtin_amdgcn_exp2f(v2[0]), __builtin_amdgcn_exp2f(v2[1])};
+                    psum2 += p2;
+                    const h2v hh = __builtin_convertvector(p2, h2v);
+                    const f32x2 q2 = p2 * f32x2{DUPL_LO_SCALE, DUPL_LO_SCALE};
+                    ph[idx][e & 7] = hh[0];
+                    ph[idx][(e & 7) + 1] = hh[1];
+                    pl[idx][e & 7] = (_Float16)__builtin_fmaf((float)hh[0], -DUPL_LO_SCALE, q2[0]);
+                    pl[idx][(e & 7) + 1] = (_Float16)__builtin_fmaf((float)hh[1], -DUPL_LO_SCALE, q2[1]);
+                }
             }
         const float psum = psum2[0] + psum2[1];
         l_run = l_run * alpha + psum;
@@ -270,15 +308,18 @@
 #pragma unroll
             for (int d = 0; d < 2; ++d)
 #pragma unroll
-                for (int e = 0; e < 16; ++e) { oM[d][e] *= alpha; oX[d][e] *= alpha; }
+                for (int e = 0; e < 16; ++e) {
+                    oM[d][e] *= alpha;
+                    if constexpr (!SINGLE) oX[d][e] *= alpha;
+                }
         }
         m_run = m_run2;
-        if (ATT_ABL & 16) { asm volatile("" ::"v"(ph[0]), "v"(ph[3]), "v"(pl[0]), "v"(pl[3]), "v"(oM[0]), "v"(oX[1])); }
+        if (ATT_ABL & 16) { asm volatile("" ::"v"(ph[0]), "v"(ph[2 * NS - 1]), "v"(pl[0]), "v"(pl[2 * NS - 1]), "v"(oM[0]), "v"(oX[0])); }
         ATT_STAMP(2)
         __builtin_amdgcn_s_setprio(ATT_PRIO);
-        static_for<4>([&](auto sgc) __attribute__((always_inline)) {
+        static_for<2 * NS>([&](auto sgc) __attribute__((always_inline)) {
             constexpr int sg = decltype(sgc)::value, cur = sg & 1;
-            if constexpr (sg + 1 < 4) {
+            if constexpr (sg + 1 < 2 * NS) {
                 v_read(std::integral_constant<int, sg + 1>{}, vf[cur ^ 1]);
                 asm volatile("s_waitcnt lgkmcnt(8)" ::: "memory");
             } else {
@@ -290,14 +331,21 @@
             const h8 vl0 = __builtin_shufflevector(f[4], f[5], 0, 1, 2, 3, 4, 5, 6, 7), vl1 = __builtin_shufflevector(f[6], f[7], 0, 1, 2, 3, 4, 5, 6, 7);
             oM[0] = MFMA16(vh0, ph[sg], oM[0]);
             oM[1] = MFMA16(vh1, ph[sg], oM[1]);
-            oX[0] = MFMA16(vh0, pl[sg], oX[0]);
-            oX[1] = MFMA16(vh1, pl[sg], oX[1]);
-            oX[0] = MFMA16(vl0, ph[sg], oX[0]);
-            oX[1] = MFMA16(vl1, ph[sg], oX[1]);
+            if constexpr (SINGLE) {
+                oM[0] = MFMA16(vh0, pl[sg], oM[0]);
+                oM[1] = MFMA16(vh1, pl[sg], oM[1]);
+                oM[0] = MFMA16(vl0, ph[sg], oM[0]);
+                oM[1] = MFMA16(vl1, ph[sg], oM[1]);
+            } else {
+                oX[0] = MFMA16(vh0, pl[sg], oX[0]);
+                oX[1] = MFMA16(vh1, pl[sg], oX[1]);
+                oX[0] = MFMA16(vl0, ph[sg], oX[0]);
+                oX[1] = MFMA16(vl1, ph[sg], oX[1]);
+            }
             __builtin_amdgcn_sched_barrier(0);
         });
         __builtin_amdgcn_s_setprio(0);
-        if (ATT_ABL & 16) { asm volatile("" ::"v"(oM[0]), "v"(oM[1]), "v"(oX[0]), "v"(oX[1])); }
+        if (ATT_ABL & 16) { asm volatile("" ::"v"(oM[0]), "v"(oM[1]), "v"(oX[0])); }
         ATT_STAMP(3)
     }
     if ((ATT_ABL & 16) && lse && tid == 0) {
@@ -307,7 +355,7 @@
     }
     if (!wave_active) return;
     const float l_tot = l_run + __shfl_xor(l_run, 32, 64);
-    const float inv = 1.f / l_tot;
+    const float inv = SINGLE ? qkv_inv / l_tot : 1.f / l_tot;
     if (b >= B_f32) { out = nullptr; lse = nullptr; }
     if (qrow < N) {
         const size_t ro = ((size_t)b * N + qrow) * D + h * HD;
@@ -317,7 +365,7 @@
             for (int g = 0; g < 4; ++g) {
                 float v[4];
 #pragma unroll
-                for (int j = 0; j < 4; ++j) v[j] = (oM[d][4 * g + j] + oX[d][4 * g + j] * LO_INV) * inv;
+                for (int j = 0; j < 4; ++j) v[j] = SINGLE ? oM[d][4 * g + j] * inv : (oM[d][4 * g + j] + oX[d][4 * g + j] * LO_INV) * inv;
                 const int col = d * 32 + 8 * g + 4 * hf;
                 if (out) *reinterpret_cast<float4*>(out + ro + col) = make_float4(v[0], v[1], v[2], v[3]);
                 if (out_hi) {
@@ -331,7 +379,7 @@
                     *reinterpret_cast<uint2*>(out_lo + ro + col) = *reinterpret_cast<const uint2*>(ll);
                 }
             }
-        if (lse && hf == 0) lse[((size_t)b * H + h) * N + qrow] = m_run * 0.6931471805599453f + logf(l_tot);
+        if (lse && hf == 0) lse[((size_t)b * H + h) * N + qrow] = (m_run - (SINGLE ? (float)P_EXP : 0.f)) * 0.6931471805599453f + logf(l_tot);
     }
 }
 
@@ -339,13 +387,15 @@
 }
 
 constexpr int g_attn16_remap = 1;
+static int g_attn16_f1_waves = 4, g_attn16_f1_kt = 64;
 
 static int attn_fwd16_launch(const void* qkv_hi, const void* qkv_lo, void* out_hi, void* out_lo, const dupl_attn_seg* sv, int32_t n,
-                             int32_t H, int32_t hd, float scale, int32_t out_exp, dupl_stream_t s) {
-    if (out_exp < 0 || out_exp > 15 || !sv || n < 1 || n > DUPL_ATTN_SEGS_MAX) return DUPL_ERR_ARG;
+                             int32_t H, int32_t hd, float scale, int32_t out_exp, int32_t qkv_exp, dupl_stream_t s) {
+    if (out_exp < 0 || out_exp > 15 || qkv_exp < 0 || qkv_exp > 15 || !sv || n < 1 || n > DUPL_ATTN_SEGS_MAX) return DUPL_ERR_ARG;
     if (!qkv_hi || !qkv_lo || ((out_hi == nullptr) != (out_lo == nullptr)) || H <= 0 || hd != HD) return DUPL_ERR_ARG;
     auto al16 = [](const void* q) { return (reinterpret_cast<uintptr_t>(q) & 15) == 0; };
     if (!al16(qkv_hi) || !al16(qkv_lo)) return DUPL_ERR_ARG;
+    const int nw = qkv_exp ? g_attn16_f1_waves : 4;
     int order[DUPL_ATTN_SEGS_MAX];
     for (int i = 0; i < n; ++i) order[i] = i;
     for (int i = 1; i < n; ++i)
@@ -359,24 +409,50 @@
         if (q.B <= 0 || q.N <= 0 || q.row0 < 0 || bf < 0 || bf > q.B || (!q.out && !out_hi) || (bf < q.B && q.out && !out_hi)) return DUPL_ERR_ARG;
         g.row0[k] = (int)q.row0; g.B[k] = q.B; g.N[k] = q.N; g.B_f32[k] = bf; g.out[k] = q.out; g.lse[k] = q.lse;
         g.first[k] = total;
-        total += ((q.N + 127) / 128) * H * q.B;
+        total += ((q.N + 32 * nw - 1) / (32 * nw)) * H * q.B;
     }
     g.first[n] = total;
-    DUPL_LAUNCH(attn_fwd16_kernel, dim3((unsigned)total), dim3(256), 0, (hipStream_t)s, (const __half*)qkv_hi, (const __half*)qkv_lo,
-                       (__half*)out_hi, (__half*)out_lo, g, H, scale, g_attn16_remap, out_exp ? ldexpf(1.f, out_exp) : 0.f);
+    const float out_scale = out_exp ? ldexpf(1.f, out_exp) : 0.f, qkv_inv = ldexpf(1.f, -qkv_exp);
+#define ATTN16_GO(SINGLE, NW, KT)                                                                                                      \
+    DUPL_LAUNCH((attn_fwd16_kernel<SINGLE, NW, KT>), dim3((unsigned)total), dim3(64 * NW), 0, (hipStream_t)s, (const __half*)qkv_hi,  \
+                (const __half*)qkv_lo, (__half*)out_hi, (__half*)out_lo, g, H, scale, g_attn16_remap, out_scale, qkv_inv)
+    if (!qkv_exp) ATTN16_GO(false, 4, 64);
+    else if (nw == 6) ATTN16_GO(true, 6, 64);
+    else if (g_attn16_f1_kt == 32) ATTN16_GO(true, 4, 32);
+    else ATTN16_GO(true, 4, 64);
+#undef ATTN16_GO
     return dupl_launch_status();
+}
+
+extern "C" int dupl_attention_f1_set_shape(int32_t waves, int32_t key_tile) {
+    if (!((waves == 4 && (key_tile == 64 || key_tile == 32)) || (waves == 6 && key_tile == 64))) return DUPL_ERR_ARG;
+    g_attn16_f1_waves = waves;
+    g_attn16_f1_kt = key_tile;
+    return 0;
+}
+
+extern "C" int dupl_attention_fwd16_f1(const void* qkv_hi, const void* qkv_lo, float* out, void* out_hi, void* out_lo, float* lse,
+                                       int32_t B, int32_t N, int32_t H, int32_t hd, float scale, int32_t B_f32, int32_t out_exp,
+                                       int32_t qkv_exp, dupl_stream_t s) {
+    if (B_f32 < 0 || B_f32 > B || (B_f32 != 0 && B_f32 < B && !out_hi) || (!out && !out_hi)) return DUPL_ERR_ARG;
+    dupl_attn_seg q;
+    q.row0 = 0; q.B = B; q.N = N; q.B_f32 = B_f32; q.out = out; q.lse = lse;
+    return attn_fwd16_launch(qkv_hi, qkv_lo, out_hi, out_lo, &q, 1, H, hd, scale, out_exp, qkv_exp, s);
 }
 
 extern "C" int dupl_attention_fwd16(const void* qkv_hi, const void* qkv_lo, float* out, void* out_hi, void* out_lo, float* lse,
                                     int32_t B, int32_t N, int32_t H, int32_t hd, float scale, int32_t B_f32, int32_t out_exp,
                                     dupl_stream_t s) {
-    if (B_f32 < 0 || B_f32 > B || (B_f32 != 0 && B_f32 < B && !out_hi) || (!out && !out_hi)) return DUPL_ERR_ARG;
-    dupl_attn_seg q;
-    q.row0 = 0; q.B = B; q.N = N; q.B_f32 = B_f32; q.out = out; q.lse = lse;
-    return attn_fwd16_launch(qkv_hi, qkv_lo, out_hi, out_lo, &q, 1, H, hd, scale, out_exp, s);
+    return dupl_attention_fwd16_f1(qkv_hi, qkv_lo, out, out_hi, out_lo, lse, B, N, H, hd, scale, B_f32, out_exp, 0, s);
+}
+
+extern "C" int dupl_attention_fwd16_segs_f1(const void* qkv_hi, const void* qkv_lo, void* out_hi, void* out_lo, const dupl_attn_seg* segs,
+                                            int32_t n, int32_t H, int32_t hd, float scale, int32_t out_exp, int32_t qkv_exp,
+                                            dupl_stream_t s) {
+    return attn_fwd16_launch(qkv_hi, qkv_lo, out_hi, out_lo, segs, n, H, hd, scale, out_exp, qkv_exp, s);
 }
 
 extern "C" int dupl_attention_fwd16_segs(const void* qkv_hi, const void* qkv_lo, void* out_hi, void* out_lo, const dupl_attn_seg* segs,
                                          int32_t n, int32_t H, int32_t hd, float scale, int32_t out_exp, dupl_stream_t s) {
-    return attn_fwd16_launch(qkv_hi, qkv_lo, out_hi, out_lo, segs, n, H, hd, scale, out_exp, s);
-}
+    return attn_fwd16_launch(qkv_hi, qkv_lo, out_hi, out_lo, segs, n, H, hd, scale, out_exp, 0, s);
+}
diff --git a/dupl_amd/csrc/attn_split_bwd.hip b/dupl_amd/csrc/attn_split_bwd.hip
--- a/dupl_amd/csrc/attn_split_bwd.hip
+++ b/dupl_amd/csrc/attn_split_bwd.hip
@@ -111,12 +111,13 @@
     delta[((long)b * H + h) * N + n] = s;
 }
 
+template <bool F1>
 __device__ __forceinline__ void attn_bwd16_dq_body(char* __restrict__ smem, const int bx, const int h, const int b,
                                                    const __half* __restrict__ qkv_hi, const __half* __restrict__ qkv_lo,
                                                    const __half* __restrict__ do_hi, const __half* __restrict__ do_lo,
                                                    const float* __restrict__ lse, const float* __restrict__ delta,
                                                    const float* __restrict__ slot, float* __restrict__ dqkv, unsigned int* __restrict__ amax_out, int N, int H,
-                                                   float scale) {
+                                                   float scale, float qkv_inv) {
     constexpr int STAGE = 6 * PL;
     const int tid = threadIdx.x, lane = tid & 63, wave = tid >> 6, l31 = lane & 31, hf = lane >> 5;
     const int q0 = bx * 128 + wave * 32;
@@ -184,21 +185,32 @@
             const h8 kl = *reinterpret_cast<const h8*>(st + PL + a_off + ch);
             const h8 vh = *reinterpret_cast<const h8*>(st + 2 * PL + a_off + ch);
             const h8 vl = *reinterpret_cast<const h8*>(st + 3 * PL + a_off + ch);
-            sM = MFMA16(kh, qh[s], sM);
-            sX = MFMA16(kh, ql[s], sX);
-            sX = MFMA16(kl, qh[s], sX);
-            pM = MFMA16(vh, oh[s], pM);
-            pX = MFMA16(vh, ol[s], pX);
-            pX = MFMA16(vl, oh[s], pX);
-        }
+            if constexpr (F1) {
+                sM = MFMA16(kh, qh[s], sM);
+                pM = MFMA16(vh, oh[s], pM);
+                pX = MFMA16(vh, ol[s], pX);
+                sM = MFMA16(kh, ql[s], sM);
+                pM = MFMA16(vl, oh[s], pM);
+                sM = MFMA16(kl, qh[s], sM);
+            } else {
+                sM = MFMA16(kh, qh[s], sM);
+                sX = MFMA16(kh, ql[s], sX);
+                sX = MFMA16(kl, qh[s], sX);
+                pM = MFMA16(vh, oh[s], pM);
+                pX = MFMA16(vh, ol[s], pX);
+                pX = MFMA16(vl, oh[s], pX);
+            }
+        }
+        const float s_scale = F1 ? scale * qkv_inv * qkv_inv : scale;
         const int kb = t * TT + 8 * hf;
         f32x16 ds;
 #pragma unroll
         for (int e = 0; e < 16; ++e) {
             const bool kvld = kb + 16 * (e >> 3) + (e & 7) < N;
-            const float sv = (sM[e] + sX[e] * LO_INV) * scale;
+            const float sv = F1 ? sM[e] * s_scale : (sM[e] + sX[e] * LO_INV) * scale;
             const float p = kvld ? fast_exp(sv - my_lse) : 0.f;
-            ds[e] = __fmul_rn(p, __fsub_rn(pM[e] + pX[e] * LO_INV, my_delta));
+            const float dp = F1 ? (pM[e] + pX[e] * LO_INV) * qkv_inv : pM[e] + pX[e] * LO_INV;
+            ds[e] = __fmul_rn(p, __fsub_rn(dp, my_delta));
         }
         h4 kf[8][2];
         km_read_tile(km_lds + (t & 1) * STAGE, kf);
@@ -213,13 +225,14 @@
                 const h8 tl = h8of(kf[(sg * 2 + d) * 2 + 1][0], kf[(sg * 2 + d) * 2 + 1][1]);
                 dqM[d] = MFMA16(th, dh[sg], dqM[d]);
                 dqX[d] = MFMA16(th, dl[sg], dqX[d]);
-                dqX[d] = MFMA16(tl, dh[sg], dqX[d]);
+                if constexpr (F1) dqM[d] = MFMA16(tl, dh[sg], dqM[d]);
+                else dqX[d] = MFMA16(tl, dh[sg], dqX[d]);
             }
         }
     }
     float amx = 0.f;
     if (wave_active && qv) {
-        const float f = scale * inv_s;
+        const float f = scale * inv_s * (F1 ? qkv_inv : 1.f);
         float* op = dqkv + ((size_t)b * N + qrow) * ld + h * HD;
 #pragma unroll
         for (int d = 0; d < 2; ++d)
@@ -237,13 +250,13 @@
     attn_bwd_amax_flush(amax_out, amx);
 }
 
-template <int MODE>
+template <int MODE, bool F1>
 __device__ __forceinline__ void attn_bwd16_dkv_body(char* __restrict__ smem, const int bx, const int h, const int b,
                                                     const __half* __restrict__ qkv_hi, const __half* __restrict__ qkv_lo,
                                                     const __half* __restrict__ do_hi, const __half* __restrict__ do_lo,
                                                     const float* __restrict__ lse, const float* __restrict__ delta,
                                                     const float* __restrict__ slot, float* __restrict__ dqkv, unsigned int* __restrict__ amax_out, int N, int H,
-                                                    float scale) {
+                                                    float scale, float qkv_inv) {
     constexpr int NPL = MODE == 0 ? 4 : 6;
     constexpr int STAGE = NPL * PL;
     float* Ls = reinterpret_cast<float*>(smem + 2 * STAGE);
@@ -325,16 +338,32 @@
             const h8 ah = *reinterpret_cast<const h8*>(st + a_off + ch);
             const h8 al = *reinterpret_cast<const h8*>(st + PL + a_off + ch);
             sM = MFMA16(ah, kh[s], sM);
-            sX = MFMA16(ah, kl[s], sX);
-            sX = MFMA16(al, kh[s], sX);
-            if (MODE == 1) {
-                const h8 bh = *reinterpret_cast<const h8*>(st + 2 * PL + a_off + ch);
-                const h8 bl = *reinterpret_cast<const h8*>(st + 3 * PL + a_off + ch);
-                pM = MFMA16(bh, vh[s], pM);
-                pX = MFMA16(bh, vl[s], pX);
-                pX = MFMA16(bl, vh[s], pX);
-            }
-        }
+            if constexpr (F1) {
+                if (MODE == 1) {
+                    const h8 bh = *reinterpret_cast<const h8*>(st + 2 * PL + a_off + ch);
+                    const h8 bl = *reinterpret_cast<const h8*>(st + 3 * PL + a_off + ch);
+                    pM = MFMA16(bh, vh[s], pM);
+                    sM = MFMA16(ah, kl[s], sM);
+                    pX = MFMA16(bl, vh[s], pX);
+                    sM = MFMA16(al, kh[s], sM);
+                    pM = MFMA16(bh, vl[s], pM);
+                } else {
+                    sX = MFMA16(ah, kl[s], sX);
+                    sX = MFMA16(al, kh[s], sX);
+                }
+            } else {
+                sX = MFMA16(ah, kl[s], sX);
+                sX = MFMA16(al, kh[s], sX);
+                if (MODE == 1) {
+                    const h8 bh = *reinterpret_cast<const h8*>(st + 2 * PL + a_off + ch);
+                    const h8 bl = *reinterpret_cast<const h8*>(st + 3 * PL + a_off + ch);
+                    pM = MFMA16(bh, vh[s], pM);
+                    pX = MFMA16(bh, vl[s], pX);
+                    pX = MFMA16(bl, vh[s], pX);
+                }
+            }
+        }
+        const float s_scale = F1 ? scale * qkv_inv * qkv_inv : scale;
         const int qb = t * TT + 8 * hf;
         f32x16 w;
 #pragma unroll
@@ -342,9 +371,10 @@
             const int qi = qb + 16 * (e >> 3) + (e & 7);
             const bool ok = qi < N && kv;
             const int qc = min(qi, N - 1);
-            const float sv = (sM[e] + sX[e] * LO_INV) * scale;
+            const float sv = F1 ? (MODE == 1 ? sM[e] : sM[e] + sX[e]) * s_scale : (sM[e] + sX[e] * LO_INV) * scale;
             const float p = ok ? fast_exp(sv - Ls[qc]) : 0.f;
-            w[e] = MODE == 0 ? p : __fmul_rn(p, __fsub_rn(pM[e] + pX[e] * LO_INV, Ds[qc]));
+            const float dp = F1 ? (pM[e] + pX[e] * LO_INV) * qkv_inv : pM[e] + pX[e] * LO_INV;
+            w[e] = MODE == 0 ? p : __fmul_rn(p, __fsub_rn(dp, Ds[qc]));
         }
         h4 xf[8][2];
         km_read_tile(km_lds + (t & 1) * STAGE, xf);
@@ -359,13 +389,14 @@
                 const h8 tl = h8of(xf[(sg * 2 + d) * 2 + 1][0], xf[(sg * 2 + d) * 2 + 1][1]);
                 gM[d] = MFMA16(th, wh[sg], gM[d]);
                 gX[d] = MFMA16(th, wl[sg], gX[d]);
-                gX[d] = MFMA16(tl, wh[sg], gX[d]);
+                if constexpr (F1 && MODE == 1) gM[d] = MFMA16(tl, wh[sg], gM[d]);
+                else gX[d] = MFMA16(tl, wh[sg], gX[d]);
             }
         }
     }
     float amx = 0.f;
     if (wave_active && kv) {
-        const float f = MODE == 0 ? inv_s : scale * inv_s;
+        const float f = MODE == 0 ? inv_s : scale * inv_s * (F1 ? qkv_inv : 1.f);
         float* op = dqkv + ((size_t)b * N + krow) * ld + (MODE == 0 ? 2 * D : D) + h * HD;
 #pragma unroll
         for (int d = 0; d < 2; ++d)
@@ -384,12 +415,13 @@
 }
 
 constexpr int ATTNB_LDS = 2 * 6 * PL + 2 * MAXN * 4;
+template <bool F1>
 __global__ __launch_bounds__(256, 2) void attn_bwd16_all_kernel(const __half* __restrict__ qkv_hi, const __half* __restrict__ qkv_lo,
                                                                 const __half* __restrict__ do_hi, const __half* __restrict__ do_lo,
                                                                 const float* __restrict__ lse, const float* __restrict__ delta,
                                                                 const float* __restrict__ slot, float* __restrict__ dqkv,
                                                                 unsigned int* __restrict__ amax_out, int N, int H, int B, float scale,
-                                                                int remap) {
+                                                                int remap, float qkv_inv) {
     __shared__ __attribute__((aligned(1024))) char smem[ATTNB_LDS];
     const int gx = (N + 127) / 128;
     const int G = gx * H * B;
@@ -402,27 +434,40 @@
         w = (xcd < r ? xcd * (q + 1) : r * (q + 1) + (xcd - r) * q) + idx;
     }
     const int bx = w % gx, h = (w / gx) % H, b = w / (gx * H);
-    if (role == 0) attn_bwd16_dkv_body<1>(smem, bx, h, b, qkv_hi, qkv_lo, do_hi, do_lo, lse, delta, slot, dqkv, amax_out, N, H, scale);
-    else if (role == 1) attn_bwd16_dq_body(smem, bx, h, b, qkv_hi, qkv_lo, do_hi, do_lo, lse, delta, slot, dqkv, amax_out, N, H, scale);
-    else attn_bwd16_dkv_body<0>(smem, bx, h, b, qkv_hi, qkv_lo, do_hi, do_lo, lse, delta, slot, dqkv, amax_out, N, H, scale);
+    if (role == 0) attn_bwd16_dkv_body<1, F1>(smem, bx, h, b, qkv_hi, qkv_lo, do_hi, do_lo, lse, delta, slot, dqkv, amax_out, N, H, scale, qkv_inv);
+    else if (role == 1) attn_bwd16_dq_body<F1>(smem, bx, h, b, qkv_hi, qkv_lo, do_hi, do_lo, lse, delta, slot, dqkv, amax_out, N, H, scale, qkv_inv);
+    else attn_bwd16_dkv_body<0, F1>(smem, bx, h, b, qkv_hi, qkv_lo, do_hi, do_lo, lse, delta, slot, dqkv, amax_out, N, H, scale, qkv_inv);
 }
 
 }
 
 constexpr int g_attnb16_remap = 1;
 
-extern "C" int dupl_attention_bwd16(const void* qkv_hi, const void* qkv_lo, const float* out, const float* dout, const void* do_hi,
-                                    const void* do_lo, const float* do_slot, const float* lse, float* delta, float* dqkv, int32_t B,
-                                    int32_t N, int32_t H, int32_t hd, float scale, void* amax_out, dupl_stream_t stream) {
+extern "C" int dupl_attention_bwd16_f1(const void* qkv_hi, const void* qkv_lo, const float* out, const float* dout, const void* do_hi,
+                                       const void* do_lo, const float* do_slot, const float* lse, float* delta, float* dqkv, int32_t B,
+                                       int32_t N, int32_t H, int32_t hd, float scale, int32_t qkv_exp, void* amax_out,
+                                       dupl_stream_t stream) {
     unsigned int* ax = static_cast<unsigned int*>(amax_out);
     if (!qkv_hi || !qkv_lo || !out || !dout || !do_hi || !do_lo || !do_slot || !lse || !delta || !dqkv || B <= 0 || N <= 0 ||
-        N > MAXN || H <= 0 || hd != HD)
+        N > MAXN || H <= 0 || hd != HD || qkv_exp < 0 || qkv_exp > 15)
         return DUPL_ERR_ARG;
     hipStream_t s = (hipStream_t)stream;
     const long total = (long)B * N * H;
     DUPL_LAUNCH(delta_kernel, dim3((unsigned)((total + 255) / 256)), dim3(256), 0, s, out, dout, delta, B, N, H);
     const unsigned blocks = 3u * (unsigned)(((N + 127) / 128) * H * B);
-    DUPL_LAUNCH(attn_bwd16_all_kernel, dim3(blocks), dim3(256), 0, s, (const __half*)qkv_hi, (const __half*)qkv_lo,
-                       (const __half*)do_hi, (const __half*)do_lo, lse, delta, do_slot, dqkv, ax, N, H, B, scale, g_attnb16_remap);
+#define ATTNB16_GO(F1)                                                                                                                 \
+    DUPL_LAUNCH(attn_bwd16_all_kernel<F1>, dim3(blocks), dim3(256), 0, s, (const __half*)qkv_hi, (const __half*)qkv_lo,                \
+                (const __half*)do_hi, (const __half*)do_lo, lse, delta, do_slot, dqkv, ax, N, H, B, scale, g_attnb16_remap,            \
+                ldexpf(1.f, -qkv_exp))
+    if (qkv_exp) ATTNB16_GO(true);
+    else ATTNB16_GO(false);
+#undef ATTNB16_GO
     return dupl_launch_status();
 }
+
+extern "C" int dupl_attention_bwd16(const void* qkv_hi, const void* qkv_lo, const float* out, const float* dout, const void* do_hi,
+                                    const void* do_lo, const float* do_slot, const float* lse, float* delta, float* dqkv, int32_t B,
+                                    int32_t N, int32_t H, int32_t hd, float scale, void* amax_out, dupl_stream_t stream) {
+    return dupl_attention_bwd16_f1(qkv_hi, qkv_lo, out, dout, do_hi, do_lo, do_slot, lse, delta, dqkv, B, N, H, hd, scale, 0, amax_out,
+                                   stream);
+}
diff --git a/dupl_amd/engine.py b/dupl_amd/engine.py
--- a/dupl_amd/engine.py
+++ b/dupl_amd/engine.py
@@ -90,6 +90,15 @@
 
 FMT1 = os.environ.get("DUPL_FMT1", "1") != "0"
 KM_BWD = os.environ.get("DUPL_KM_BWD", "1") != "0"
+ATTN_F1 = os.environ.get("DUPL_ATTN_F1", "1") != "0"
+
+
+def fmt1_exponent(bound: float, margin: float = 2.0, cap: int = ops.EXP_ACT) -> int:
+    b = float(bound)
+    for s in range(int(cap), 0, -1):
+        if b * 2.0 ** s * float(margin) <= F16_MAX:
+            return s
+    return 0
 SK_DGRAD = os.environ.get("DUPL_SK_DGRAD", "1") != "0"
 WGRAD_GROUP = os.environ.get("DUPL_WGRAD_GROUP", "1") != "0"
 
@@ -331,6 +340,9 @@
         self._event.record()
         self._pending = True
 
+    def attn_exp(self, bound: float) -> int:
+        return fmt1_exponent(bound, self.margin, ops.EXP_ACT) if (FMT1 and ATTN_F1) else 0
+
     def _harvest(self, wait: bool):
         if not self._pending:
             return
@@ -394,6 +406,9 @@
             ops_ = {"qkv": (el1, amax(p + "attn.qkv.weight")), "proj": (e_qkv, amax(p + "attn.proj.weight")),
                     "fc1": (el2, amax(p + "mlp.fc1.weight")), "fc2": (e_h, amax(p + "mlp.fc2.weight"))}
             blk = {"attn": ok(e_qkv)}
+            blk["attn_f1"] = self.attn_exp(e_qkv) if blk["attn"] else 0
+            if blk["attn_f1"]:
+                worst1[0] = max(worst1[0], e_qkv * 2.0 ** blk["attn_f1"])
             for site, (ea_, ew_) in ops_.items():
                 blk[site] = ok(ea_, ew_)
                 blk[site + "_f1"] = exp1(ea_, ew_) if blk[site] else 0
@@ -436,6 +451,8 @@
             if FMT1:
                 n0 += int(s["patch"] and not s["patch_f1"]) + sum(b[k] and not b[k + "_f1"] for b in s["blocks"]
                                                                   for k in ("qkv", "proj", "fc1", "fc2"))
+                if ATTN_F1 and self.store.cfg.head_dim == 64:
+                    n0 += sum(bool(b["attn"]) and not b.get("attn_f1", 0) for b in s["blocks"])
         return {"sites_on_f32": n, "sites_on_fmt0": n0, "checks": self.checks, "margin": self.margin,
                 "headroom": (None if self.headroom == float("inf") else round(self.headroom, 1)),
                 "headroom_fmt1": (None if self.headroom1 == float("inf") else round(self.headroom1, 1))}
@@ -601,12 +618,13 @@
                                                   exp=ea(g, "qkv"))
         lse = None
         need_qkv32 = (not attn16) or (save and groups[0][2] > 2048)
+        qe = int(g.get("attn_f1", 0)) if (attn16 and FMT1 and ATTN_F1 and (ln1_16.exp > 0 or not g["qkv"])) else 0
         if g["qkv"]:
             qkv, qkv16 = _lin16(P, ln1_16, P.w16(p + "attn.qkv.weight", 3 * D, bool(ln1_16.exp)), W[p + "attn.qkv.bias"],
-                                      want_f32=need_qkv32, want16=attn16)
+                                      want_f32=need_qkv32, want16=attn16, out_exp=qe)
         else:
             qkv = ops.linear(ln1, W[p + "attn.qkv.weight"], W[p + "attn.qkv.bias"])
-            qkv16 = ops.split16(qkv) if attn16 else None
+            qkv16 = ops.split16(qkv, exp=qe) if attn16 else None
         ln1_keep = ln1_16 if km["qkv"] else None
         del ln1_16
         need_att32 = save or not g["proj"]
diff --git a/dupl_amd/ops.py b/dupl_amd/ops.py
--- a/dupl_amd/ops.py
+++ b/dupl_amd/ops.py
@@ -485,15 +485,19 @@
     lse = torch.empty((bf, H, N), device=dev, dtype=torch.float32) if need_lse else None
     if out is not None:
         assert out.shape == (bf * N, H * hd) and out.is_contiguous()
-    assert getattr(qkv16, "exp", 0) == 0, "the split attention reads format 0 planes"
-    L().dupl_attention_fwd16(qkv16.hi, qkv16.lo, _p(out), out16.hi if out16 is not None else None,
-                              out16.lo if out16 is not None else None, _p(lse), B, N, H, hd, float(scale), bf,
-                              out16.exp if out16 is not None else 0, _stream())
+    qe = int(getattr(qkv16, "exp", 0))
+    a = (qkv16.hi, qkv16.lo, _p(out), out16.hi if out16 is not None else None, out16.lo if out16 is not None else None, _p(lse),
+         B, N, H, hd, float(scale), bf, out16.exp if out16 is not None else 0)
+    if qe:
+        L().dupl_attention_fwd16_f1(*a, qe, _stream())
+    else:
+        L().dupl_attention_fwd16(*a, _stream())
     return lse
 
 
 def attention_fwd16_segs(qkv16, segs, H: int, hd: int, scale: float, out16=None):
-    assert hd == 64 and 1 <= len(segs) <= _lib.ATTN_SEGS_MAX and getattr(qkv16, "exp", 0) == 0
+    assert hd == 64 and 1 <= len(segs) <= _lib.ATTN_SEGS_MAX
+    qe = int(getattr(qkv16, "exp", 0))
     dev = qkv16.planes.device if isinstance(qkv16, Split16) else qkv16.base.planes.device
     arr = (_lib.AttnSeg * len(segs))()
     lses = []
@@ -506,9 +510,12 @@
         lses.append(lse)
         arr[i].row0, arr[i].B, arr[i].N, arr[i].B_f32 = int(row0), int(B), int(N), int(b_f32)
         arr[i].out, arr[i].lse = _p(out), _p(lse)
-    L().dupl_attention_fwd16_segs(qkv16.hi, qkv16.lo, out16.hi if out16 is not None else None,
-                                   out16.lo if out16 is not None else None, ctypes.cast(arr, ctypes.c_void_p), len(segs), H, hd,
-                                   float(scale), out16.exp if out16 is not None else 0, _stream())
+    a = (qkv16.hi, qkv16.lo, out16.hi if out16 is not None else None, out16.lo if out16 is not None else None,
+         ctypes.cast(arr, ctypes.c_void_p), len(segs), H, hd, float(scale), out16.exp if out16 is not None else 0)
+    if qe:
+        L().dupl_attention_fwd16_segs_f1(*a, qe, _stream())
+    else:
+        L().dupl_attention_fwd16_segs(*a, _stream())
     return lses
 
 
@@ -522,8 +529,13 @@
     delta = torch.empty((B, H, N), device=dev, dtype=torch.float32)
     dqkv = torch.empty((B * N, 3 * H * hd), device=dev, dtype=torch.float32)
     word, tok = reserve_amax(dev) if amax_for_next else (None, None)
-    L().dupl_attention_bwd16(qkv16.hi, qkv16.lo, out.data_ptr(), dout.data_ptr(), do16.hi, do16.lo, int(alpha) - 4, lse.data_ptr(),
-                             delta.data_ptr(), dqkv.data_ptr(), B, N, H, hd, float(scale), word, _stream())
+    a = (qkv16.hi, qkv16.lo, out.data_ptr(), dout.data_ptr(), do16.hi, do16.lo, int(alpha) - 4, lse.data_ptr(), delta.data_ptr(),
+         dqkv.data_ptr(), B, N, H, hd, float(scale))
+    qe = int(getattr(qkv16, "exp", 0))
+    if qe:
+        L().dupl_attention_bwd16_f1(*a, qe, word, _stream())
+    else:
+        L().dupl_attention_bwd16(*a, word, _stream())
     if tok is not None:
         dqkv._dupl_amax = tok
     return dqkv
diff --git a/include/dupl_hip.h b/include/dupl_hip.h
--- a/include/dupl_hip.h
+++ b/include/dupl_hip.h
@@ -125,6 +125,12 @@
 } dupl_attn_seg;
 int dupl_attention_fwd16_segs(const void* qkv_hi, const void* qkv_lo, void* out_hi, void* out_lo, const dupl_attn_seg* segs, int32_t n,
                               int32_t H, int32_t hd, float scale, int32_t out_exp, dupl_stream_t s);
+int dupl_attention_fwd16_f1(const void* qkv_hi, const void* qkv_lo, float* out, void* out_hi, void* out_lo, float* lse, int32_t B,
+                            int32_t N, int32_t H, int32_t hd, float scale, int32_t B_f32, int32_t out_exp, int32_t qkv_exp,
+                            dupl_stream_t s);
+int dupl_attention_fwd16_segs_f1(const void* qkv_hi, const void* qkv_lo, void* out_hi, void* out_lo, const dupl_attn_seg* segs, int32_t n,
+                                 int32_t H, int32_t hd, float scale, int32_t out_exp, int32_t qkv_exp, dupl_stream_t s);
+int dupl_attention_f1_set_shape(int32_t waves, int32_t key_tile);
 int dupl_attention_bwd(const float* qkv, const float* out, const float* dout, const float* lse,
                        float* delta, float* dqkv, int32_t B, int32_t N, int32_t H, int32_t hd,
                        float scale, dupl_stream_t s);
@@ -224,6 +230,9 @@
 int dupl_attention_bwd16(const void* qkv_hi, const void* qkv_lo, const float* out, const float* dout, const void* do_hi,
                          const void* do_lo, const float* do_slot, const float* lse, float* delta, float* dqkv, int32_t B, int32_t N,
                          int32_t H, int32_t hd, float scale, void* amax_out, dupl_stream_t stream);
+int dupl_attention_bwd16_f1(const void* qkv_hi, const void* qkv_lo, const float* out, const float* dout, const void* do_hi,
+                            const void* do_lo, const float* do_slot, const float* lse, float* delta, float* dqkv, int32_t B, int32_t N,
+                            int32_t H, int32_t hd, float scale, int32_t qkv_exp, void* amax_out, dupl_stream_t stream);
 
 int dupl_aug_to_u8(const float* x, uint8_t* out, int64_t n, dupl_stream_t s);
 int dupl_aug_lut_op(uint8_t* img, int32_t H, int32_t W, int32_t mode, uint32_t* hist_scratch, uint8_t* lut_scratch,
```

New measurement: 79.26 (median of 6 runs). About the same (+0.8%).
